# RozDavid/UnScene3D

Measured on AMD Instinct MI355X. Metric: training scenes/sec (Res16UNet34C+Mask3D, 150k voxels), higher is better.
Workload: dtype f32

## Files before the change

include/usc3d.h:

```cpp
#ifndef USC3D_H
#define USC3D_H

#include <stdint.h>

#ifdef __cplusplus
extern "C" {
#endif

typedef void* usc_stream_t;

enum usc_status {
  USC_OK = 0,
  USC_ERR_ARG = -1,
  USC_ERR_LAUNCH = -2,
  USC_ERR_RANGE = -3
};

const char* usc_last_error(void);
int usc_abi_version(void);
const char* usc_build_info(void);
int usc_device_count(void);


int usc_voxel_floor_f64(const double* xyz, int64_t n, double voxel_size,
                        int32_t* coords_out, usc_stream_t s);

int usc_voxel_floor_f64_host(const double* xyz, int64_t n, double voxel_size,
                             int32_t* coords_out);
int usc_unique_coords_host(const int32_t* coords, int64_t n, int32_t d,
                           int64_t* unique_idx, int64_t* inverse,
                           int64_t* n_out);

int64_t usc_coordmap_capacity(int64_t n);
int64_t usc_coordmap_ws_bytes(int64_t n);

int usc_coordmap_build(const int32_t* coords, int64_t n, int32_t quant,
                       uint64_t* table_keys, int32_t* table_vals, int64_t cap,
                       int64_t* unique_idx, int64_t* inverse,
                       int32_t* out_coords, int64_t* n_out,
                       void* ws, int64_t ws_bytes, usc_stream_t s);

int usc_morton_cell_ids(const int32_t* coords, int64_t n, int32_t shift,
                        int32_t lo_x, int32_t lo_y, int32_t lo_z,
                        int32_t bits_per_axis, int64_t* ids, usc_stream_t s);


int usc_kernel_map_cube(const int32_t* coords, int64_t n, int32_t tensor_stride,
                        int32_t ksize, const uint64_t* table_keys,
                        const int32_t* table_vals, int64_t cap, int32_t* nbr,
                        usc_stream_t s);

int usc_kernel_map_down2(const int32_t* fine_coords, int64_t n_fine,
                         int32_t tensor_stride, const int64_t* parent,
                         const int32_t* coarse_coords, int64_t n_coarse,
                         int32_t* nbr2, uint8_t* kidx, usc_stream_t s);

int64_t usc_rulebook_ws_bytes(int64_t K, int64_t n_out);
int usc_rulebook_compact(const int32_t* nbr, int64_t K, int64_t n_out,
                         int32_t* in_idx, int32_t* out_idx, int64_t* koff,
                         void* ws, int64_t ws_bytes, usc_stream_t s);


int usc_weight_transpose(const float* W, int32_t K, int32_t cin, int32_t cout,
                         int32_t mirror, float* out, usc_stream_t s);

int usc_spconv_plan(int32_t kind, int64_t n, int32_t cin, int32_t cout,
                    int32_t K);
int64_t usc_rowsort_ws_bytes(int32_t K, int64_t n_out);
int usc_rowsort_build(const int32_t* nbr, int32_t K, int64_t n_out,
                      int32_t* perm, uint32_t* tile_mask, void* ws,
                      int64_t ws_bytes, usc_stream_t s);
int64_t usc_spconv_sorted_ws_bytes(int64_t n_out, int32_t cin, int32_t cout,
                                   int32_t K);
int usc_spconv_sorted_gemm(const float* in, int64_t n_in, int32_t cin,
                           const float* W, int32_t K, int32_t cout,
                           const int32_t* nbr, const int32_t* perm,
                           const uint32_t* tile_mask, int64_t n_out,
                           const float* bias, float* out, int32_t accumulate,
                           int32_t w_transposed, void* ws, int64_t ws_bytes,
                           usc_stream_t s);
int usc_spconv_sorted_gemm_ex(const float* in, int64_t n_in, int32_t cin,
                              const float* W, int32_t K, int32_t cout,
                              const int32_t* nbr, const int32_t* perm,
                              const uint32_t* tile_mask, int64_t n_out,
                              const float* bias, float* out, int32_t accumulate,
                              int32_t w_transposed, void* ws, int64_t ws_bytes,
                              int32_t* slices_left, usc_stream_t s);
int usc_group_reduce(const float* partial, int32_t G, int64_t n, int32_t c,
                     const float* bias, int32_t accumulate, float* out,
                     usc_stream_t s);

int64_t usc_spconv_gather_gemm_ws_bytes(int64_t n_out, int32_t cin,
                                        int32_t cout, int32_t K);
int usc_spconv_gather_gemm(const float* in, int64_t n_in, int32_t cin,
                           const float* W, int32_t K, int32_t cout,
                           const int32_t* nbr, int64_t n_out,
                           const float* bias, float* out, int32_t accumulate, int32_t w_transposed,
                           void* ws, int64_t ws_bytes, usc_stream_t s);

int usc_spconv_pairs_gemm(const float* in, int32_t cin, const float* W,
                          int32_t K, int32_t cout, const int32_t* rows_in,
                          const int32_t* rows_out, const int64_t* koff,
                          int64_t P_capacity, float* out, usc_stream_t s);

int usc_cast_bf16(const float* in, int64_t n, uint16_t* out, usc_stream_t s);
int usc_spconv_pack_w_bf16(const float* W, int32_t K, int32_t cin, int32_t cout,
                           uint16_t* Wp, usc_stream_t s);
int64_t usc_spconv_gather_gemm_bf16_ws_bytes(int64_t n_out, int32_t cin,
                                             int32_t cout, int32_t K);
int usc_spconv_gather_gemm_bf16(const uint16_t* in, int64_t n_in, int32_t cin,
                                const uint16_t* Wp, int32_t K, int32_t cout,
                                const int32_t* nbr, int64_t n_out,
                                const float* bias, float* out, int32_t accumulate,
                                void* ws, int64_t ws_bytes, usc_stream_t s);

int usc_split_bf16_rows(const float* in, int64_t rows, int32_t c, int32_t P,
                        uint16_t* out, usc_stream_t s);
int usc_split_bf16(const float* in, int64_t n, int32_t P, uint16_t* out,
                   usc_stream_t s);
int usc_spconv_pack_w_split(const float* W, int32_t K, int32_t cin, int32_t cout,
                            int32_t P, int32_t transposed, uint16_t* Wp,
                            usc_stream_t s);
int64_t usc_spconv_gather_gemm_split_ws_bytes(int64_t n_out, int32_t cin,
                                              int32_t cout, int32_t K, int32_t P);
int usc_spconv_gather_gemm_split(const uint16_t* in, int64_t n_in, int32_t cin,
                                 const uint16_t* Wp, int32_t K, int32_t cout,
                                 int32_t P, const int32_t* nbr, int64_t n_out,
                                 const float* bias, float* out,
                                 int32_t accumulate, void* ws, int64_t ws_bytes,
                                 usc_stream_t s);

int64_t usc_spconv_wgrad_ws_bytes(int32_t K, int32_t cin, int32_t cout);
int usc_spconv_wgrad(const float* a, int32_t cin, const float* b, int32_t cout,
                     int32_t K, const int32_t* a_idx, const int32_t* b_idx,
                     const int64_t* koff, int64_t n_rows, float* dW, int32_t accumulate, void* ws,
                     int64_t ws_bytes, usc_stream_t s);
int64_t usc_spconv_wgrad_ws_bytes_rows(int32_t K, int32_t cin, int32_t cout,
                                       int64_t n_rows);
int64_t usc_spconv_wgrad_table_ws_bytes(int32_t K, int32_t cin, int32_t cout);
int usc_spconv_wgrad_table(const float* in, int32_t cin, const float* dy, int32_t cout, const int32_t* nbr, int32_t K,
                           int64_t n_out, float* dW, int32_t accumulate, void* ws, int64_t ws_bytes, usc_stream_t s);

void usc_spconv_wgrad_grid_limit(int32_t max_workgroups);
int32_t usc_spconv_wgrad_group_max(void);
int usc_spconv_wgrad_group_ok(int32_t R, int32_t cin, int32_t cout, int32_t K, int64_t n_rows);
int usc_spconv_wgrad_group(int32_t R, const float* const* a, const float* const* b, float* const* dW, int32_t cin,
                           int32_t cout, int32_t K, const int32_t* a_idx, const int32_t* b_idx, const int64_t* koff,
                           int64_t n_rows, int32_t accumulate, usc_stream_t s);

typedef struct usc_kmap {
  const int32_t* nbr;
  const int32_t* perm;
  const uint32_t* tile_mask;
  const int32_t* pair_in;
  const int32_t* pair_out;
  const int64_t* koff;
  int64_t n_in, n_out;
  int64_t pair_capacity;
  int32_t K;
  int32_t reserved;
} usc_kmap;

enum usc_conv_kind { USC_CONV_SAME = 0, USC_CONV_DOWN = 1, USC_CONV_UP = 2 };

typedef struct usc_bn {
  const float* gamma;
  const float* beta;
  float* running_mean;
  float* running_var;
  int64_t* num_batches_tracked;
  float eps, momentum;
  int32_t c;
  int32_t training;
} usc_bn;

int usc_set_wgrad_lane(usc_stream_t lane, void* lane_ws, int64_t lane_ws_bytes, int64_t max_rows);
int usc_wgrad_lane_join(usc_stream_t s);
int usc_wgrad_lane_hold(int32_t mode, int64_t hold_min_rows, int64_t release_max_rows, usc_stream_t s);
int32_t usc_wgrad_lane_holding(void);
typedef struct usc_launch_stat { int64_t n_out; int32_t cin, cout, K, nb; } usc_launch_stat;
int usc_launch_stats_begin(void* ring_dev, int64_t slots, usc_stream_t s);
int64_t usc_launch_stats_end(usc_launch_stat* host_out, int64_t max_out);
int64_t usc_wall_clock_khz(void);
int64_t usc_conv_ws_bytes(const usc_kmap* m, int32_t kind, int32_t cin,
                          int32_t cout);
int64_t usc_unit_ws_bytes(const usc_kmap* m, int32_t kind, int32_t cin,
                          int32_t cout);
int usc_conv_forward(const usc_kmap* m, int32_t kind, const float* x,
                     int32_t cin, const float* W, int32_t cout,
                     const float* bias, float* y, void* ws, int64_t ws_bytes,
                     usc_stream_t s);
int usc_conv_backward(const usc_kmap* m, int32_t kind, const float* x,
                      int32_t cin, const float* W, int32_t cout,
                      const float* dy, float* dx, int32_t dx_accumulate,
                      float* dW, int32_t dW_accumulate, void* ws,
                      int64_t ws_bytes, usc_stream_t s);
int usc_bn_eval_stats(const float* gamma, const float* beta,
                      const float* running_mean, const float* running_var,
                      float eps, int32_t c, float* mean, float* invstd,
                      float* scale, float* shift, usc_stream_t s);
int usc_conv_bn_act_forward(const usc_kmap* m, int32_t kind, const float* x,
                            int32_t cin, const float* W, int32_t cout,
                            const usc_bn* bn, const float* residual,
                            int32_t relu, float* y, float* stats, float* out,
                            void* ws, int64_t ws_bytes, usc_stream_t s);
int usc_conv_bn_act_backward(const usc_kmap* m, int32_t kind, const float* x,
                             int32_t cin, const float* W, int32_t cout,
                             const usc_bn* bn, const float* y,
                             const float* stats, const float* out_relu,
                             const float* dout, float* dy, float* dres,
                             float* dx, int32_t dx_accumulate, float* dW,
                             int32_t dW_accumulate, float* dgamma,
                             float* dbeta, int32_t dbn_accumulate, void* ws,
                             int64_t ws_bytes, usc_stream_t s);
int64_t usc_unit_bf16_ws_bytes(const usc_kmap* m, int32_t kind, int32_t cin,
                               int32_t cout);
int usc_conv_bn_act_forward_bf16(const usc_kmap* m, int32_t kind,
                                 const float* x, int32_t cin,
                                 const uint16_t* Wp, int32_t cout,
                                 const usc_bn* bn, const float* residual,
                                 int32_t relu, float* y, float* stats,
                                 float* out, void* ws, int64_t ws_bytes,
                                 usc_stream_t s);

int64_t usc_unit_split_ws_bytes(const usc_kmap* m, int32_t kind, int32_t cin,
                                int32_t cout, int32_t P);
int usc_conv_bn_act_forward_split(const usc_kmap* m, int32_t kind,
                                  const float* x, int32_t cin, const float* W,
                                  int32_t cout, int32_t P, const usc_bn* bn,
                                  const float* residual, int32_t relu, float* y,
                                  float* stats, float* out, void* ws,
                                  int64_t ws_bytes, usc_stream_t s);
int usc_conv_bn_act_backward_split(const usc_kmap* m, int32_t kind,
                                   const float* x, int32_t cin, const float* W,
                                   int32_t cout, int32_t P, const usc_bn* bn,
                                   const float* y, const float* stats,
                                   const float* out_relu, const float* dout,
                                   float* dy, float* dres, float* dx,
                                   int32_t dx_accumulate, float* dW,
                                   int32_t dW_accumulate, float* dgamma,
                                   float* dbeta, int32_t dbn_accumulate,
                                   void* ws, int64_t ws_bytes, usc_stream_t s);

enum usc_step_op { USC_STEP_UNIT_FWD = 0, USC_STEP_UNIT_BWD = 1, USC_STEP_CAT = 2, USC_STEP_SPLIT = 3, USC_STEP_ADD = 4,
                   USC_STEP_UNIT_FWD_BF16 = 5 };
typedef struct usc_step {
  int32_t op, kind, cin, cout, relu;
  int32_t dx_accumulate, dW_accumulate, dbn_accumulate, defer_wgrad, accumulate;
  const usc_kmap* map;
  const usc_bn* bn;
  const float* x;
  const float* W;
  const float* residual;
  float* y;
  float* stats;
  float* out;
  const float* dout;
  float* dy;
  float* dres;
  float* dx;
  float* dW;
  float* dgamma;
  float* dbeta;
  const float* a;
  const float* b;
  float* dst;
  float* dst2;
  int64_t n;
  int32_t ca, cb;
  int32_t split_planes, reserved;
} usc_step;
int32_t usc_step_size(void);
int64_t usc_program_ws_bytes(const usc_step* steps, int32_t n_steps);
int usc_program_run(const usc_step* steps, int32_t begin, int32_t end, void* ws, int64_t ws_bytes, usc_stream_t s);


int64_t usc_colstats_ws_bytes(int64_t n, int32_t c);
int usc_colstats(const float* x, const float* y, int64_t n, int32_t c,
                 double* sum1, double* sum2, void* ws, int64_t ws_bytes,
                 usc_stream_t s);
int usc_bn_forward_stats(const float* x, int64_t n, int32_t c, const float* gamma,
                         const float* beta, float eps, float momentum,
                         float* running_mean, float* running_var, int64_t* num_batches_tracked, float* mean,
                         float* invstd, float* scale, float* shift, void* ws,
                         int64_t ws_bytes, usc_stream_t s);
int usc_bn_apply(const float* x, const float* scale, const float* shift,
                 const float* residual, int32_t relu, float* y, int64_t n,
                 int32_t c, usc_stream_t s);
int usc_bn_backward_dx(const float* x, const float* dy, const float* y_out,
                       const float* mean, const float* invstd,
                       const float* gamma, const float* mean_g,
                       const float* mean_gxhat, float* dx, float* dres,
                       int64_t n, int32_t c, usc_stream_t s);
int64_t usc_bn_tile_max_rows(void);
int64_t usc_bn_plan(int64_t n, int32_t c, int32_t backward);
int usc_bn_tile_ok(int64_t n, int32_t c);
int64_t usc_bn_tile_ws_bytes(int32_t c);
int usc_bn_tile_forward(const float* partial, int32_t G, float* y, int64_t n,
                        int32_t c, const float* gamma, const float* beta,
                        float eps, float momentum, float* running_mean,
                        float* running_var, int64_t* num_batches_tracked,
                        float* mean, float* invstd, float* scale, float* shift,
                        const float* residual, int32_t relu, float* out,
                        void* ws, int64_t ws_bytes, usc_stream_t s);
int usc_bn_tile_backward(const float* partial, int32_t G, int32_t accumulate,
                         float* dout, const float* y, const float* y_out,
                         const float* mean, const float* invstd,
                         const float* gamma, int64_t n, int32_t c,
                         int32_t training, int32_t dbn_accumulate,
                         float* dgamma, float* dbeta, float* dy, float* dres,
                         void* ws, int64_t ws_bytes, usc_stream_t s);
int usc_bn_backward_reduce(const float* x, const float* dy, const float* y_out,
                           const float* mean, const float* invstd, int64_t n,
                           int32_t c, int32_t training, int32_t accumulate, float* dgamma,
                           float* dbeta, float* mean_g, float* mean_gxhat,
                           void* ws, int64_t ws_bytes, usc_stream_t s);
int usc_relu_fwd(const float* x, float* y, int64_t numel, usc_stream_t s);
int usc_relu_bwd(const float* y, const float* dy, float* dx, int64_t numel,
                 usc_stream_t s);

int usc_avgpool_down2(const float* in, int32_t c, const int32_t* nbr2,
                      int64_t n_coarse, float* out, usc_stream_t s);
int usc_avgpool_down2_ex(const float* in, int32_t c, int32_t ld,
                         const int64_t* row_of, const int32_t* nbr2,
                         int64_t n_coarse, float* out, uint8_t* mask_out,
                         usc_stream_t s);

int usc_gather_rows(const float* src, int32_t c, const int64_t* idx, int64_t n,
                    float* out, usc_stream_t s);

int usc_scatter_add_rows(const float* src, int32_t c, const int64_t* idx,
                         int64_t n, float* dst, usc_stream_t s);

int usc_scatter_rows_unique(const float* src, int32_t c, const int64_t* idx,
                            int64_t n, float* dst, usc_stream_t s);
int usc_scatter_rows_unique_add(const float* src, int32_t c, const int64_t* idx,
                                int64_t n, float* dst, usc_stream_t s);

int64_t usc_sample_keys_ws_bytes(int32_t n_scenes, int32_t K, int32_t q);
int usc_sample_keys(const float* feats, int32_t c, const uint8_t* mask, int32_t q, const float* pos, int32_t p,
                    const int64_t* idx, int32_t n_scenes, int32_t K, const int32_t* n_valid, float* out_feats,
                    uint8_t* out_mask, float* out_pos, void* ws, int64_t ws_bytes, usc_stream_t s);

int64_t usc_segment_csr_ws_bytes(int64_t n, int64_t S);
int usc_segment_csr(const int64_t* seg, int64_t n, int64_t S, int64_t* order,
                    int64_t* seg_off, void* ws, int64_t ws_bytes,
                    usc_stream_t s);
int usc_segment_mean_fwd(const float* src, int32_t c, const int64_t* order,
                         const int64_t* seg_off, int64_t S, float* out,
                         usc_stream_t s);
int usc_segment_mean_bwd(const float* dout, int32_t c, const int64_t* seg,
                         const int64_t* seg_off, int64_t n, float* dsrc,
                         usc_stream_t s);

int usc_segment_mean_nonzero(const float* feats, int32_t d,
                             const int64_t* order, const int64_t* seg_off,
                             int64_t S, float* out, int64_t* nonzero_cnt,
                             usc_stream_t s);
int usc_segment_max_nonzero(const float* feats, int32_t d,
                            const int64_t* order, const int64_t* seg_off,
                            int64_t S, float* out, int64_t* nonzero_cnt,
                            usc_stream_t s);

int32_t usc_attn_max_queries(void);
int32_t usc_attn_lse_stride(int32_t L);
int64_t usc_attn_ws_bytes(int32_t L, int32_t S, int32_t B, int32_t H);
int usc_attn_fwd(const float* q, const float* k, const float* v,
                 const uint8_t* mask, int32_t L, int32_t S, int32_t B, int32_t H,
                 int32_t E, float* o, float* lse, void* ws, int64_t ws_bytes,
                 usc_stream_t s);
int usc_attn_bwd(const float* q, const float* k, const float* v,
                 const uint8_t* mask, const float* o, const float* lse,
                 const float* dO, int32_t L, int32_t S, int32_t B, int32_t H,
                 int32_t E, float* dq, float* dk, float* dv,
                 int32_t mask_bits_in_ws ,
                 void* ws, int64_t ws_bytes, usc_stream_t s);

int usc_self_attn_fwd(const float* q, const float* k, const float* v, int32_t L,
                      int32_t B, int32_t H, int32_t E, float* o, float* lse,
                      usc_stream_t s);
int usc_self_attn_bwd(const float* q, const float* k, const float* v, const float* o,
                      const float* lse, const float* dO, int32_t L, int32_t B,
                      int32_t H, int32_t E, float* dq, float* dk, float* dv,
                      usc_stream_t s);

int usc_lsap_batch(const float* cost, int32_t n_prob, int32_t nr, int32_t nc,
                   int64_t* row_ind, int64_t* col_ind, int32_t* status, usc_stream_t s);

int64_t usc_criterion_ws_bytes(int32_t L, int32_t S, int32_t T);
int usc_criterion_target_bits(const uint8_t* tm, int32_t T, int32_t max_targets, int32_t S,
                              uint32_t* bits, int32_t* cnt, usc_stream_t s);
int usc_criterion_costs(const float* const* masks, int32_t L, int32_t ld, int32_t S,
                        int32_t Q, int32_t T, int32_t max_targets, const uint32_t* bits,
                        const int32_t* cnt, const float* logits, int64_t ls_level, int64_t ls_q,
                        int32_t C, const int64_t* labels, float w_mask, float w_class,
                        float w_dice, float* cost, float* cmask, float* cdice, float* nmat,
                        float* ssum, float* logp, void* ws, int64_t ws_bytes, usc_stream_t s);
int usc_criterion_drop_counts(const float* const* masks, int32_t L, int32_t ld, int32_t S,
                              int32_t Q, int32_t T, int32_t max_targets, const uint32_t* bits,
                              const int64_t* src, const int64_t* tid, int32_t* counts,
                              usc_stream_t s);
int usc_criterion_losses(const float* cmask, const float* cdice, const float* logp,
                         const int64_t* src, const int64_t* tid, const int64_t* labels,
                         const float* class_w, int32_t L, int32_t Q, int32_t T,
                         int32_t max_targets, int32_t C, int32_t noobj, int32_t* tcls, float* part,
                         const int32_t* counts, const int32_t* cnt, float thresh, float* wts,
                         usc_stream_t s);
int usc_criterion_table(const float* parts, int32_t B, int32_t L, float* table,
                        float* den_tot, usc_stream_t s);
int usc_criterion_backward(const float* const* masks, float* const* dmasks, int32_t L,
                           int32_t ld, int32_t S, int32_t Q, int32_t T, int32_t max_targets,
                           const uint32_t* bits, const int32_t* cnt, const int64_t* src,
                           const int64_t* tid, const float* nmat, const float* ssum,
                           const float* logp, const int32_t* tcls, const float* class_w,
                           const float* gtable, const float* den_tot, int32_t C, int64_t ls_level,
                           int64_t ls_q, float* dlogits, const float* wts, usc_stream_t s);

int usc_linear_fwd(const float* x, const float* W, const float* b, int32_t M,
                   int32_t N, int32_t K, float* y, usc_stream_t s);
int usc_linear_bwd(const float* dy, const float* x, const float* W, int32_t M,
                   int32_t N, int32_t K, float* dx, float* dW, float* db,
                   int32_t accumulate, usc_stream_t s);
int usc_linear_fwd_ex(const float* x, const float* x2, const float* W,
                      const float* b, int32_t M, int32_t N, int32_t K,
                      int32_t relu, float* y, usc_stream_t s);
int usc_linear_fwd_pad(const float* x, const float* x2, const float* W, const float* b, int32_t M, int32_t N, int32_t K,
                       int32_t relu, float* y, int32_t M_pad, usc_stream_t s);
int usc_linear_fwd_split(const float* x, const float* x2, const float* W, const float* b, int32_t M, int32_t N, int32_t K,
                         int32_t x2_cols, int32_t split_cols, float* y, usc_stream_t s);
int usc_linear_bwd_ex(const float* dy, const float* y_relu, const float* x,
                      const float* x2, const float* W, int32_t M, int32_t N,
                      int32_t K, float* dx, const float* dx_add, float* dW,
                      float* db, int32_t accumulate, usc_stream_t s);
int usc_linear_bwd_ex2(const float* dy, const float* y_relu, const float* x, const float* x2, const float* W, int32_t M,
                       int32_t N, int32_t K, float* dx, const float* dx_add, const float* dx_add2, float* dx_b, float* dW,
                       float* db, int32_t accumulate, usc_stream_t s);
int usc_qkv_proj_bwd(const float* dy3, const float* x, const float* pos, const float* W, int32_t M, int32_t E, float* dx,
                     float* dx_b, const float* dres, float* dW, float* db, int32_t accumulate, usc_stream_t s);
int64_t usc_col_sum_ws_bytes(int64_t n, int32_t c);
int usc_col_sum(const float* x, int64_t n, int32_t c, float* out,
                int32_t accumulate, void* ws, int64_t ws_bytes, usc_stream_t s);

int usc_layernorm_fwd(const float* x, const float* gamma, const float* beta,
                      int64_t rows, int32_t d, float eps, float* y, float* mean,
                      float* rstd, usc_stream_t s);
int usc_add_layernorm_fwd(const float* x, const float* res, const float* gamma,
                          const float* beta, int64_t rows, int32_t d, float eps,
                          float* y, float* sum_out, float* mean, float* rstd,
                          usc_stream_t s);
int64_t usc_layernorm_bwd_ws_bytes(int64_t rows, int32_t d);
int usc_layernorm_bwd(const float* dy, const float* x, const float* mean,
                      const float* rstd, const float* gamma, int64_t rows,
                      int32_t d, float* dx, float* dgamma, float* dbeta,
                      int32_t accumulate, void* ws, int64_t ws_bytes,
                      usc_stream_t s);
int usc_layernorm_bwd_ex(const float* dy, const float* x, const float* mean,
                         const float* rstd, const float* gamma, int64_t rows,
                         int32_t d, const float* dx_add, float* dx, float* dgamma,
                         float* dbeta, int32_t accumulate, void* ws,
                         int64_t ws_bytes, usc_stream_t s);

int usc_furthest_point_sampling(const float* xyz, int32_t b, int32_t n,
                                int32_t m, float* tmp, int32_t* idx,
                                usc_stream_t s);

int usc_fourier_posenc(const float* xyz, int64_t n, const float* lo,
                       const float* hi, const float* gauss_B, int32_t d,
                       float* out, usc_stream_t s);

int usc_ncut_similarity(const float* F, int64_t S, int32_t d,
                        int32_t cosine_mode, float* normed, float* sim,
                        usc_stream_t s);
int usc_ncut_similarity_masked(const float* F, const uint8_t* zero_rows, int64_t S,
                               int32_t d, int32_t cosine_mode, float* normed,
                               float* sim, usc_stream_t s);
int usc_ncut_normalize_mat(float* A, int64_t S, void* ws, int64_t ws_bytes,
                           usc_stream_t s);
int usc_ncut_binarize(const float* simA, const float* simB, int64_t S, float tau,
                      double eps, const uint8_t* painted, uint8_t* Abin,
                      double* deg, usc_stream_t s);
int64_t usc_ncut_fiedler_ws_bytes(int64_t S);
int usc_ncut_fiedler(const uint8_t* Abin, const double* deg, int64_t S, double eps,
                     double* evec, double* eval, void* ws, int64_t ws_bytes,
                     usc_stream_t s);
int usc_ncut_fiedler_ex(const uint8_t* Abin, const double* deg, int64_t S, double eps,
                        double* evec, double* eval, void* ws, int64_t ws_bytes,
                        usc_stream_t s, int32_t flags);
int32_t usc_ncut_fiedler_plan(int64_t S, int32_t cus, int32_t flags);

int usc_knn1(const float* query, int64_t nq, const float* ref, int64_t nr,
             int64_t* idx, float* dist2, usc_stream_t s);

int usc_cc_eps_init(int32_t* label, int64_t n, usc_stream_t s);
int usc_cc_eps_step(const float* xyz, int64_t n, float eps,
                    const int32_t* label_in, int32_t* label_out,
                    int32_t* changed, usc_stream_t s);
int usc_cc_eps_finish(const int32_t* label, int64_t n, int32_t* rank_ws,
                      int64_t* labels, usc_stream_t s);

int usc_project_planes_fwd(const int32_t* coords, const float* pred,
                           const float* target, int64_t V, int32_t inst,
                           int32_t dim_x, int32_t dim_y, int32_t dim_z,
                           float* pred_xy, float* pred_xz, float* pred_yz,
                           float* tgt_xy, float* tgt_xz, float* tgt_yz,
                           int32_t* cnt_xy, int32_t* cnt_xz, int32_t* cnt_yz,
                           usc_stream_t s);
int usc_project_planes_bwd(const int32_t* coords, int64_t V, int32_t inst,
                           int32_t dim_x, int32_t dim_y, int32_t dim_z,
                           const float* g_xy, const float* g_xz,
                           const float* g_yz, float* grad_pred,
                           usc_stream_t s);

int usc_brick_mask_build(const int32_t* coords, int64_t n, const int32_t* shift, int32_t B,
                         int32_t bricks_x, int32_t bricks_y, int32_t bricks_z,
                         uint32_t* mask, usc_stream_t s);
int usc_raycast_first_hit_map(const uint64_t* table_keys, const int32_t* table_vals,
                              int64_t cap, int64_t n_rows, const int32_t* shift,
                              const uint32_t* brick_mask , int32_t bricks_x,
                              int32_t bricks_y, int32_t bricks_z,
                              const float* views, const float* intrinsics,
                              int32_t B, int32_t V, int32_t H, int32_t W,
                              float depth_min, float depth_max, float ray_increment,
                              int32_t* hit, int64_t* seg, usc_stream_t s);
int usc_raycast_first_hit_dense(const int64_t* occupancy, int32_t dim_z, int32_t dim_y,
                                int32_t dim_x, int64_t n_rows, const float* views,
                                const float* intrinsics, int32_t B, int32_t V,
                                int32_t H, int32_t W, float depth_min, float depth_max,
                                float ray_increment, int32_t* hit, int64_t* seg,
                                usc_stream_t s);
int usc_project_reduce(const float* feats, int32_t c, const int64_t* order,
                       const int64_t* seg_off, int64_t n_rows, int32_t mode,
                       float* out, int32_t* num, usc_stream_t s);
int usc_project_predictions(const int32_t* preds, int32_t c, const int32_t* hit,
                            int64_t n_pix, int32_t* out, usc_stream_t s);
int usc_unproject_depth(const float* depth, const float* views, const float* intrinsics,
                        int32_t V, int32_t H, int32_t W, float* cloud, usc_stream_t s);

int usc_spin(int64_t microseconds, int wgs, usc_stream_t s);

int usc_adamw_step(float* param, const float* grad, float* exp_avg, float* exp_avg_sq,
                   int64_t n, float lr, float beta1, float beta2, float eps,
                   float weight_decay, int64_t step, usc_stream_t s);

int usc_adamw_step_scaled(float* param, float* grad, float* exp_avg, float* exp_avg_sq, int64_t n,
                          float grad_scale, int32_t write_back_grad,
                          float lr, float beta1, float beta2, float eps, float weight_decay,
                          int64_t step, usc_stream_t s);

int usc_elastic_displace(const void* xyz_in, int32_t is_f64, int64_t n, int32_t row_stride,
                         const float* noise, int32_t dim_x, int32_t dim_y, int32_t dim_z,
                         const double* axis_x, const double* axis_y, const double* axis_z,
                         double magnitude, void* xyz_out, usc_stream_t s);

int usc_affine_rows(void* x, int32_t is_f64, int64_t n, int32_t row_stride,
                    const double* M, const double* t, usc_stream_t s);
int usc_colsum_sequential(const float* x, int64_t n, int32_t row_stride,
                          int32_t cols, float* out, usc_stream_t s);
int usc_color_lut(const float* color, int64_t n, int32_t row_stride,
                  const float* lut, float* out, int32_t out_stride,
                  usc_stream_t s);

int usc_felz_face_normals(const float* vertices, const int32_t* faces,
                          int64_t n_faces, float* face_normals, usc_stream_t s);
int usc_felz_vertex_normals(const float* face_normals, const int64_t* corner_order,
                            const int64_t* vertex_off, int64_t n_vertices,
                            float* normals, usc_stream_t s);
int usc_felz_edge_weights(const float* vertices, const float* colors,
                          const float* normals, const int32_t* faces,
                          int64_t n_faces, int32_t* edge_a, int32_t* edge_b,
                          float* weights, usc_stream_t s);
int usc_felz_merge_host(const int32_t* edge_a, const int32_t* edge_b,
                        const float* weights, int64_t n_edges, int32_t n_vertices,
                        float kthr, int32_t seg_min_verts, int32_t* comps);

int usc_mask_gt_overlap(const uint8_t* masks, int64_t n, int32_t k, int64_t ld,
                        const int32_t* slot, int32_t nslots, int32_t* counts,
                        usc_stream_t s);
// ... 20 lines not shown
```

unscene3d_amd/_lib.py:

```python
from __future__ import annotations

import ctypes as C
import os

import torch

_HERE = os.path.dirname(os.path.abspath(__file__))
LIB_PATH = os.environ.get("USC3D_LIB") or os.path.join(_HERE, "libusc3d_hip.so")

_p = C.c_void_p
_i32 = C.c_int32
_i64 = C.c_int64
_f64 = C.c_double
_f32 = C.c_float

class KMap(C.Structure):
    _fields_ = [("nbr", _p), ("perm", _p), ("tile_mask", _p), ("pair_in", _p), ("pair_out", _p), ("koff", _p),
                ("n_in", _i64), ("n_out", _i64), ("pair_capacity", _i64), ("K", _i32), ("reserved", _i32)]


class BNDesc(C.Structure):
    _fields_ = [("gamma", _p), ("beta", _p), ("running_mean", _p), ("running_var", _p), ("num_batches_tracked", _p),
                ("eps", _f32), ("momentum", _f32), ("c", _i32), ("training", _i32)]


_kp = C.POINTER(KMap)
_bp = C.POINTER(BNDesc)


class Step(C.Structure):
    _fields_ = [("op", _i32), ("kind", _i32), ("cin", _i32), ("cout", _i32), ("relu", _i32),
                ("dx_accumulate", _i32), ("dW_accumulate", _i32), ("dbn_accumulate", _i32), ("defer_wgrad", _i32),
                ("accumulate", _i32),
                ("map", _p), ("bn", _p),
                ("x", _p), ("W", _p), ("residual", _p), ("y", _p), ("stats", _p), ("out", _p),
                ("dout", _p), ("dy", _p), ("dres", _p), ("dx", _p), ("dW", _p), ("dgamma", _p), ("dbeta", _p),
                ("a", _p), ("b", _p), ("dst", _p), ("dst2", _p), ("n", _i64), ("ca", _i32), ("cb", _i32),
                ("split_planes", _i32), ("reserved", _i32)]


_sp = C.POINTER(Step)
STEP_UNIT_FWD, STEP_UNIT_BWD, STEP_CAT, STEP_SPLIT, STEP_ADD, STEP_UNIT_FWD_BF16 = 0, 1, 2, 3, 4, 5

SIGNATURES = {
    "usc_last_error": (C.c_char_p, []),
    "usc_abi_version": (C.c_int, []),
    "usc_build_info": (C.c_char_p, []),
    "usc_device_count": (C.c_int, []),
    "usc_voxel_floor_f64": (C.c_int, [_p, _i64, _f64, _p, _p]),
    "usc_voxel_floor_f64_host": (C.c_int, [_p, _i64, C.c_double, _p]),
    "usc_unique_coords_host": (C.c_int, [_p, _i64, _i32, _p, _p, _p]),
    "usc_coordmap_capacity": (_i64, [_i64]),
    "usc_coordmap_ws_bytes": (_i64, [_i64]),
    "usc_coordmap_build": (C.c_int, [_p, _i64, _i32, _p, _p, _i64, _p, _p, _p, _p, _p, _i64, _p]),
    "usc_morton_cell_ids": (C.c_int, [_p, _i64, _i32, _i32, _i32, _i32, _i32, _p, _p]),
    "usc_kernel_map_cube": (C.c_int, [_p, _i64, _i32, _i32, _p, _p, _i64, _p, _p]),
    "usc_kernel_map_down2": (C.c_int, [_p, _i64, _i32, _p, _p, _i64, _p, _p, _p]),
    "usc_rulebook_ws_bytes": (_i64, [_i64, _i64]),
    "usc_rulebook_compact": (C.c_int, [_p, _i64, _i64, _p, _p, _p, _p, _i64, _p]),
    "usc_weight_transpose": (C.c_int, [_p, _i32, _i32, _i32, _i32, _p, _p]),
    "usc_spconv_plan": (C.c_int, [_i32, _i64, _i32, _i32, _i32]),
    "usc_spconv_gather_gemm_ws_bytes": (_i64, [_i64, _i32, _i32, _i32]),
    "usc_spconv_gather_gemm": (C.c_int, [_p, _i64, _i32, _p, _i32, _i32, _p, _i64, _p, _p, _i32, _i32, _p, _i64, _p]),
    "usc_rowsort_ws_bytes": (_i64, [_i32, _i64]),
    "usc_rowsort_build": (C.c_int, [_p, _i32, _i64, _p, _p, _p, _i64, _p]),
    "usc_spconv_sorted_ws_bytes": (_i64, [_i64, _i32, _i32, _i32]),
    "usc_spconv_sorted_gemm": (C.c_int, [_p, _i64, _i32, _p, _i32, _i32, _p, _p, _p, _i64, _p, _p, _i32, _i32, _p, _i64, _p]),
    "usc_spconv_sorted_gemm_ex": (C.c_int, [_p, _i64, _i32, _p, _i32, _i32, _p, _p, _p, _i64, _p, _p, _i32, _i32, _p, _i64, _p, _p]),
    "usc_group_reduce": (C.c_int, [_p, _i32, _i64, _i32, _p, _i32, _p, _p]),
    "usc_bn_tile_max_rows": (C.c_int64, []),
    "usc_bn_plan": (_i64, [_i64, _i32, _i32]),
    "usc_bn_tile_ok": (C.c_int, [_i64, _i32]),
    "usc_bn_tile_ws_bytes": (C.c_int64, [_i32]),
    "usc_bn_tile_forward": (C.c_int, [_p, _i32, _p, _i64, _i32, _p, _p, _f32, _f32, _p, _p, _p, _p, _p, _p, _p, _p, _i32, _p,
                                      _p, _i64, _p]),
    "usc_bn_tile_backward": (C.c_int, [_p, _i32, _i32, _p, _p, _p, _p, _p, _p, _i64, _i32, _i32, _i32, _p, _p, _p, _p, _p,
                                       _i64, _p]),
    "usc_spconv_pairs_gemm": (C.c_int, [_p, _i32, _p, _i32, _i32, _p, _p, _p, _i64, _p, _p]),
    "usc_cast_bf16": (C.c_int, [_p, _i64, _p, _p]),
    "usc_spconv_pack_w_bf16": (C.c_int, [_p, _i32, _i32, _i32, _p, _p]),
    "usc_spconv_gather_gemm_bf16_ws_bytes": (_i64, [_i64, _i32, _i32, _i32]),
    "usc_spconv_gather_gemm_bf16": (C.c_int, [_p, _i64, _i32, _p, _i32, _i32, _p, _i64, _p, _p, _i32, _p, _i64, _p]),
    "usc_split_bf16_rows": (C.c_int, [_p, _i64, _i32, _i32, _p, _p]),
    "usc_split_bf16": (C.c_int, [_p, _i64, _i32, _p, _p]),
    "usc_spconv_pack_w_split": (C.c_int, [_p, _i32, _i32, _i32, _i32, _i32, _p, _p]),
    "usc_spconv_gather_gemm_split_ws_bytes": (_i64, [_i64, _i32, _i32, _i32, _i32]),
    "usc_spconv_gather_gemm_split": (C.c_int, [_p, _i64, _i32, _p, _i32, _i32, _i32, _p, _i64, _p, _p, _i32, _p, _i64, _p]),
    "usc_spconv_wgrad_ws_bytes": (_i64, [_i32, _i32, _i32]),
    "usc_spconv_wgrad": (C.c_int, [_p, _i32, _p, _i32, _i32, _p, _p, _p, _i64, _p, _i32, _p, _i64, _p]),
    "usc_spconv_wgrad_ws_bytes_rows": (_i64, [_i32, _i32, _i32, _i64]),
    "usc_step_size": (_i32, []),
    "usc_program_ws_bytes": (_i64, [_sp, _i32]),
    "usc_program_run": (C.c_int, [_sp, _i32, _i32, _p, _i64, _p]),
    "usc_spconv_wgrad_group_max": (_i32, []),
    "usc_spconv_wgrad_grid_limit": (None, [_i32]),
    "usc_spconv_wgrad_group_ok": (C.c_int, [_i32, _i32, _i32, _i32, _i64]),
    "usc_spconv_wgrad_group": (C.c_int, [_i32, _p, _p, _p, _i32, _i32, _i32, _p, _p, _p, _i64, _i32, _p]),
    "usc_spconv_wgrad_table_ws_bytes": (_i64, [_i32, _i32, _i32]),
    "usc_spconv_wgrad_table": (C.c_int, [_p, _i32, _p, _i32, _p, _i32, _i64, _p, _i32, _p, _i64, _p]),
    "usc_set_wgrad_lane": (C.c_int, [_p, _p, _i64, _i64]),
    "usc_wgrad_lane_join": (C.c_int, [_p]),
    "usc_wgrad_lane_hold": (C.c_int, [_i32, _i64, _i64, _p]),
    "usc_wgrad_lane_holding": (_i32, []),
    "usc_launch_stats_begin": (C.c_int, [_p, _i64, _p]),
    "usc_launch_stats_end": (_i64, [_p, _i64]),
    "usc_wall_clock_khz": (_i64, []),
    "usc_conv_ws_bytes": (_i64, [_kp, _i32, _i32, _i32]),
    "usc_unit_ws_bytes": (_i64, [_kp, _i32, _i32, _i32]),
    "usc_conv_forward": (C.c_int, [_kp, _i32, _p, _i32, _p, _i32, _p, _p, _p, _i64, _p]),
    "usc_conv_backward": (C.c_int, [_kp, _i32, _p, _i32, _p, _i32, _p, _p, _i32, _p, _i32, _p, _i64, _p]),
    "usc_bn_eval_stats": (C.c_int, [_p, _p, _p, _p, _f32, _i32, _p, _p, _p, _p, _p]),
    "usc_conv_bn_act_forward": (C.c_int, [_kp, _i32, _p, _i32, _p, _i32, _bp, _p, _i32, _p, _p, _p, _p, _i64, _p]),
    "usc_unit_bf16_ws_bytes": (_i64, [_kp, _i32, _i32, _i32]),
    "usc_conv_bn_act_forward_bf16": (C.c_int, [_kp, _i32, _p, _i32, _p, _i32, _bp, _p, _i32, _p, _p, _p, _p, _i64, _p]),
    "usc_unit_split_ws_bytes": (_i64, [_kp, _i32, _i32, _i32, _i32]),
    "usc_conv_bn_act_forward_split": (C.c_int, [_kp, _i32, _p, _i32, _p, _i32, _i32, _bp, _p, _i32, _p, _p, _p, _p, _i64, _p]),
    "usc_conv_bn_act_backward_split": (C.c_int, [_kp, _i32, _p, _i32, _p, _i32, _i32, _bp, _p, _p, _p, _p, _p, _p, _p, _i32, _p,
                                                 _i32, _p, _p, _i32, _p, _i64, _p]),
    "usc_conv_bn_act_backward": (C.c_int, [_kp, _i32, _p, _i32, _p, _i32, _bp, _p, _p, _p, _p, _p, _p, _p, _i32, _p,
                                           _i32, _p, _p, _i32, _p, _i64, _p]),
    "usc_colstats_ws_bytes": (_i64, [_i64, _i32]),
    "usc_colstats": (C.c_int, [_p, _p, _i64, _i32, _p, _p, _p, _i64, _p]),
    "usc_bn_apply": (C.c_int, [_p, _p, _p, _p, _i32, _p, _i64, _i32, _p]),
    "usc_bn_backward_dx": (C.c_int, [_p, _p, _p, _p, _p, _p, _p, _p, _p, _p, _i64, _i32, _p]),
    "usc_bn_backward_reduce": (C.c_int, [_p, _p, _p, _p, _p, _i64, _i32, _i32, _i32, _p, _p, _p, _p, _p, _i64, _p]),
    "usc_bn_forward_stats": (C.c_int, [_p, _i64, _i32, _p, _p, _f32, _f32, _p, _p, _p, _p, _p, _p, _p, _p, _i64, _p]),
    "usc_relu_fwd": (C.c_int, [_p, _p, _i64, _p]),
    "usc_relu_bwd": (C.c_int, [_p, _p, _p, _i64, _p]),
    "usc_avgpool_down2": (C.c_int, [_p, _i32, _p, _i64, _p, _p]),
    "usc_avgpool_down2_ex": (C.c_int, [_p, _i32, _i32, _p, _p, _i64, _p, _p, _p]),
    "usc_gather_rows": (C.c_int, [_p, _i32, _p, _i64, _p, _p]),
    "usc_scatter_add_rows": (C.c_int, [_p, _i32, _p, _i64, _p, _p]),
    "usc_scatter_rows_unique": (C.c_int, [_p, _i32, _p, _i64, _p, _p]),
    "usc_scatter_rows_unique_add": (C.c_int, [_p, _i32, _p, _i64, _p, _p]),
    "usc_sample_keys_ws_bytes": (_i64, [_i32, _i32, _i32]),
    "usc_sample_keys": (C.c_int, [_p, _i32, _p, _i32, _p, _i32, _p, _i32, _i32, _p, _p, _p, _p, _p, _i64, _p]),
    "usc_segment_csr_ws_bytes": (_i64, [_i64, _i64]),
    "usc_segment_csr": (C.c_int, [_p, _i64, _i64, _p, _p, _p, _i64, _p]),
    "usc_segment_mean_fwd": (C.c_int, [_p, _i32, _p, _p, _i64, _p, _p]),
    "usc_segment_mean_bwd": (C.c_int, [_p, _i32, _p, _p, _i64, _p, _p]),
    "usc_segment_mean_nonzero": (C.c_int, [_p, _i32, _p, _p, _i64, _p, _p, _p]),
    "usc_segment_max_nonzero": (C.c_int, [_p, _i32, _p, _p, _i64, _p, _p, _p]),
    "usc_ncut_similarity": (C.c_int, [_p, _i64, _i32, _i32, _p, _p, _p]),
    "usc_ncut_similarity_masked": (C.c_int, [_p, _p, _i64, _i32, _i32, _p, _p, _p]),
    "usc_ncut_normalize_mat": (C.c_int, [_p, _i64, _p, _i64, _p]),
    "usc_ncut_binarize": (C.c_int, [_p, _p, _i64, _f32, _f64, _p, _p, _p, _p]),
    "usc_ncut_fiedler_ws_bytes": (_i64, [_i64]),
    "usc_ncut_fiedler": (C.c_int, [_p, _p, _i64, _f64, _p, _p, _p, _i64, _p]),
    "usc_ncut_fiedler_ex": (C.c_int, [_p, _p, _i64, _f64, _p, _p, _p, _i64, _p, _i32]),
    "usc_ncut_fiedler_plan": (_i32, [_i64, _i32, _i32]),
    "usc_knn1": (C.c_int, [_p, _i64, _p, _i64, _p, _p, _p]),
    "usc_cc_eps_init": (C.c_int, [_p, _i64, _p]),
    "usc_cc_eps_step": (C.c_int, [_p, _i64, _f32, _p, _p, _p, _p]),
    "usc_cc_eps_finish": (C.c_int, [_p, _i64, _p, _p, _p]),
    "usc_project_planes_fwd": (C.c_int, [_p, _p, _p, _i64, _i32, _i32, _i32, _i32] + [_p] * 10),
    "usc_project_planes_bwd": (C.c_int, [_p, _i64, _i32, _i32, _i32, _i32, _p, _p, _p, _p, _p]),
    "usc_brick_mask_build": (C.c_int, [_p, _i64, _p, _i32, _i32, _i32, _i32, _p, _p]),
    "usc_raycast_first_hit_map": (C.c_int, [_p, _p, _i64, _i64, _p, _p, _i32, _i32, _i32, _p, _p, _i32, _i32, _i32, _i32,
                                            _f32, _f32, _f32, _p, _p, _p]),
    "usc_raycast_first_hit_dense": (C.c_int, [_p, _i32, _i32, _i32, _i64, _p, _p, _i32, _i32, _i32, _i32, _f32, _f32,
                                              _f32, _p, _p, _p]),
    "usc_project_reduce": (C.c_int, [_p, _i32, _p, _p, _i64, _i32, _p, _p, _p]),
    "usc_project_predictions": (C.c_int, [_p, _i32, _p, _i64, _p, _p]),
    "usc_unproject_depth": (C.c_int, [_p, _p, _p, _i32, _i32, _i32, _p, _p]),
    "usc_spin": (C.c_int, [_i64, C.c_int, _p]),
    "usc_adamw_step": (C.c_int, [_p, _p, _p, _p, _i64, _f32, _f32, _f32, _f32, _f32, _i64, _p]),
    "usc_adamw_step_scaled": (C.c_int, [_p, _p, _p, _p, _i64, _f32, _i32, _f32, _f32, _f32, _f32, _f32, _i64, _p]),
    "usc_elastic_displace": (C.c_int, [_p, _i32, _i64, _i32, _p, _i32, _i32, _i32, _p, _p, _p, _f64, _p, _p]),
    "usc_attn_max_queries": (_i32, []),
    "usc_attn_lse_stride": (_i32, [_i32]),
    "usc_attn_ws_bytes": (_i64, [_i32, _i32, _i32, _i32]),
    "usc_attn_fwd": (C.c_int, [_p, _p, _p, _p, _i32, _i32, _i32, _i32, _i32, _p, _p, _p, _i64, _p]),
    "usc_attn_bwd": (C.c_int, [_p, _p, _p, _p, _p, _p, _p, _i32, _i32, _i32, _i32, _i32, _p, _p, _p, _i32, _p, _i64, _p]),
    "usc_lsap_batch": (C.c_int, [_p, _i32, _i32, _i32, _p, _p, _p, _p]),
    "usc_criterion_ws_bytes": (_i64, [_i32, _i32, _i32]),
    "usc_criterion_target_bits": (C.c_int, [_p, _i32, _i32, _i32, _p, _p, _p]),
    "usc_criterion_costs": (C.c_int, [_p, _i32, _i32, _i32, _i32, _i32, _i32, _p, _p, _p, _i64, _i64, _i32, _p, _f32, _f32,
                                      _f32, _p, _p, _p, _p, _p, _p, _p, _i64, _p]),
    "usc_criterion_drop_counts": (C.c_int, [_p, _i32, _i32, _i32, _i32, _i32, _i32, _p, _p, _p, _p, _p]),
    "usc_criterion_losses": (C.c_int, [_p, _p, _p, _p, _p, _p, _p, _i32, _i32, _i32, _i32, _i32, _i32, _p, _p, _p, _p,
                                       _f32, _p, _p]),
    "usc_criterion_table": (C.c_int, [_p, _i32, _i32, _p, _p, _p]),
    "usc_criterion_backward": (C.c_int, [_p, _p, _i32, _i32, _i32, _i32, _i32, _i32, _p, _p, _p, _p, _p, _p, _p, _p, _p,
                                         _p, _p, _i32, _i64, _i64, _p, _p, _p]),
    "usc_self_attn_fwd": (C.c_int, [_p, _p, _p, _i32, _i32, _i32, _i32, _p, _p, _p]),
    "usc_self_attn_bwd": (C.c_int, [_p, _p, _p, _p, _p, _p, _i32, _i32, _i32, _i32, _p, _p, _p, _p]),
    "usc_linear_fwd": (C.c_int, [_p, _p, _p, _i32, _i32, _i32, _p, _p]),
    "usc_linear_bwd": (C.c_int, [_p, _p, _p, _i32, _i32, _i32, _p, _p, _p, _i32, _p]),
    "usc_layernorm_fwd": (C.c_int, [_p, _p, _p, _i64, _i32, _f32, _p, _p, _p, _p]),
    "usc_add_layernorm_fwd": (C.c_int, [_p, _p, _p, _p, _i64, _i32, _f32, _p, _p, _p, _p, _p]),
    "usc_linear_fwd_ex": (C.c_int, [_p, _p, _p, _p, _i32, _i32, _i32, _i32, _p, _p]),
    "usc_linear_fwd_pad": (C.c_int, [_p, _p, _p, _p, _i32, _i32, _i32, _i32, _p, _i32, _p]),
    "usc_linear_fwd_split": (C.c_int, [_p, _p, _p, _p, _i32, _i32, _i32, _i32, _i32, _p, _p]),
    "usc_linear_bwd_ex": (C.c_int, [_p, _p, _p, _p, _p, _i32, _i32, _i32, _p, _p, _p, _p, _i32, _p]),
    "usc_qkv_proj_bwd": (C.c_int, [_p, _p, _p, _p, _i32, _i32, _p, _p, _p, _p, _p, _i32, _p]),
    "usc_linear_bwd_ex2": (C.c_int, [_p, _p, _p, _p, _p, _i32, _i32, _i32, _p, _p, _p, _p, _p, _p, _i32, _p]),
    "usc_layernorm_bwd_ws_bytes": (_i64, [_i64, _i32]),
    "usc_layernorm_bwd": (C.c_int, [_p, _p, _p, _p, _p, _i64, _i32, _p, _p, _p, _i32, _p, _i64, _p]),
    "usc_layernorm_bwd_ex": (C.c_int, [_p, _p, _p, _p, _p, _i64, _i32, _p, _p, _p, _p, _i32, _p, _i64, _p]),
    "usc_affine_rows": (C.c_int, [_p, _i32, _i64, _i32, _p, _p, _p]),
    "usc_colsum_sequential": (C.c_int, [_p, _i64, _i32, _i32, _p, _p]),
    "usc_col_sum_ws_bytes": (_i64, [_i64, _i32]),
    "usc_col_sum": (C.c_int, [_p, _i64, _i32, _p, _i32, _p, _i64, _p]),
    "usc_color_lut": (C.c_int, [_p, _i64, _i32, _p, _p, _i32, _p]),
    "usc_felz_face_normals": (C.c_int, [_p, _p, _i64, _p, _p]),
    "usc_felz_vertex_normals": (C.c_int, [_p, _p, _p, _i64, _p, _p]),
    "usc_felz_edge_weights": (C.c_int, [_p, _p, _p, _p, _i64, _p, _p, _p, _p]),
    "usc_felz_merge_host": (C.c_int, [_p, _p, _p, _i64, _i32, _f32, _i32, _p]),
    "usc_furthest_point_sampling": (C.c_int, [_p, _i32, _i32, _i32, _p, _p, _p]),
    "usc_fourier_posenc": (C.c_int, [_p, _i64, _p, _p, _p, _i32, _p, _p]),
    "usc_mask_gt_overlap": (C.c_int, [_p, _i64, _i32, _i64, _p, _i32, _p, _p]),
    "usc_vit_attn_head_dim": (_i32, []),
    "usc_vit_attn_fwd": (C.c_int, [_p, _i32, _i32, _i32, _f32, _i32, _p, _p]),
    "usc_instance_index": (C.c_int, [_p, _i64, _i32, _p, _i32, _p, _p, _p, _p]),
    "usc_instance_select": (C.c_int, [_p, _i64, _i32, _p, _i32, _p, _p, _p, _i32, _i64, _p, _p, _p, _p]),
    "usc_instance_masks": (C.c_int, [_p, _i64, _p, _i32, _i32, _p, _p, _i32, _i64, _p, _p]),
}


class LaunchStat(C.Structure):
    _fields_ = [("n_out", _i64), ("cin", _i32), ("cout", _i32), ("K", _i32), ("nb", _i32)]


def _load():
    if not os.path.exists(LIB_PATH):
        raise ImportError(
            f"{LIB_PATH} is missing: build the HIP extension first "
            "(`python -c 'import __graft_entry__ as g; g.build()'`). "
            "unscene3d_amd has no CPU fallback."
        )
    lib = C.CDLL(LIB_PATH)
    for name, (res, args) in SIGNATURES.items():
        fn = getattr(lib, name)
        fn.restype = res
        fn.argtypes = args
    return lib


lib = _load()
if lib.usc_step_size() != C.sizeof(Step):
    raise ImportError(f"unscene3d_amd._lib.Step ({C.sizeof(Step)} bytes) does not mirror usc_step "
                      f"({lib.usc_step_size()} bytes): rebuild the library or fix the binding")


def last_error() -> str:
    return lib.usc_last_error().decode("utf-8", "replace")


def check(rc: int, what: str = "") -> None:
    if rc != 0:
        raise RuntimeError(f"{what or 'libusc3d_hip'} failed (status {rc}): {last_error()}")


def require_device() -> None:
    n = lib.usc_device_count()
    if n <= 0:
        raise RuntimeError(
            "unscene3d_amd: no HIP device visible — the MI355X kernels cannot run and there is no CPU fallback"
        )
```

unscene3d_amd/csrc/spconv.hip:

```cpp
#include "common.h"

#include <stdlib.h>

#include <vector>

namespace usc {

typedef float f32x16 __attribute__((ext_vector_type(16)));

#define MFMA32(a, b, c) __builtin_amdgcn_mfma_f32_32x32x2f32((a), (b), (c), 0, 0, 0)

struct GemmParams {
  const float* in;
  const float* W;
  const int32_t* nbr;
  const float* bias;
  float* out;
  int64_t n_out;
  int cin, cout, K;
  int accumulate;
  int G;
  int TM;
  int wt1;
  const int32_t* rows_in;
// ... 585 lines not shown
  f32x16 acc[NB];
#pragma unroll
  for (int nb = 0; nb < NB; ++nb)
#pragma unroll
    for (int r = 0; r < 16; ++r) acc[nb][r] = 0.f;

  const bool ci_ok = ci0 + i < cin;
  const int acol = ci0 + i;
  const int bcol = ALIGNED ? co0 + NB * i : co0 + i;
  auto load_idx = [&](int64_t q) -> int64_t {
    int64_t idxreg = -1;
    const int l16 = lane & 15;
    const int64_t pp = q + l16;
    if (lane < 32 && pp < ce) {
      if (p.a_idx)
        idxreg = (lane < 16) ? p.a_idx[pp] : p.b_idx[pp];
      else
        idxreg = pp;
    }
    return idxreg;
  };
  auto load_rows = [&](int64_t idxreg, float (&av)[8], float (&bv)[8][NB]) {
#pragma unroll
    for (int u = 0; u < 8; ++u) {
      const int64_t ia = __shfl(idxreg, 2 * u + h, 64);
      const int64_t ib = __shfl(idxreg, 16 + 2 * u + h, 64);
      if (ALIGNED) {
        const float t = p.a[(ia >= 0 ? ia : 0) * cin + acol];
        av[u] = ia >= 0 ? t : 0.f;
        load_b<NB>(p.b + (ib >= 0 ? ib : 0) * cout + bcol, bv[u]);
      } else {
        av[u] = (ia >= 0 && ci_ok) ? p.a[ia * cin + acol] : 0.f;
#pragma unroll
        for (int nb = 0; nb < NB; ++nb)
          bv[u][nb] = (ib >= 0 && bcol + nb * 32 < cout) ? p.b[ib * cout + bcol + nb * 32] : 0.f;
      }
    }
  };
  auto run = [&](float (&av)[8], float (&bv)[8][NB]) {
#pragma unroll
    for (int u = 0; u < 8; ++u)
#pragma unroll
      for (int nb = 0; nb < NB; ++nb) acc[nb] = MFMA32(av[u], bv[u][nb], acc[nb]);
  };
  if (ALIGNED) {
    float aX[8], aY[8];
    float bX[8][NB], bY[8][NB];
    int64_t id1 = load_idx(cb), id2 = load_idx(cb + 16);
    load_rows(id1, aX, bX);
    for (int64_t q = cb; q < ce; q += 32) {
      int64_t id3 = load_idx(q + 32);
      load_rows(id2, aY, bY);
      run(aX, bX);
      id2 = load_idx(q + 48);
      load_rows(id3, aX, bX);
      if (q + 16 < ce) run(aY, bY);
    }
  } else {
    float av[8];
    float bv[8][NB];
    for (int64_t q = cb; q < ce; q += 16) {
      load_rows(load_idx(q), av, bv);
      run(av, bv);
    }
  }

  if (wave > 0) {
#pragma unroll
    for (int nb = 0; nb < NB; ++nb)
#pragma unroll
      for (int r = 0; r < 16; ++r) red[((wave - 1) * NB * 16 + nb * 16 + r) * 64 + lane] = acc[nb][r];
  }
  __syncthreads();
  if (wave == 0) {
#pragma unroll
    for (int w = 0; w < 3; ++w)
#pragma unroll
      for (int nb = 0; nb < NB; ++nb)
#pragma unroll
        for (int r = 0; r < 16; ++r) acc[nb][r] += red[(w * NB * 16 + nb * 16 + r) * 64 + lane];
    float* dst = p.partial + ((int64_t)s * p.K + k) * cin * cout;
#pragma unroll
    for (int r = 0; r < 16; ++r) {
      const int ci = ci0 + acc_row(r, h);
      if (ci >= cin) continue;
#pragma unroll
      for (int nb = 0; nb < NB; ++nb) {
        const int co = ALIGNED ? bcol + nb : bcol + nb * 32;
        if (co < cout) dst[(int64_t)ci * cout + co] = acc[nb][r];
      }
    }
  }
}

constexpr int kMaxWgradGroup = 16;
struct WgradGroup { const float* a[kMaxWgradGroup]; const float* b[kMaxWgradGroup]; float* dW[kMaxWgradGroup]; int R; };

template <int CT, int NB>
__global__ __launch_bounds__(256, (CT * NB > 9) ? 1 : 2) void wgrad_full_kernel(WgradParams p, WgradGroup g) {
  extern __shared__ float red[];
  constexpr int NA = CT * NB;
  const int lane = threadIdx.x & 63, wave = threadIdx.x >> 6;
  const int i = lane & 31, h = lane >> 5;
  const int vtotal = p.vblocks > 0 ? p.vblocks : (int)gridDim.x;
  for (int vb = blockIdx.x; vb < vtotal; vb += gridDim.x) {
  int bx = vb;
  if (g.R > 0) {
    const int per = p.K * p.S, r = bx / per;
    bx -= r * per;
    p.a = g.a[r]; p.b = g.b[r]; p.direct = g.dW[r];
  }
  const int k = bx / p.S, s = bx % p.S;
  const int ci0 = blockIdx.y * (32 * CT), co0 = blockIdx.z * (NB * 32);
  const int cin = p.cin, cout = p.cout;
  int64_t pb, pe;
  if (p.a_idx) { pb = p.koff[k]; pe = p.koff[k + 1]; } else { pb = 0; pe = p.n_rows; }
  const int64_t nchunks = (int64_t)p.S * 4;
  int64_t L = (pe - pb + nchunks - 1) / nchunks;
  L = (L + 7) & ~7ll;
  const int64_t cb = pb + ((int64_t)s * 4 + wave) * L;
  int64_t ce = cb + L;
  if (ce > pe) ce = pe;

  f32x16 acc[NA];
#pragma unroll
  for (int t = 0; t < NA; ++t)
#pragma unroll
    for (int r = 0; r < 16; ++r) acc[t][r] = 0.f;

  auto load_idx = [&](int64_t q) __attribute__((always_inline)) -> int {
    int v = -1;
    const int64_t pp = q + (lane & 7);
    if (lane < 16 && pp < ce) v = p.a_idx ? ((lane < 8) ? p.a_idx[pp] : p.b_idx[pp]) : (int)pp;
    return v;
  };
  auto load_rows = [&](int idxreg, float (&av)[4][CT], float (&bv)[4][NB]) __attribute__((always_inline)) {
#pragma unroll
    for (int u = 0; u < 4; ++u) {
      const int ia = __shfl(idxreg, 2 * u + h, 64);
      const int ib = __shfl(idxreg, 8 + 2 * u + h, 64);
      const float* ap = p.a + (int64_t)(ia >= 0 ? ia : 0) * cin + ci0 + CT * i;
      const float* bp = p.b + (int64_t)(ib >= 0 ? ib : 0) * cout + co0 + NB * i;
      const float keep = ia >= 0 ? 1.f : 0.f;
      load_b<CT>(ap, av[u]);
#pragma unroll
      for (int ct = 0; ct < CT; ++ct) av[u][ct] *= keep;
      load_b<NB>(bp, bv[u]);
    }
  };
  auto run = [&](float (&av)[4][CT], float (&bv)[4][NB]) __attribute__((always_inline)) {
#pragma unroll
    for (int u = 0; u < 4; ++u)
#pragma unroll
      for (int ct = 0; ct < CT; ++ct)
#pragma unroll
        for (int nb = 0; nb < NB; ++nb) acc[ct * NB + nb] = MFMA32(av[u][ct], bv[u][nb], acc[ct * NB + nb]);
  };
  float aX[4][CT], aY[4][CT], bX[4][NB], bY[4][NB];
  int id1 = load_idx(cb), id2 = load_idx(cb + 8);
  load_rows(id1, aX, bX);
  for (int64_t q = cb; q < ce; q += 16) {
    const int id3 = load_idx(q + 16);
    load_rows(id2, aY, bY);
    run(aX, bX);
    id2 = load_idx(q + 24);
    load_rows(id3, aX, bX);
    if (q + 8 < ce) run(aY, bY);
  }

  float* dst = (p.direct ? p.direct : p.partial + (int64_t)s * p.K * cin * cout) + (int64_t)k * cin * cout;
  const bool rmw = p.direct && p.accumulate;
  const bool vec_ok = (reinterpret_cast<uintptr_t>(dst) & (NB * 4 - 1)) == 0;
#pragma unroll
  for (int ct = 0; ct < CT; ++ct) {
    if (ct) __syncthreads();
#pragma unroll
    for (int nb = 0; nb < NB; ++nb)
#pragma unroll
      for (int r = 0; r < 16; ++r) red[((wave * NB + nb) * 16 + r) * 64 + lane] = acc[ct * NB + nb][r];
    __syncthreads();
#pragma unroll
    for (int rr = 0; rr < 4; ++rr) {
      const int r = 4 * wave + rr;
      float v[NB];
#pragma unroll
      for (int nb = 0; nb < NB; ++nb) {
        float t = red[((3 * NB + nb) * 16 + r) * 64 + lane];
        t += red[((2 * NB + nb) * 16 + r) * 64 + lane];
        t += red[((1 * NB + nb) * 16 + r) * 64 + lane];
        v[nb] = red[(nb * 16 + r) * 64 + lane] + t;
      }
      const int ci = ci0 + CT * acc_row(r, h) + ct;
      float* o = dst + (int64_t)ci * cout + co0 + NB * i;
      if (NB == 4 && vec_ok) {
        float4 w4 = make_float4(v[0], v[1], v[2 % NB], v[3 % NB]);
        if (rmw) {
          const float4 old = *reinterpret_cast<const float4*>(o);
          w4.x += old.x; w4.y += old.y; w4.z += old.z; w4.w += old.w;
        }
        *reinterpret_cast<float4*>(o) = w4;
      } else if (NB == 2 && vec_ok) {
        float2 w2 = make_float2(v[0], v[1 % NB]);
        if (rmw) {
          const float2 old = *reinterpret_cast<const float2*>(o);
          w2.x += old.x; w2.y += old.y;
        }
        *reinterpret_cast<float2*>(o) = w2;
      } else {
#pragma unroll
        for (int nb = 0; nb < NB; ++nb) o[nb] = rmw ? o[nb] + v[nb] : v[nb];
      }
    }
  }
  __syncthreads();
  }
}

constexpr int kStemSplits = 64;
constexpr int kStemWaves = 16;
__global__ __launch_bounds__(64 * kStemWaves) void stem_wgrad_kernel(const float* __restrict__ in, const float* __restrict__ dy,
                                                                    const int32_t* __restrict__ nbr, int64_t n_out, int K,
                                                                    int cin, float* __restrict__ partial) {
  __shared__ float red[kStemWaves][16][64];
  const int lane = threadIdx.x & 63, wave = threadIdx.x >> 6, i = lane & 31, h = lane >> 5;
  const int per = 32 / cin;
  const int g = blockIdx.y, s = blockIdx.x, S = gridDim.x;
  const int j = i / cin, c = i - j * cin, k = g * per + j;
  const bool active = j < per && k < K;
  int64_t L = (n_out + S - 1) / S;
  L = (L + 2 * kStemWaves - 1) / (2 * kStemWaves) * (2 * kStemWaves);
  const int64_t r_begin = (int64_t)s * L;
  int64_t r_end = r_begin + L;
  if (r_end > n_out) r_end = n_out;
  const int32_t* nk = nbr + (int64_t)(active ? k : 0) * n_out;
  f32x16 acc;
#pragma unroll
  for (int r = 0; r < 16; ++r) acc[r] = 0.f;
  for (int64_t rb = r_begin + 2 * wave; rb < r_end; rb += 8 * kStemWaves) {
    int id[4];
    float b[4];
#pragma unroll
    for (int u = 0; u < 4; ++u) {
      const int64_t r = rb + h + 2 * kStemWaves * u;
      const bool ok = r < r_end;
      id[u] = (ok && active) ? nk[r] : -1;
      b[u] = ok ? dy[r * 32 + i] : 0.f;
    }
    float a[4];
#pragma unroll
    for (int u = 0; u < 4; ++u) a[u] = id[u] >= 0 ? in[(int64_t)id[u] * cin + c] : 0.f;
#pragma unroll
    for (int u = 0; u < 4; ++u) acc = __builtin_amdgcn_mfma_f32_32x32x2f32(a[u], b[u], acc, 0, 0, 0);
  }
#pragma unroll
  for (int r = 0; r < 16; ++r) red[wave][r][lane] = acc[r];
  __syncthreads();
  if (wave >= 4) return;
  float* dst = partial + (int64_t)s * K * cin * 32;
#pragma unroll
  for (int q = 0; q < 4; ++q) {
    const int r = 4 * wave + q;
    const int m = acc_row(r, h);
    float v = red[kStemWaves - 1][r][lane];
#pragma unroll
    for (int w = kStemWaves - 2; w >= 0; --w) v += red[w][r][lane];
    const int row = g * per * cin + m;
    if (m < per * cin && row < K * cin) dst[(int64_t)row * 32 + i] = v;
  }
}

__global__ void wgrad_reduce_kernel(const float* __restrict__ partial, int S, int64_t numel, int accumulate,
                                    float* __restrict__ dW) {
  if ((numel & 3) == 0 && (reinterpret_cast<uintptr_t>(dW) & 15) == 0) {
    const int64_t n4 = numel >> 2;
    for (int64_t j = (int64_t)blockIdx.x * blockDim.x + threadIdx.x; j < n4; j += (int64_t)gridDim.x * blockDim.x) {
      float4 v = make_float4(0.f, 0.f, 0.f, 0.f);
      int s = 0;
      for (; s + 8 <= S; s += 8) {
        float4 t[8];
#pragma unroll
        for (int u = 0; u < 8; ++u) t[u] = reinterpret_cast<const float4*>(partial)[(int64_t)(s + u) * n4 + j];
#pragma unroll
        for (int u = 0; u < 8; ++u) { v.x += t[u].x; v.y += t[u].y; v.z += t[u].z; v.w += t[u].w; }
      }
      for (; s < S; ++s) {
        const float4 t = reinterpret_cast<const float4*>(partial)[(int64_t)s * n4 + j];
        v.x += t.x; v.y += t.y; v.z += t.z; v.w += t.w;
      }
      if (accumulate) {
        const float4 o = reinterpret_cast<const float4*>(dW)[j];
        v.x += o.x; v.y += o.y; v.z += o.z; v.w += o.w;
      }
      reinterpret_cast<float4*>(dW)[j] = v;
    }
    return;
  }
  for (int64_t j = (int64_t)blockIdx.x * blockDim.x + threadIdx.x; j < numel; j += (int64_t)gridDim.x * blockDim.x) {
    float v = 0.f;
    for (int s = 0; s < S; ++s) v += partial[(int64_t)s * numel + j];
    dW[j] = accumulate ? dW[j] + v : v;
  }
}

__global__ void weight_transpose_kernel(const float* __restrict__ W, int K, int cin, int cout, int mirror,
                                        float* __restrict__ out) {
  const int64_t per = (int64_t)cin * cout;
  const int64_t total = per * K;
  for (int64_t j = (int64_t)blockIdx.x * blockDim.x + threadIdx.x; j < total; j += (int64_t)gridDim.x * blockDim.x) {
    const int k = (int)(j / per);
    const int64_t rem = j - (int64_t)k * per;
    const int co = (int)(rem / cin), ci = (int)(rem - (int64_t)co * cin);
    const int ks = mirror ? (K - 1 - k) : k;
    out[j] = W[(int64_t)ks * per + (int64_t)ci * cout + co];
  }
}

__global__ void weight_pack_kernel(const float* __restrict__ W, int K, int cin, int cout, int NB, int wt,
                                   float* __restrict__ out) {
  const int64_t total = (int64_t)K * cin * cout;
  const int nq = cin >> 3, BN = NB * 32;
  for (int64_t e = (int64_t)blockIdx.x * blockDim.x + threadIdx.x; e < total; e += (int64_t)gridDim.x * blockDim.x) {
    int64_t r = e;
    const int j = (int)(r & 3); r >>= 2;
    const int ln = (int)(r & 63); r >>= 6;
    const int nb = (int)(r % NB); r /= NB;
    const int q = (int)(r % nq); r /= nq;
    const int k = (int)(r % K);
    const int cb = (int)(r / K);
    const int i = ln & 31, h = ln >> 5;
    const int c = 8 * q + 4 * h + j, n = cb * BN + NB * i + nb;
    out[e] = wt ? W[((int64_t)(K - 1 - k) * cout + n) * cin + c] : W[((int64_t)k * cin + c) * cout + n];
  }
}

static int wgrad_splits(int K, int cin, int cout, int NB, int64_t n_rows) {
  const int64_t tiles = (int64_t)K * ceil_div(cin, 32) * ceil_div(cout, NB * 32);
  const int target = (K > 1 && n_rows >= (int64_t)2 << 20) ? 4096 : 2048;
  int64_t S = ceil_div(target, tiles);
  const int64_t by_rows = n_rows / 2048 + 1;
  if (S > by_rows) S = by_rows;
  if (S > 64) S = 64;
  if (S < 1) S = 1;
  return (int)S;
}
static int wgrad_full_nb(int cb) { return (cb % 3 == 0) ? 3 : (cb % 4 == 0 ? 4 : (cb % 2 == 0 ? 2 : 1)); }
static int wgrad_full_ct(int ctiles, int NBf) {
  if (NBf == 3 && ctiles % 3 != 0 && ctiles % 4 == 0) return 4;
  return (ctiles % 3 == 0 && NBf * 3 <= 9) ? 3 : ((ctiles % 4 == 0 && NBf * 4 <= 9) ? 4 : ((ctiles % 2 == 0 && NBf * 2 <= 9) ? 2 : 1));
}
static int64_t wgrad_full_splits(int K, int ctiles, int cb, int CT, int NBf, int64_t n_rows) {
  const int64_t blocks_per_split = (int64_t)K * (ctiles / CT) * (cb / NBf);
  const int64_t tgt = (K > 1 && n_rows >= (int64_t)2 << 20) ? 2048 : 512;
  int64_t S = tgt / blocks_per_split;
  const int64_t by_rows = n_rows / (K > 1 ? 4096 : 256) + 1;
  if (S > by_rows) S = by_rows;
  if (S > 64) S = 64;
  if (S < 1) S = 1;
  return S;
}
static int pick_nb(int cout) {
  if (cout <= 32) return 1;
  if (cout <= 64) return 2;
  if (cout % 128 == 0) return 4;
  if (cout % 96 == 0) return 3;
  return 4;
}

struct GemmPlan { int NB; int G; bool aligned; int TM; };
constexpr int64_t kTargetWaves = 3072;

static bool stem_form(bool has_table, int cin, int cout, int K) {
  return has_table && cin >= 1 && cin <= 4 && cout == 32 && K >= 1 && K <= 32;
}

static GemmPlan plan_table(int64_t n_out, int cin, int cout, int K) {
  GemmPlan pl{pick_nb(cout), 1, false, 0};
  const bool al = (cin % 32 == 0) && (cout % 32 == 0);
  if (!al) return pl;
  pl.aligned = true;
  if (K > 1 && K <= kMaxK && n_out >= 24576 && cin >= 64 && cin <= kZeroRowFloats) {
    const int cb = cout / 32;
    const int nb = (cb % 3 == 0) ? 3 : (cb % 2 == 0 ? 2 : 1);
    constexpr int kTmMax3 = 192;
    constexpr int64_t kTileSlots = 256;
    const int tm_max = nb == 3 ? kTmMax3 : 256;
    int64_t R = 1;
    int64_t tm = ceil_div(n_out, kTileSlots * R);
    while (tm > tm_max) { ++R; tm = ceil_div(n_out, kTileSlots * R); }
    tm = (tm + 3) & ~3ll;
    pl.NB = nb;
    pl.TM = (int)tm;
    return pl;
  }
  const int64_t row_tiles = ceil_div(n_out, 32);
  const int cb = cout / 32;
  const int cands[4] = {4, 3, 2, 1};
  int chosen = 1;
  for (int c = 0; c < 4; ++c) {
    const int nb = cands[c];
    if (cb % nb) continue;
    if (row_tiles * (cb / nb) >= kTargetWaves) { chosen = nb; break; }
  }
  pl.NB = chosen;
  const int64_t waves = row_tiles * (cb / chosen);
  if (waves > 0 && waves < kTargetWaves && K > 1) {
    int64_t G = ceil_div(kTargetWaves, waves);
    if (G > K) G = K;
    pl.G = (int)G;
  }
  return pl;
}
static GemmPlan plan_list(int64_t max_tiles, int cin, int cout) {
  GemmPlan pl{pick_nb(cout), 1, false, 0};
  const bool al = (cin % 32 == 0) && (cout % 32 == 0);
  if (!al) return pl;
  pl.aligned = true;
  const int cb = cout / 32;
  const int cands[4] = {4, 3, 2, 1};
  int chosen = 1;
  for (int c = 0; c < 4; ++c) {
    const int nb = cands[c];
    if (cb % nb) continue;
    if (max_tiles * (cb / nb) >= kTargetWaves) { chosen = nb; break; }
  }
  pl.NB = chosen;
  return pl;
}

template <bool LIST>
static void launch_gemm(const GemmPlan& pl, dim3 grid, hipStream_t st, const GemmParams& p) {
#define USC_GG(NBv)                                                                                      \
  if (pl.aligned && p.wt1)        \
    hipLaunchKernelGGL((gather_gemm_aligned_kernel<NBv, false, true>), grid, dim3(256), 0, st, p);      \
  else if (pl.aligned)                                                                                   \
    hipLaunchKernelGGL((gather_gemm_aligned_kernel<NBv, LIST>), grid, dim3(256), 0, st, p);             \
  else                                                                                                   \
    hipLaunchKernelGGL((gather_gemm_kernel<NBv, LIST>), grid, dim3(256), 0, st, p);
  switch (pl.NB) {
    case 1: USC_GG(1) break;
    case 2: USC_GG(2) break;
    case 3: USC_GG(3) break;
    default: USC_GG(4) break;
  }
#undef USC_GG
}

}

using namespace usc;

extern "C" {

int usc_weight_transpose(const float* W, int32_t K, int32_t cin, int32_t cout, int32_t mirror, float* out,
                         usc_stream_t s) {
  USC_REQUIRE(W && out && K >= 1 && cin >= 1 && cout >= 1, "usc_weight_transpose: bad argument");
  const int64_t total = (int64_t)K * cin * cout;
  hipLaunchKernelGGL(weight_transpose_kernel, dim3(stream_grid(total, 256)), dim3(256), 0, as_stream(s), W, (int)K,
                     (int)cin, (int)cout, (int)mirror, out);
  USC_CHECK_LAUNCH("usc_weight_transpose");
  return USC_OK;
}

int usc_spconv_plan(int32_t kind, int64_t n, int32_t cin, int32_t cout, int32_t K) {
  GemmPlan pl;
  if (kind == 0 && stem_form(K > 1, cin, cout, K)) return 1 | (1 << 14);
  if (kind == 0) pl = plan_table(n, cin, cout, K);
  else if (kind == 1) pl = plan_list(ceil_div(n, 32) + K, cin, cout);
  else {
    const int ctiles = cin / 32, cb = cout / 32;
    const int NBf = (cb % 3 == 0) ? 3 : (cb % 4 == 0 ? 4 : (cb % 2 == 0 ? 2 : 1));
    if (cin % 32 == 0 && cout % 32 == 0 && (!(NBf == 3 && ctiles % 3 != 0) || ctiles % 4 == 0)) {
      const int CT = wgrad_full_ct(ctiles, NBf);
      return NBf | (1 << 8) | (1 << 13) | (CT << 16);
    }
    const int NB = pick_nb(cout);
    pl = GemmPlan{NB, 1, (cin % 32 == 0) && (cout % (NB * 32) == 0), 0};
  }
  return pl.NB | ((pl.aligned ? 1 : 0) << 8) | ((pl.TM > 0 ? 1 : 0) << 12) | (pl.G << 16);
}

int64_t usc_spconv_gather_gemm_ws_bytes(int64_t n_out, int32_t cin, int32_t cout, int32_t K) {
  const GemmPlan pl = plan_table(n_out, cin, cout, K);
  if (pl.TM > 0) return (int64_t)K * cin * cout * 4;
  return pl.G > 1 ? (int64_t)pl.G * n_out * cout * 4 : 0;
}

namespace {
struct LaunchStats { unsigned long long* ring = nullptr; int64_t slots = 0, count = 0; std::vector<usc_launch_stat> meta; };
LaunchStats g_lstats;
__global__ void launch_stats_init_kernel(unsigned long long* ring, int64_t slots) {
  const int64_t i = (int64_t)blockIdx.x * blockDim.x + threadIdx.x;
  if (i < slots) { ring[4 * i] = ~0ull; ring[4 * i + 1] = 0; ring[4 * i + 2] = 0; ring[4 * i + 3] = 0; }
}
}

int usc_launch_stats_begin(void* ring_dev, int64_t slots, usc_stream_t s) {
  USC_REQUIRE(ring_dev && slots > 0, "usc_launch_stats_begin: needs a device ring of slots x 4 x u64");
  hipLaunchKernelGGL(launch_stats_init_kernel, dim3((unsigned)ceil_div(slots, 256)), dim3(256), 0, as_stream(s),
                     (unsigned long long*)ring_dev, slots);
  USC_CHECK_LAUNCH("usc_launch_stats_begin");
  g_lstats.ring = (unsigned long long*)ring_dev;
  g_lstats.slots = slots;
  g_lstats.count = 0;
  g_lstats.meta.clear();
  g_lstats.meta.reserve((size_t)slots);
  return USC_OK;
}

int64_t usc_launch_stats_end(usc_launch_stat* host_out, int64_t max_out) {
  const int64_t n = g_lstats.count;
  if (host_out)
    for (int64_t i = 0; i < n && i < max_out; ++i) host_out[i] = g_lstats.meta[(size_t)i];
  g_lstats.ring = nullptr;
  g_lstats.slots = g_lstats.count = 0;
  g_lstats.meta.clear();
  return n;
}

int64_t usc_wall_clock_khz(void) {
  int dev = 0, khz = 0;
  if (hipGetDevice(&dev) != hipSuccess || hipDeviceGetAttribute(&khz, hipDeviceAttributeWallClockRate, dev) != hipSuccess) return 0;
  return khz;
}

int usc_spconv_gather_gemm(const float* in, int64_t n_in, int32_t cin, const float* W, int32_t K, int32_t cout,
                           const int32_t* nbr, int64_t n_out, const float* bias, float* out, int32_t accumulate,
                           int32_t w_transposed, void* ws, int64_t ws_bytes, usc_stream_t s) {
  USC_REQUIRE(cin >= 1 && cout >= 1 && K >= 1 && n_out >= 0 && n_in >= 0, "usc_spconv_gather_gemm: bad sizes");
  USC_REQUIRE(nbr || K == 1, "usc_spconv_gather_gemm: K>1 needs a neighbour table");
  USC_REQUIRE(nbr || n_in == n_out, "usc_spconv_gather_gemm: identity map needs n_in == n_out");
  if (n_out == 0) return USC_OK;
  USC_REQUIRE(in && W && out, "usc_spconv_gather_gemm: null pointer");
  if (stem_form(nbr != nullptr, cin, cout, K) && !accumulate && !w_transposed) {
    hipLaunchKernelGGL(stem_conv_kernel, dim3((unsigned)ceil_div(n_out, 256)), dim3(256), 0, as_stream(s), in, W, nbr, bias,
                       out, n_out, (int)K, (int)cin);
    USC_CHECK_LAUNCH("usc_spconv_gather_gemm");
    return USC_OK;
  }
  const GemmPlan pl = plan_table(n_out, cin, cout, K);
  GemmParams p{};
  p.in = in; p.W = W; p.nbr = nbr; p.bias = bias; p.out = out;
  p.n_out = n_out; p.cin = cin; p.cout = cout; p.K = K; p.accumulate = accumulate; p.G = pl.G;
  if (pl.G > 1) {
    USC_REQUIRE(ws && ws_bytes >= (int64_t)pl.G * n_out * cout * 4, "usc_spconv_gather_gemm: workspace too small");
    p.out = (float*)ws;
  }
  hipStream_t st = as_stream(s);
  const bool wt1 = w_transposed && K == 1 && !nbr && pl.aligned && pl.TM == 0;
  USC_REQUIRE(!w_transposed || pl.TM > 0 || wt1,
              "usc_spconv_gather_gemm: w_transposed is only folded into the tile-compacted kernel (usc_spconv_plan bit 12) "
              "and, for K = 1 on identity rows with channel counts in multiples of 32, into the row-order kernel; "
              "use usc_weight_transpose for other shapes");
  p.wt1 = wt1 ? 1 : 0;
  if (pl.TM > 0) {
    p.TM = pl.TM;
    USC_REQUIRE(ws && ws_bytes >= (int64_t)K * cin * cout * 4, "usc_spconv_gather_gemm: workspace too small");
    hipLaunchKernelGGL(weight_pack_kernel, dim3(stream_grid((int64_t)K * cin * cout, 256)), dim3(256), 0, st, W, (int)K,
                       (int)cin, (int)cout, pl.NB, (int)w_transposed, (float*)ws);
    p.W = (const float*)ws;
    dim3 cgrid((unsigned)ceil_div(n_out, pl.TM), (unsigned)(cout / (pl.NB * 32)));
    const size_t lds = compact_lds_bytes(pl.NB, pl.TM);
    if (g_lstats.ring && g_lstats.count < g_lstats.slots) {
      p.stats = g_lstats.ring + 4 * g_lstats.count++;
      g_lstats.meta.push_back(usc_launch_stat{n_out, cin, cout, K, pl.NB});
    }
#define USC_CG(NBv)                                                                                        \
    {                                                                                                      \
      static bool attr_set = false;                                                                        \
      auto kfn = gather_gemm_compact_kernel<NBv>;                                                          \
      if (!attr_set) {                                                                                     \
        (void)hipFuncSetAttribute((const void*)kfn, hipFuncAttributeMaxDynamicSharedMemorySize, 160 * 1024); \
        attr_set = true;                                                                                   \
      }                                                                                                    \
      hipLaunchKernelGGL(kfn, cgrid, dim3(64 * kCompactWaves), lds, st, p);                                \
    }
    if (pl.NB == 3) USC_CG(3) else if (pl.NB == 2) USC_CG(2) else USC_CG(1)
#undef USC_CG
    USC_CHECK_LAUNCH("usc_spconv_gather_gemm");
    return USC_OK;
  }
  dim3 grid((unsigned)ceil_div(n_out, 128), (unsigned)ceil_div(cout, pl.NB * 32), (unsigned)pl.G);
  launch_gemm<false>(pl, grid, st, p);
  if (pl.G > 1) {
    const int64_t numel4 = n_out * cout / 4;
    hipLaunchKernelGGL(group_reduce_kernel, dim3(stream_grid(numel4, 256)), dim3(256), 0, st, (const float*)ws, pl.G,
                       numel4, (int)cout, bias, (int)accumulate, out);
  }
  USC_CHECK_LAUNCH("usc_spconv_gather_gemm");
  return USC_OK;
}

int usc_spconv_pairs_gemm(const float* in, int32_t cin, const float* W, int32_t K, int32_t cout,
                          const int32_t* rows_in, const int32_t* rows_out, const int64_t* koff, int64_t P_capacity,
                          float* out, usc_stream_t s) {
  USC_REQUIRE(cin >= 1 && cout >= 1 && K >= 1 && P_capacity >= 0, "usc_spconv_pairs_gemm: bad sizes");
  if (P_capacity == 0) return USC_OK;
  USC_REQUIRE(in && W && rows_in && rows_out && koff && out, "usc_spconv_pairs_gemm: null pointer");
  GemmParams p{};
  p.in = in; p.W = W; p.out = out; p.cin = cin; p.cout = cout; p.K = K; p.G = 1;
  p.rows_in = rows_in; p.rows_out = rows_out; p.koff = koff;
  const int64_t max_tiles = ceil_div(P_capacity, 32) + K;
  const GemmPlan pl = plan_list(max_tiles, cin, cout);
  dim3 grid((unsigned)ceil_div(max_tiles, 4), (unsigned)ceil_div(cout, pl.NB * 32));
  launch_gemm<true>(pl, grid, as_stream(s), p);
  USC_CHECK_LAUNCH("usc_spconv_pairs_gemm");
  return USC_OK;
}

int64_t usc_spconv_wgrad_ws_bytes(int32_t K, int32_t cin, int32_t cout) {
  return (int64_t)64 * K * cin * cout * (int64_t)sizeof(float);
}

int64_t usc_spconv_wgrad_ws_bytes_rows(int32_t K, int32_t cin, int32_t cout, int64_t n_rows) {
  const int64_t numel = (int64_t)K * cin * cout;
  const int ctiles = cin / 32, cb = cout / 32;
  if (cin % 32 == 0 && cout % 32 == 0 && cb > 0) {
    const int NBf = wgrad_full_nb(cb);
    if (!(NBf == 3 && ctiles % 3 != 0) || ctiles % 4 == 0)
      return wgrad_full_splits(K, ctiles, cb, wgrad_full_ct(ctiles, NBf), NBf, n_rows) * numel * 4;
  }
  return (int64_t)wgrad_splits(K, cin, cout, pick_nb(cout), n_rows) * numel * 4;
}

int64_t usc_spconv_wgrad_table_ws_bytes(int32_t K, int32_t cin, int32_t cout) {
  return (int64_t)kStemSplits * K * cin * cout * 4;
}

int usc_spconv_wgrad_table(const float* in, int32_t cin, const float* dy, int32_t cout, const int32_t* nbr, int32_t K,
                           int64_t n_out, float* dW, int32_t accumulate, void* ws, int64_t ws_bytes, usc_stream_t s) {
  USC_REQUIRE(cin >= 1 && cin <= 4 && cout == 32 && K >= 1 && K <= 32 && n_out >= 0,
              "usc_spconv_wgrad_table: the table form covers <= 4 input channels and 32 output channels (the stem)");
  USC_REQUIRE(in && dy && nbr && dW && ws, "usc_spconv_wgrad_table: null pointer");
  USC_REQUIRE(ws_bytes >= usc_spconv_wgrad_table_ws_bytes(K, cin, cout), "usc_spconv_wgrad_table: workspace too small");
  hipStream_t st = as_stream(s);
  const int per = 32 / cin, groups = (K + per - 1) / per;
  const int64_t numel = (int64_t)K * cin * 32;
  hipLaunchKernelGGL(stem_wgrad_kernel, dim3(kStemSplits, (unsigned)groups), dim3(64 * kStemWaves), 0, st, in, dy, nbr, n_out, (int)K,
                     (int)cin, (float*)ws);
  hipLaunchKernelGGL(wgrad_reduce_kernel, dim3(stream_grid(numel, 256)), dim3(256), 0, st, (const float*)ws, kStemSplits, numel,
                     (int)accumulate, dW);
  USC_CHECK_LAUNCH("usc_spconv_wgrad_table");
  return USC_OK;
}

static int g_wgrad_grid_limit = 0;
void usc_spconv_wgrad_grid_limit(int32_t max_workgroups) { g_wgrad_grid_limit = max_workgroups; }

int usc_spconv_wgrad(const float* a, int32_t cin, const float* b, int32_t cout, int32_t K, const int32_t* a_idx,
                     const int32_t* b_idx, const int64_t* koff, int64_t n_rows, float* dW, int32_t accumulate, void* ws, int64_t ws_bytes,
                     usc_stream_t s) {
  USC_REQUIRE(cin >= 1 && cout >= 1 && K >= 1 && n_rows >= 0, "usc_spconv_wgrad: bad sizes");
  USC_REQUIRE(a && b && dW && ws, "usc_spconv_wgrad: null pointer");
  USC_REQUIRE((a_idx && b_idx && koff) || (!a_idx && K == 1), "usc_spconv_wgrad: pair lists required for K>1");
  const int64_t numel = (int64_t)K * cin * cout;
  hipStream_t st = as_stream(s);
  WgradParams p{};
  p.a = a; p.b = b; p.a_idx = a_idx; p.b_idx = b_idx; p.koff = koff; p.n_rows = n_rows;
  p.partial = (float*)ws; p.cin = cin; p.cout = cout; p.K = K;
  const int ctiles = cin / 32, cb = cout / 32;
  const int NBf = wgrad_full_nb(cb);
  if (cin % 32 == 0 && cout % 32 == 0 && (!(NBf == 3 && ctiles % 3 != 0) || ctiles % 4 == 0)) {
    const int CT = wgrad_full_ct(ctiles, NBf);
    const int64_t S = wgrad_full_splits(K, ctiles, cb, CT, NBf, n_rows);
    USC_REQUIRE(ws_bytes >= S * numel * 4, "usc_spconv_wgrad: workspace too small");
    p.S = (int)S;
    if (S == 1) { p.direct = dW; p.accumulate = accumulate; }
    dim3 grid((unsigned)(K * S), (unsigned)(ctiles / CT), (unsigned)(cb / NBf));
    if (g_wgrad_grid_limit > 0 && (int64_t)K * S > g_wgrad_grid_limit) {
      p.vblocks = (int)(K * S);
      grid.x = (unsigned)g_wgrad_grid_limit;
    }
    const size_t lds = (size_t)4 * NBf * 16 * 64 * sizeof(float);
#define USC_WF(C, N) if (CT == C && NBf == N) { \
      static bool attr_set = false; auto kfn = wgrad_full_kernel<C, N>; \
      if (!attr_set) { (void)hipFuncSetAttribute((const void*)kfn, hipFuncAttributeMaxDynamicSharedMemorySize, 64 * 1024); attr_set = true; } \
      hipLaunchKernelGGL(kfn, grid, dim3(256), lds, st, p, WgradGroup{}); }
    USC_WF(3, 3) USC_WF(2, 3) USC_WF(1, 3) USC_WF(2, 4) USC_WF(1, 4) USC_WF(4, 2) USC_WF(3, 2) USC_WF(2, 2) USC_WF(1, 2) USC_WF(4, 1) USC_WF(3, 1) USC_WF(2, 1) USC_WF(1, 1)
    USC_WF(4, 3)
#undef USC_WF
    if (S > 1)
      hipLaunchKernelGGL(wgrad_reduce_kernel, dim3(stream_grid(numel, 256)), dim3(256), 0, st, (const float*)ws, (int)S,
                         numel, (int)accumulate, dW);
    USC_CHECK_LAUNCH("usc_spconv_wgrad");
    return USC_OK;
  }
  const int NB = pick_nb(cout);
  const bool aligned = (cin % 32 == 0) && (cout % (NB * 32) == 0);
  const int S = wgrad_splits(K, cin, cout, NB, n_rows);
  USC_REQUIRE(ws_bytes >= (int64_t)S * numel * 4, "usc_spconv_wgrad: workspace too small");
  p.S = S;
  dim3 grid((unsigned)(K * S), (unsigned)ceil_div(cin, 32), (unsigned)ceil_div(cout, NB * 32));
  const size_t lds = (size_t)3 * NB * 16 * 64 * sizeof(float);
#define USC_WG(NBv)                                                                          \
  if (aligned) hipLaunchKernelGGL((wgrad_kernel<NBv, true>), grid, dim3(256), lds, st, p);  \
  else hipLaunchKernelGGL((wgrad_kernel<NBv, false>), grid, dim3(256), lds, st, p);
  switch (NB) {
    case 1: USC_WG(1) break;
    case 2: USC_WG(2) break;
    case 3: USC_WG(3) break;
    default: USC_WG(4) break;
  }
#undef USC_WG
  hipLaunchKernelGGL(wgrad_reduce_kernel, dim3(stream_grid(numel, 256)), dim3(256), 0, st, (const float*)ws, S, numel,
                     (int)accumulate, dW);
  USC_CHECK_LAUNCH("usc_spconv_wgrad");
  return USC_OK;
}

int32_t usc_spconv_wgrad_group_max(void) { return kMaxWgradGroup; }

int usc_spconv_wgrad_group_ok(int32_t R, int32_t cin, int32_t cout, int32_t K, int64_t n_rows) {
  if (R < 2 || R > kMaxWgradGroup || cin % 32 || cout % 32 || K < 1 || n_rows <= 0) return 0;
  const int ctiles = cin / 32, cb = cout / 32;
  const int NBf = wgrad_full_nb(cb);
  if (NBf == 3 && ctiles % 3 != 0) return 0;
  const int CT = wgrad_full_ct(ctiles, NBf);
  const int64_t blocks = (int64_t)R * K * (ctiles / CT) * (cb / NBf);
  return blocks >= 256 && n_rows / K <= 2048 ? 1 : 0;
}

int usc_spconv_wgrad_group(int32_t R, const float* const* a, const float* const* b, float* const* dW, int32_t cin,
                           int32_t cout, int32_t K, const int32_t* a_idx, const int32_t* b_idx, const int64_t* koff,
                           int64_t n_rows, int32_t accumulate, usc_stream_t s) {
  USC_REQUIRE(R >= 1 && R <= kMaxWgradGroup, "usc_spconv_wgrad_group: 1 <= R <= %d problems per launch", kMaxWgradGroup);
  USC_REQUIRE(a && b && dW, "usc_spconv_wgrad_group: null pointer table");
  USC_REQUIRE(cin >= 32 && cin % 32 == 0 && cout >= 32 && cout % 32 == 0 && K >= 1 && n_rows >= 0,
              "usc_spconv_wgrad_group: channels must be multiples of 32");
  USC_REQUIRE((a_idx && b_idx && koff) || (!a_idx && K == 1), "usc_spconv_wgrad_group: pair lists required for K>1");
  const int ctiles = cin / 32, cb = cout / 32;
  const int NBf = wgrad_full_nb(cb);
  USC_REQUIRE(!(NBf == 3 && ctiles % 3 != 0), "usc_spconv_wgrad_group: unsupported channel pair %d -> %d", cin, cout);
  if (n_rows == 0) return USC_OK;
  WgradGroup g{};
  g.R = R;
  for (int r = 0; r < R; ++r) {
    USC_REQUIRE(a[r] && b[r] && dW[r], "usc_spconv_wgrad_group: null pointer in problem %d", r);
    g.a[r] = a[r]; g.b[r] = b[r]; g.dW[r] = dW[r];
  }
  WgradParams p{};
  p.a_idx = a_idx; p.b_idx = b_idx; p.koff = koff; p.n_rows = n_rows; p.cin = cin; p.cout = cout; p.K = K;
  p.S = 1; p.accumulate = accumulate; p.direct = g.dW[0]; p.a = g.a[0]; p.b = g.b[0];
  const int CT = wgrad_full_ct(ctiles, NBf);
  hipStream_t st = as_stream(s);
  dim3 grid((unsigned)(R * K), (unsigned)(ctiles / CT), (unsigned)(cb / NBf));
  const size_t lds = (size_t)4 * NBf * 16 * 64 * sizeof(float);
#define USC_WF(C, N) if (CT == C && NBf == N) { \
    static bool attr_set = false; auto kfn = wgrad_full_kernel<C, N>; \
    if (!attr_set) { (void)hipFuncSetAttribute((const void*)kfn, hipFuncAttributeMaxDynamicSharedMemorySize, 64 * 1024); attr_set = true; } \
    hipLaunchKernelGGL(kfn, grid, dim3(256), lds, st, p, g); }
  USC_WF(3, 3) USC_WF(2, 3) USC_WF(1, 3) USC_WF(2, 4) USC_WF(1, 4) USC_WF(4, 2) USC_WF(3, 2) USC_WF(2, 2) USC_WF(1, 2) USC_WF(4, 1) USC_WF(3, 1) USC_WF(2, 1) USC_WF(1, 1)
#undef USC_WF
  USC_CHECK_LAUNCH("usc_spconv_wgrad_group");
  return USC_OK;
}

}
```

unscene3d_amd/csrc/units.hip:

```cpp
#include <stdlib.h>

#include <vector>

#include "common.h"

namespace usc { bool tile_rows_ok(int64_t n, int c); }

using namespace usc;

namespace {

struct WsCursor {
  char* base; int64_t bytes; int64_t off;
  void* take(int64_t n) {
    n = align_up(n > 0 ? n : 16, 256);
    if (off + n > bytes) return nullptr;
    void* p = base + off;
    off += n;
    return p;
  }
  int64_t left() const { return bytes - off; }
  void* rest() { return base + off; }
};

inline bool table_is_compact(int64_t n_out, int cin, int cout, int K) {
  return (usc_spconv_plan(0, n_out, cin, cout, K) >> 12) & 1;
}
inline bool sorted_ok(const usc_kmap* m, int cin, int cout) {
  return m->nbr && m->perm && m->tile_mask && m->K > 1 && m->K <= 32 && cin % 32 == 0 && cout % 32 == 0 && cin <= 4096;
}

int64_t table_gemm_ws(const usc_kmap* m, int64_t n_out, int cin, int cout, int K, bool want_transposed) {
  if (m->nbr && sorted_ok(m, cin, cout) && !table_is_compact(n_out, cin, cout, K))
    return align_up(usc_spconv_sorted_ws_bytes(n_out, cin, cout, K), 256);
  int64_t b = align_up(usc_spconv_gather_gemm_ws_bytes(n_out, cin, cout, K), 256);
  if (want_transposed && !(m->nbr && table_is_compact(n_out, cin, cout, K))) b += align_up((int64_t)K * cin * cout * 4, 256);
  return b;
}

struct Slices { const float* partial = nullptr; int G = 0; };

int table_gemm(const usc_kmap* m, const int32_t* nbr, const float* in, int64_t n_in, int cin, const float* W, int K,
               int cout, int64_t n_out, const float* bias, float* out, int accumulate, int wt, WsCursor ws,
               usc_stream_t s, Slices* left = nullptr) {
  if (left) *left = Slices{};
  if (n_out == 0) return USC_OK;
  const bool compact = nbr && table_is_compact(n_out, cin, cout, K);
  if (nbr && nbr == m->nbr && sorted_ok(m, cin, cout) && !compact) {
    const int64_t b = usc_spconv_sorted_ws_bytes(n_out, cin, cout, K);
    void* w = b > 0 ? ws.take(b) : nullptr;
    USC_REQUIRE(b == 0 || w, "usc unit: workspace too small (sorted gemm)");
    int32_t G = 0;
    const int rc = usc_spconv_sorted_gemm_ex(in, n_in, cin, W, K, cout, nbr, m->perm, m->tile_mask, n_out, bias, out,
                                             accumulate, wt, w, b, left ? &G : nullptr, s);
    if (!rc && left && G > 0) { left->partial = (const float*)w; left->G = G; }
    return rc;
  }
  if (wt && !compact) {
    float* Wt = (float*)ws.take((int64_t)K * cin * cout * 4);
    USC_REQUIRE(Wt, "usc unit: workspace too small (weight transpose)");
    int rc = usc_weight_transpose(W, K, cout, cin, K > 1 ? 1 : 0, Wt, s);
    if (rc) return rc;
    W = Wt;
    wt = 0;
  }
  const int64_t b = usc_spconv_gather_gemm_ws_bytes(n_out, cin, cout, K);
  void* w = b > 0 ? ws.take(b) : nullptr;
  USC_REQUIRE(b == 0 || w, "usc unit: workspace too small (gather gemm)");
  return usc_spconv_gather_gemm(in, n_in, cin, W, K, cout, nbr, n_out, bias, out, accumulate, wt, w, b, s);
}

struct HeldWgrad { const float* x; const float* dy; float* dW; const int32_t* a_idx; const int32_t* b_idx; const int64_t* koff;
                   int64_t rows, ws_bytes; int cin, cout, K; };
struct Lane { hipStream_t st = nullptr; hipEvent_t fork = nullptr, join = nullptr; void* ws = nullptr; int64_t ws_bytes = 0;
              int64_t max_rows = 0; bool dirty = false;
              bool hold = false; int64_t hold_min_rows = 0, release_max_rows = 0; std::vector<HeldWgrad> held; };
Lane g_lane[16];
Lane* lane_for_current_device() {
  int dev = 0;
  if (hipGetDevice(&dev) != hipSuccess || dev < 0 || dev >= 16) return nullptr;
  return g_lane[dev].st ? &g_lane[dev] : nullptr;
}

int lane_release(Lane* lane, usc_stream_t s) {
  lane->hold = false;
  if (lane->held.empty()) return USC_OK;
  if (hipEventRecord(lane->fork, as_stream(s)) != hipSuccess || hipStreamWaitEvent(lane->st, lane->fork, 0) != hipSuccess) {
    lane->held.clear();
    set_error("usc wgrad lane: releasing the held weight gradients failed (event)");
    return USC_ERR_LAUNCH;
  }
  int rc = USC_OK;
  lane->dirty = true;
  for (const HeldWgrad& h : lane->held) {
    rc = usc_spconv_wgrad(h.x, h.cin, h.dy, h.cout, h.K, h.a_idx, h.b_idx, h.koff, h.rows, h.dW, 1, lane->ws, h.ws_bytes,
                          (usc_stream_t)lane->st);
    if (rc) break;
  }
  lane->held.clear();
  return rc;
}

struct ConvShape { int64_t n_in, n_out; };
inline ConvShape conv_shape(const usc_kmap* m, int kind) {
  return kind == USC_CONV_UP ? ConvShape{m->n_out, m->n_in} : ConvShape{m->n_in, m->n_out};
}

int check_map(const usc_kmap* m, int kind, int cin, int cout, const char* who) {
  USC_REQUIRE(m, "%s: null kernel map", who);
  USC_REQUIRE(kind == USC_CONV_SAME || kind == USC_CONV_DOWN || kind == USC_CONV_UP, "%s: unknown conv kind %d", who, kind);
  USC_REQUIRE(cin >= 1 && cout >= 1 && m->K >= 1 && m->n_in >= 0 && m->n_out >= 0, "%s: bad sizes", who);
  USC_REQUIRE(m->nbr || (m->K == 1 && kind == USC_CONV_SAME), "%s: K>1 needs a neighbour table", who);
  USC_REQUIRE(kind != USC_CONV_SAME || m->n_in == m->n_out, "%s: a stride-1 map has n_in == n_out", who);
  return USC_OK;
}


__global__ __launch_bounds__(256) void cat_cols_kernel(const float4* __restrict__ a, int ca4, const float4* __restrict__ b,
                                                      int cb4, float4* __restrict__ dst, int64_t total4) {
  const int c4 = ca4 + cb4;
  for (int64_t e = (int64_t)blockIdx.x * 256 + threadIdx.x; e < total4; e += (int64_t)gridDim.x * 256) {
    const int64_t r = e / c4;
    const int j = (int)(e - r * c4);
    dst[e] = j < ca4 ? a[r * ca4 + j] : b[r * cb4 + (j - ca4)];
  }
}
__global__ __launch_bounds__(256) void split_cols_kernel(const float4* __restrict__ src, int ca4, int cb4, float4* __restrict__ da,
                                                        float4* __restrict__ db, int accumulate, int64_t total4) {
  const int c4 = ca4 + cb4;
  for (int64_t e = (int64_t)blockIdx.x * 256 + threadIdx.x; e < total4; e += (int64_t)gridDim.x * 256) {
    const int64_t r = e / c4;
    const int j = (int)(e - r * c4);
    const float4 v = src[e];
    if (j < ca4) {
      da[r * ca4 + j] = v;
    } else {
      float4* o = db + r * cb4 + (j - ca4);
      if (accumulate) { const float4 t = *o; *o = make_float4(t.x + v.x, t.y + v.y, t.z + v.z, t.w + v.w); }
      else *o = v;
    }
  }
}
__global__ __launch_bounds__(256) void add_inplace_kernel(float* __restrict__ dst, const float* __restrict__ src, int64_t n) {
  const int64_t n4 = n >> 2;
  for (int64_t e = (int64_t)blockIdx.x * 256 + threadIdx.x; e < n4; e += (int64_t)gridDim.x * 256) {
    float4 d = reinterpret_cast<float4*>(dst)[e];
    const float4 v = reinterpret_cast<const float4*>(src)[e];
    d.x += v.x; d.y += v.y; d.z += v.z; d.w += v.w;
    reinterpret_cast<float4*>(dst)[e] = d;
  }
  for (int64_t e = (n4 << 2) + (int64_t)blockIdx.x * 256 + threadIdx.x; e < n; e += (int64_t)gridDim.x * 256) dst[e] += src[e];
}
inline unsigned ew_grid(int64_t work) {
  int64_t g = ceil_div(work, (int64_t)256 * 4);
  if (g < 1) g = 1;
  if (g > 2048) g = 2048;
  return (unsigned)g;
}

struct DeferredWgrads {
  const usc_kmap* map = nullptr; int cin = 0, cout = 0, n = 0;
  const float* a[16]; const float* b[16]; float* dW[16];
};
int flush_deferred(DeferredWgrads& q, void* ws, int64_t ws_bytes, usc_stream_t s) {
  if (q.n == 0) return USC_OK;
  const usc_kmap* m = q.map;
  int rc = USC_OK;
  if (q.n >= 2 && usc_spconv_wgrad_group_ok(q.n, q.cin, q.cout, m->K, m->pair_capacity)) {
    rc = usc_spconv_wgrad_group(q.n, q.a, q.b, q.dW, q.cin, q.cout, m->K, m->pair_in, m->pair_out, m->koff, m->pair_capacity, 1, s);
  } else {
    const int64_t b = usc_spconv_wgrad_ws_bytes_rows(m->K, q.cin, q.cout, m->pair_capacity);
    if (b > ws_bytes) { set_error("usc_program_run: workspace too small (weight gradient)"); rc = USC_ERR_ARG; }
    for (int r = 0; r < q.n && !rc; ++r)
      rc = usc_spconv_wgrad(q.a[r], q.cin, q.b[r], q.cout, m->K, m->pair_in, m->pair_out, m->koff, m->pair_capacity, q.dW[r], 1, ws, b, s);
  }
  q.n = 0;
  q.map = nullptr;
  return rc;
}
}

extern "C" {

int usc_set_wgrad_lane(usc_stream_t lane, void* lane_ws, int64_t lane_ws_bytes, int64_t max_rows) {
  int dev = 0;
  if (hipGetDevice(&dev) != hipSuccess || dev < 0 || dev >= 16) {
    set_error("usc_set_wgrad_lane: unsupported device index");
    return USC_ERR_ARG;
  }
  Lane& e = g_lane[dev];
  if (!lane) {
    e.st = nullptr;
    e.held.clear();
    e.hold = false;
    return USC_OK;
  }
  USC_REQUIRE(lane_ws && lane_ws_bytes > 0 && max_rows > 0, "usc_set_wgrad_lane: the lane needs its own scratch and a row bound");
  if (!e.fork) {
    if (hipEventCreateWithFlags(&e.fork, hipEventDisableTiming) != hipSuccess ||
        hipEventCreateWithFlags(&e.join, hipEventDisableTiming) != hipSuccess) {
      set_error("usc_set_wgrad_lane: hipEventCreate failed");
      return USC_ERR_LAUNCH;
    }
  }
  e.st = as_stream(lane);
  e.ws = lane_ws;
  e.ws_bytes = lane_ws_bytes;
  e.max_rows = max_rows;
  e.dirty = false;
  return USC_OK;
}

int usc_wgrad_lane_hold(int32_t mode, int64_t hold_min_rows, int64_t release_max_rows, usc_stream_t s) {
  Lane* lane = lane_for_current_device();
  if (!lane) return USC_OK;
  if (mode > 0) {
    USC_REQUIRE(hold_min_rows > release_max_rows && release_max_rows >= 0, "usc_wgrad_lane_hold: hold_min_rows must exceed release_max_rows");
    if (!lane->held.empty()) { const int rc = lane_release(lane, s); if (rc) return rc; }
    lane->hold = true;
    lane->hold_min_rows = hold_min_rows;
    lane->release_max_rows = release_max_rows;
    return USC_OK;
  }
  if (mode < 0) {
    lane->held.clear();
    lane->hold = false;
    return USC_OK;
  }
  return lane_release(lane, s);
}

int32_t usc_wgrad_lane_holding(void) {
  Lane* lane = lane_for_current_device();
  return lane && lane->hold ? 1 : 0;
}

int usc_wgrad_lane_join(usc_stream_t s) {
  Lane* lane = lane_for_current_device();
  if (lane && !lane->held.empty()) { const int rc = lane_release(lane, s); if (rc) return rc; }
  if (!lane || !lane->dirty) return USC_OK;
  if (hipEventRecord(lane->join, lane->st) != hipSuccess || hipStreamWaitEvent(as_stream(s), lane->join, 0) != hipSuccess) {
    set_error("usc_wgrad_lane_join: joining the lane failed");
    return USC_ERR_LAUNCH;
  }
  lane->dirty = false;
  return USC_OK;
}

static bool split_dgrad_ok(const usc_kmap* m, int cin, int cout, int planes) {
  return usc_spconv_gather_gemm_split_ws_bytes(m->n_in, cout, cin, m->K, planes) >= 0;
}
static int64_t split_gemm_ws(const usc_kmap* m, int64_t n_src, int c_src, int c_dst, int planes) {
  const int64_t g = usc_spconv_gather_gemm_split_ws_bytes(m->n_out, c_src, c_dst, m->K, planes);
  return align_up(n_src * c_src * planes * 2, 256) + align_up((int64_t)planes * m->K * c_src * c_dst * 2, 256) +
         align_up(g > 0 ? g : 16, 256);
}
static int split_gemm(const usc_kmap* m, const float* src, int64_t n_src, int c_src, const float* W, int c_dst, int64_t n_dst,
                      int planes, int transposed, float* dst, int accumulate, WsCursor cur, usc_stream_t s, const char* who) {
  const int K = m->K;
  const int64_t gb = usc_spconv_gather_gemm_split_ws_bytes(n_dst, c_src, c_dst, K, planes);
  USC_REQUIRE(gb >= 0, "%s: shape not covered by the split kernel (P=%d, K=%d, %d -> %d channels)", who, planes, K, c_src, c_dst);
  uint16_t* xs = (uint16_t*)cur.take(n_src * c_src * planes * 2);
  uint16_t* wp = (uint16_t*)cur.take((int64_t)planes * K * c_src * c_dst * 2);
  void* gws = gb > 0 ? cur.take(gb) : nullptr;
  USC_REQUIRE(xs && wp && (gb == 0 || gws), "%s: workspace too small for the split precision (usc_unit_split_ws_bytes)", who);
  int rc = usc_split_bf16_rows(src, n_src, c_src, planes, xs, s);
  if (rc) return rc;
  rc = transposed ? usc_spconv_pack_w_split(W, K, c_dst, c_src, planes, 1, wp, s)
                  : usc_spconv_pack_w_split(W, K, c_src, c_dst, planes, 0, wp, s);
  if (rc) return rc;
  return usc_spconv_gather_gemm_split(xs, n_src, c_src, wp, K, c_dst, planes, m->nbr, n_dst, nullptr, dst, accumulate, gws, gb, s);
}

static void conv_ws_parts(const usc_kmap* m, int kind, int cin, int cout, int64_t* fwd, int64_t* dgrad, int64_t* wg) {
  const int K = m->K;
  const ConvShape sh = conv_shape(m, kind);
  const int64_t wbytes = align_up((int64_t)K * cin * cout * 4, 256);
  if (kind == USC_CONV_SAME) {
    *fwd = table_gemm_ws(m, sh.n_out, cin, cout, K, false);
    *dgrad = table_gemm_ws(m, sh.n_in, cout, cin, K, true);
  } else if (kind == USC_CONV_DOWN) {
    *fwd = table_gemm_ws(m, sh.n_out, cin, cout, K, false);
    *dgrad = wbytes;
  } else {
    *fwd = 0;
    *dgrad = wbytes + table_gemm_ws(m, sh.n_in, cout, cin, K, false);
  }
  *dgrad = align_up(*dgrad + 256, 256);
  const int64_t rows = m->nbr ? m->pair_capacity : sh.n_in;
  *wg = align_up(usc_spconv_wgrad_ws_bytes_rows(K, cin, cout, rows), 256);
  if (kind == USC_CONV_SAME && m->nbr && cin <= 4 && cout == 32) {
    const int64_t t = align_up(usc_spconv_wgrad_table_ws_bytes(K, cin, cout), 256);
    if (t > *wg) *wg = t;
  }
}

int64_t usc_conv_ws_bytes(const usc_kmap* m, int32_t kind, int32_t cin, int32_t cout) {
  if (!m) return 0;
  int64_t fwd, dgrad, wg;
  conv_ws_parts(m, kind, cin, cout, &fwd, &dgrad, &wg);
  const int64_t bwd = dgrad + wg;
  return (fwd > bwd ? fwd : bwd) + 256;
}

static int conv_forward_impl(const usc_kmap* m, int32_t kind, const float* x, int32_t cin, const float* W, int32_t cout,
                             const float* bias, float* y, void* ws, int64_t ws_bytes, usc_stream_t s, Slices* left);

int usc_conv_forward(const usc_kmap* m, int32_t kind, const float* x, int32_t cin, const float* W, int32_t cout,
                     const float* bias, float* y, void* ws, int64_t ws_bytes, usc_stream_t s) {
  return conv_forward_impl(m, kind, x, cin, W, cout, bias, y, ws, ws_bytes, s, nullptr);
}

static int conv_forward_impl(const usc_kmap* m, int32_t kind, const float* x, int32_t cin, const float* W, int32_t cout,
                             const float* bias, float* y, void* ws, int64_t ws_bytes, usc_stream_t s, Slices* left) {
  if (left) *left = Slices{};
  int rc = check_map(m, kind, cin, cout, "usc_conv_forward");
  if (rc) return rc;
  const ConvShape sh = conv_shape(m, kind);
  if (sh.n_out == 0) return USC_OK;
  USC_REQUIRE(x && W && y, "usc_conv_forward: null pointer");
  WsCursor cur{(char*)ws, ws ? ws_bytes : 0, 0};
  if (kind == USC_CONV_UP) {
    USC_REQUIRE(m->pair_in && m->pair_out && m->koff, "usc_conv_forward: transposed conv needs the pair lists");
    USC_REQUIRE(!bias, "usc_conv_forward: bias is not supported on the pair-list form");
    return usc_spconv_pairs_gemm(x, cin, W, m->K, cout, m->pair_out, m->pair_in, m->koff, sh.n_out, y, s);
  }
  return table_gemm(m, m->nbr, x, sh.n_in, cin, W, m->K, cout, sh.n_out, bias, y, 0, 0, cur, s, left);
}

struct Pending { float* dx = nullptr; const float* partial = nullptr; int G = 0; int64_t n = 0; int c = 0; int accumulate = 0; };

static int flush_pending(Pending& p, usc_stream_t s) {
  if (p.G <= 0) return USC_OK;
  const int rc = usc_group_reduce(p.partial, p.G, p.n, p.c, nullptr, p.accumulate, p.dx, s);
  p = Pending{};
  return rc;
}

static int conv_backward_impl(const usc_kmap* m, int32_t kind, const float* x, int32_t cin, const float* W, int32_t cout,
                              const float* dy, float* dx, int32_t dx_accumulate, float* dW, int32_t dW_accumulate, void* ws,
                              int64_t ws_bytes, usc_stream_t s, Pending* out, int planes = 0);

int usc_conv_backward(const usc_kmap* m, int32_t kind, const float* x, int32_t cin, const float* W, int32_t cout,
                      const float* dy, float* dx, int32_t dx_accumulate, float* dW, int32_t dW_accumulate, void* ws,
                      int64_t ws_bytes, usc_stream_t s) {
  return conv_backward_impl(m, kind, x, cin, W, cout, dy, dx, dx_accumulate, dW, dW_accumulate, ws, ws_bytes, s, nullptr);
}

static int conv_backward_impl(const usc_kmap* m, int32_t kind, const float* x, int32_t cin, const float* W, int32_t cout,
                              const float* dy, float* dx, int32_t dx_accumulate, float* dW, int32_t dW_accumulate, void* ws,
                              int64_t ws_bytes, usc_stream_t s, Pending* out, int planes) {
  if (out) *out = Pending{};
  int rc = check_map(m, kind, cin, cout, "usc_conv_backward");
  if (rc) return rc;
  const ConvShape sh = conv_shape(m, kind);
  const int K = m->K;
  USC_REQUIRE(x && W && dy, "usc_conv_backward: null pointer");
  WsCursor cur{(char*)ws, ws ? ws_bytes : 0, 0};
  if (dW && dW_accumulate && x && dy) {
    Lane* lane = lane_for_current_device();
    const int64_t rows = m->nbr ? m->pair_capacity : sh.n_in;
    const int64_t b = usc_spconv_wgrad_ws_bytes_rows(K, cin, cout, rows);
    const bool lane_ok = lane && sh.n_in > 0 && sh.n_in <= lane->max_rows && sh.n_out <= lane->max_rows &&
                         b <= lane->ws_bytes && (!m->nbr || (m->pair_in && m->pair_out && m->koff));
    const int64_t big = sh.n_in > sh.n_out ? sh.n_in : sh.n_out;
    if (lane && lane->hold && big <= lane->release_max_rows) { rc = lane_release(lane, s); if (rc) return rc; }
    if (lane_ok && lane->hold && big >= lane->hold_min_rows) {
      HeldWgrad h{x, dy, dW, nullptr, nullptr, nullptr, m->nbr ? rows : sh.n_in, b, cin, cout, m->nbr ? K : 1};
      if (m->nbr) {
        h.a_idx = kind == USC_CONV_UP ? m->pair_out : m->pair_in;
        h.b_idx = kind == USC_CONV_UP ? m->pair_in : m->pair_out;
        h.koff = m->koff;
      }
      lane->held.push_back(h);
      dW = nullptr;
    } else if (lane_ok &&
        hipEventRecord(lane->fork, as_stream(s)) == hipSuccess && hipStreamWaitEvent(lane->st, lane->fork, 0) == hipSuccess) {
      usc_stream_t ls = (usc_stream_t)lane->st;
      lane->dirty = true;
      const int64_t bt = usc_spconv_wgrad_table_ws_bytes(K, cin, cout);
      if (kind == USC_CONV_SAME && m->nbr && cin <= 4 && cout == 32 && K <= 32 && bt <= lane->ws_bytes)
        rc = usc_spconv_wgrad_table(x, cin, dy, cout, m->nbr, K, sh.n_out, dW, 1, lane->ws, bt, ls);
      else if (!m->nbr)
        rc = usc_spconv_wgrad(x, cin, dy, cout, 1, nullptr, nullptr, nullptr, sh.n_in, dW, 1, lane->ws, b, ls);
      else if (kind == USC_CONV_UP)
        rc = usc_spconv_wgrad(x, cin, dy, cout, K, m->pair_out, m->pair_in, m->koff, rows, dW, 1, lane->ws, b, ls);
      else
        rc = usc_spconv_wgrad(x, cin, dy, cout, K, m->pair_in, m->pair_out, m->koff, rows, dW, 1, lane->ws, b, ls);
      if (rc) return rc;
      dW = nullptr;
    }
  }
  int64_t dgrad_bytes = 0;
  Slices left;
  const bool split_dx = planes > 0 && kind == USC_CONV_SAME && split_dgrad_ok(m, cin, cout, planes);
  const bool may_defer = !split_dx && out && dx && tile_rows_ok(sh.n_in, cin);
  if (may_defer) {
    int64_t f_, w_;
    conv_ws_parts(m, kind, cin, cout, &f_, &dgrad_bytes, &w_);
    if (dgrad_bytes + w_ > cur.bytes) dgrad_bytes = 0;
  }
  Slices* want = (may_defer && dgrad_bytes > 0) ? &left : nullptr;
  if (dx && sh.n_in > 0) {
    if (split_dx) {
      rc = split_gemm(m, dy, sh.n_out, cout, W, cin, sh.n_in, planes, 1, dx, dx_accumulate, cur, s, "usc_conv_backward");
    } else if (kind == USC_CONV_SAME) {
      rc = table_gemm(m, m->nbr, dy, sh.n_out, cout, W, K, cin, sh.n_in, nullptr, dx, dx_accumulate, 1, cur, s, want);
    } else if (kind == USC_CONV_DOWN) {
      USC_REQUIRE(!dx_accumulate, "usc_conv_backward: accumulate is not supported on the pair-list form");
      USC_REQUIRE(m->pair_in && m->pair_out && m->koff, "usc_conv_backward: strided conv needs the pair lists");
      float* Wt = (float*)cur.take((int64_t)K * cin * cout * 4);
      USC_REQUIRE(Wt, "usc_conv_backward: workspace too small");
      rc = usc_weight_transpose(W, K, cin, cout, 0, Wt, s);
      if (!rc) rc = usc_spconv_pairs_gemm(dy, cout, Wt, K, cin, m->pair_out, m->pair_in, m->koff, sh.n_in, dx, s);
    } else {
      float* Wt = (float*)cur.take((int64_t)K * cin * cout * 4);
      USC_REQUIRE(Wt, "usc_conv_backward: workspace too small");
      rc = usc_weight_transpose(W, K, cin, cout, 0, Wt, s);
      if (!rc) rc = table_gemm(m, m->nbr, dy, sh.n_out, cout, Wt, K, cin, sh.n_in, nullptr, dx, dx_accumulate, 0, cur, s, want);
    }
    if (!rc && left.G > 0) {
      out->dx = dx; out->partial = left.partial; out->G = left.G; out->n = sh.n_in; out->c = cin; out->accumulate = dx_accumulate;
    }
    if (rc) dW = nullptr;
  }
  if (dW) {
    WsCursor wc{(char*)ws, ws ? ws_bytes : 0, left.G > 0 ? dgrad_bytes : 0};
    const int64_t rows = m->nbr ? m->pair_capacity : sh.n_in;
    const int64_t b = usc_spconv_wgrad_ws_bytes_rows(K, cin, cout, rows);
    void* w = wc.take(b);
    if (!w) set_error("usc_conv_backward: workspace too small (weight gradient)");
    const int64_t bt = usc_spconv_wgrad_table_ws_bytes(K, cin, cout);
    if (!w) rc = USC_ERR_ARG;
    else if (kind == USC_CONV_SAME && m->nbr && cin <= 4 && cout == 32 && K <= 32 && (char*)w + bt <= (char*)ws + ws_bytes)
      rc = usc_spconv_wgrad_table(x, cin, dy, cout, m->nbr, K, sh.n_out, dW, dW_accumulate, w, bt, s);
    else if (!m->nbr)
      rc = usc_spconv_wgrad(x, cin, dy, cout, 1, nullptr, nullptr, nullptr, sh.n_in, dW, dW_accumulate, w, b, s);
    else if (kind == USC_CONV_UP)
      rc = usc_spconv_wgrad(x, cin, dy, cout, K, m->pair_out, m->pair_in, m->koff, rows, dW, dW_accumulate, w, b, s);
    else
      rc = usc_spconv_wgrad(x, cin, dy, cout, K, m->pair_in, m->pair_out, m->koff, rows, dW, dW_accumulate, w, b, s);
  }
  return rc;
}

int64_t usc_unit_ws_bytes(const usc_kmap* m, int32_t kind, int32_t cin, int32_t cout) {
  return usc_conv_ws_bytes(m, kind, cin, cout) + align_up(usc_colstats_ws_bytes(0, cout), 256) +
         align_up(2 * (int64_t)cout * 4, 256) + 256;
}

int usc_conv_bn_act_forward(const usc_kmap* m, int32_t kind, const float* x, int32_t cin, const float* W, int32_t cout,
                            const usc_bn* bn, const float* residual, int32_t relu, float* y, float* stats, float* out,
                            void* ws, int64_t ws_bytes, usc_stream_t s) {
  USC_REQUIRE(bn && bn->c == cout, "usc_conv_bn_act_forward: batch-norm width must equal the conv's output width");
  USC_REQUIRE(y && stats && out && bn->gamma && bn->beta, "usc_conv_bn_act_forward: null pointer");
  const ConvShape sh = conv_shape(m, kind);
  WsCursor cur{(char*)ws, ws ? ws_bytes : 0, 0};
  const int64_t sb = usc_colstats_ws_bytes(sh.n_out, cout);
  void* sws = cur.take(sb);
  USC_REQUIRE(sws, "usc_conv_bn_act_forward: workspace too small");
  const bool tile = bn->training && tile_rows_ok(sh.n_out, cout) && sb >= usc_bn_tile_ws_bytes(cout);
  Slices left;
  int rc = conv_forward_impl(m, kind, x, cin, W, cout, nullptr, y, cur.rest(), cur.left(), s, tile ? &left : nullptr);
  if (rc) return rc;
  if (sh.n_out == 0) return USC_OK;
  float* mean = stats, *invstd = stats + cout, *scale = stats + 2 * cout, *shift = stats + 3 * cout;
  if (tile)
    return usc_bn_tile_forward(left.partial, left.G, y, sh.n_out, cout, bn->gamma, bn->beta, bn->eps, bn->momentum,
                               bn->running_mean, bn->running_var, bn->num_batches_tracked, mean, invstd, scale, shift,
                               residual, relu, out, sws, sb, s);
  if (bn->training) {
    rc = usc_bn_forward_stats(y, sh.n_out, cout, bn->gamma, bn->beta, bn->eps, bn->momentum, bn->running_mean,
                              bn->running_var, bn->num_batches_tracked, mean, invstd, scale, shift, sws, sb, s);
  } else {
    USC_REQUIRE(bn->running_mean && bn->running_var, "usc_conv_bn_act_forward: eval mode needs running statistics");
    rc = usc_bn_eval_stats(bn->gamma, bn->beta, bn->running_mean, bn->running_var, bn->eps, cout, mean, invstd, scale,
                           shift, s);
  }
  if (rc) return rc;
  return usc_bn_apply(y, scale, shift, residual, relu, out, sh.n_out, cout, s);
}


int64_t usc_unit_bf16_ws_bytes(const usc_kmap* m, int32_t kind, int32_t cin, int32_t cout) {
  if (!m) return 0;
  const ConvShape sh = conv_shape(m, kind);
  const int64_t g = usc_spconv_gather_gemm_bf16_ws_bytes(sh.n_out, cin, cout, m->K);
  if (g < 0) return -1;
  int64_t b = align_up(usc_colstats_ws_bytes(sh.n_out, cout), 256) + align_up(sh.n_in * cin * 2, 256) + align_up(g, 256);
  if (kind == USC_CONV_UP) b += align_up((int64_t)m->K * sh.n_out * 4, 256);
  return b + 256;
}

int usc_conv_bn_act_forward_bf16(const usc_kmap* m, int32_t kind, const float* x, int32_t cin, const uint16_t* Wp,
                                 int32_t cout, const usc_bn* bn, const float* residual, int32_t relu, float* y,
                                 float* stats, float* out, void* ws, int64_t ws_bytes, usc_stream_t s) {
  int rc = check_map(m, kind, cin, cout, "usc_conv_bn_act_forward_bf16");
  if (rc) return rc;
  USC_REQUIRE(bn && bn->c == cout, "usc_conv_bn_act_forward_bf16: batch-norm width must equal the conv's output width");
  USC_REQUIRE(y && stats && out && bn->gamma && bn->beta, "usc_conv_bn_act_forward_bf16: null pointer");
  const ConvShape sh = conv_shape(m, kind);
  const int64_t gb = usc_spconv_gather_gemm_bf16_ws_bytes(sh.n_out, cin, cout, m->K);
  USC_REQUIRE(gb >= 0, "usc_conv_bn_act_forward_bf16: shape not covered (K=%d, %d -> %d channels)", m->K, cin, cout);
  if (sh.n_out == 0) return USC_OK;
  USC_REQUIRE(x && Wp, "usc_conv_bn_act_forward_bf16: null pointer");
  USC_REQUIRE(m->nbr || kind == USC_CONV_SAME, "usc_conv_bn_act_forward_bf16: strided maps need the child table");
  hipStream_t st = as_stream(s);
  WsCursor cur{(char*)ws, ws ? ws_bytes : 0, 0};
  const int64_t sb = usc_colstats_ws_bytes(sh.n_out, cout);
  void* sws = cur.take(sb);
  uint16_t* xb = (uint16_t*)cur.take(sh.n_in * cin * 2);
  void* gws = gb > 0 ? cur.take(gb) : nullptr;
  int32_t* table = kind == USC_CONV_UP ? (int32_t*)cur.take((int64_t)m->K * sh.n_out * 4) : nullptr;
  USC_REQUIRE(sws && xb && (gb == 0 || gws) && (kind != USC_CONV_UP || table),
              "usc_conv_bn_act_forward_bf16: workspace too small (usc_unit_bf16_ws_bytes)");
  rc = usc_cast_bf16(x, sh.n_in * cin, xb, s);
  if (rc) return rc;
  const int32_t* nbr = m->nbr;
  if (kind == USC_CONV_UP) {
    rc = spconv_up_table(m->nbr, m->K, m->n_out, sh.n_out, table, st);
    if (rc) return rc;
    nbr = table;
  }
  rc = usc_spconv_gather_gemm_bf16(xb, sh.n_in, cin, Wp, m->K, cout, nbr, sh.n_out, nullptr, y, 0, gws, gb, s);
  if (rc) return rc;
  float* mean = stats, *invstd = stats + cout, *scale = stats + 2 * cout, *shift = stats + 3 * cout;
  if (bn->training) {
    rc = usc_bn_forward_stats(y, sh.n_out, cout, bn->gamma, bn->beta, bn->eps, bn->momentum, bn->running_mean,
                              bn->running_var, bn->num_batches_tracked, mean, invstd, scale, shift, sws, sb, s);
  } else {
    USC_REQUIRE(bn->running_mean && bn->running_var, "usc_conv_bn_act_forward_bf16: eval mode needs running statistics");
    rc = usc_bn_eval_stats(bn->gamma, bn->beta, bn->running_mean, bn->running_var, bn->eps, cout, mean, invstd, scale,
                           shift, s);
  }
  if (rc) return rc;
  return usc_bn_apply(y, scale, shift, residual, relu, out, sh.n_out, cout, s);
}

static int unit_backward_impl(const usc_kmap* m, int32_t kind, const float* x, int32_t cin, const float* W, int32_t cout,
                              const usc_bn* bn, const float* y, const float* stats, const float* out_relu,
                              const float* dout, float* dy, float* dres, float* dx, int32_t dx_accumulate, float* dW,
                              int32_t dW_accumulate, float* dgamma, float* dbeta, int32_t dbn_accumulate, void* ws,
                              int64_t ws_bytes, usc_stream_t s, Pending* in, Pending* out, int planes = 0);

int usc_conv_bn_act_backward(const usc_kmap* m, int32_t kind, const float* x, int32_t cin, const float* W, int32_t cout,
                             const usc_bn* bn, const float* y, const float* stats, const float* out_relu,
                             const float* dout, float* dy, float* dres, float* dx, int32_t dx_accumulate, float* dW,
                             int32_t dW_accumulate, float* dgamma, float* dbeta, int32_t dbn_accumulate, void* ws,
                             int64_t ws_bytes, usc_stream_t s) {
  return unit_backward_impl(m, kind, x, cin, W, cout, bn, y, stats, out_relu, dout, dy, dres, dx, dx_accumulate, dW,
                            dW_accumulate, dgamma, dbeta, dbn_accumulate, ws, ws_bytes, s, nullptr, nullptr);
}

static int unit_backward_impl(const usc_kmap* m, int32_t kind, const float* x, int32_t cin, const float* W, int32_t cout,
                              const usc_bn* bn, const float* y, const float* stats, const float* out_relu,
                              const float* dout, float* dy, float* dres, float* dx, int32_t dx_accumulate, float* dW,
                              int32_t dW_accumulate, float* dgamma, float* dbeta, int32_t dbn_accumulate, void* ws,
                              int64_t ws_bytes, usc_stream_t s, Pending* in, Pending* out, int planes) {
  if (out) *out = Pending{};
  USC_REQUIRE(bn && bn->c == cout, "usc_conv_bn_act_backward: batch-norm width must equal the conv's output width");
  USC_REQUIRE(y && stats && dout && dy && dgamma && dbeta && bn->gamma, "usc_conv_bn_act_backward: null pointer");
  const ConvShape sh = conv_shape(m, kind);
  if (sh.n_out == 0) return USC_OK;
  if (planes > 0)
    USC_REQUIRE(ws && ws_bytes >= usc_unit_split_ws_bytes(m, kind, cin, cout, planes),
                "usc_conv_bn_act_backward_split: workspace too small (usc_unit_split_ws_bytes)");
  WsCursor cur{(char*)ws, ws ? ws_bytes : 0, 0};
  const int64_t sb = usc_colstats_ws_bytes(sh.n_out, cout);
  void* sws = cur.take(sb);
  float* red = (float*)cur.take(2 * (int64_t)cout * 4);
  USC_REQUIRE(sws && red, "usc_conv_bn_act_backward: workspace too small");
  const float* mean = stats, *invstd = stats + cout;
  int rc;
  const bool has_in = in && in->G > 0;
  if (has_in) USC_REQUIRE(in->dx == dout && in->n == sh.n_out && in->c == cout, "usc unit: pending slices do not belong to this unit");
  if (tile_rows_ok(sh.n_out, cout) && sb >= usc_bn_tile_ws_bytes(cout)) {
    rc = usc_bn_tile_backward(has_in ? in->partial : nullptr, has_in ? in->G : 0, has_in ? in->accumulate : 0, (float*)dout, y,
                              out_relu, mean, invstd, bn->gamma, sh.n_out, cout, bn->training, dbn_accumulate, dgamma,
                              dbeta, dy, dres, sws, sb, s);
    if (has_in) *in = Pending{};
    if (rc) return rc;
  } else {
    if (has_in) { rc = flush_pending(*in, s); if (rc) return rc; }
    rc = usc_bn_backward_reduce(y, dout, out_relu, mean, invstd, sh.n_out, cout, bn->training, dbn_accumulate, dgamma,
                                dbeta, red, red + cout, sws, sb, s);
    if (rc) return rc;
    rc = usc_bn_backward_dx(y, dout, out_relu, mean, invstd, bn->gamma, red, red + cout, dy, dres, sh.n_out, cout, s);
    if (rc) return rc;
  }
  return conv_backward_impl(m, kind, x, cin, W, cout, dy, dx, dx_accumulate, dW, dW_accumulate, cur.rest(), cur.left(), s, out,
                            planes);
}

static int check_split(const usc_kmap* m, int32_t kind, int32_t P, const char* who) {
  USC_REQUIRE(m, "%s: null kernel map", who);
  USC_REQUIRE(P == 2 || P == 3, "%s: P must be 2 or 3 (got %d)", who, P);
  USC_REQUIRE(kind == USC_CONV_SAME, "%s: the split precision covers stride-1 units only", who);
  return USC_OK;
}

int64_t usc_unit_split_ws_bytes(const usc_kmap* m, int32_t kind, int32_t cin, int32_t cout, int32_t P) {
  if (!m) return 0;
  if ((P != 2 && P != 3) || kind != USC_CONV_SAME) return -1;
  if (usc_spconv_gather_gemm_split_ws_bytes(m->n_out, cin, cout, m->K, P) < 0) return -1;
  const int64_t f = split_gemm_ws(m, m->n_in, cin, cout, P);
  const int64_t b = split_dgrad_ok(m, cin, cout, P) ? split_gemm_ws(m, m->n_out, cout, cin, P) : 0;
  return usc_unit_ws_bytes(m, kind, cin, cout) + (f > b ? f : b) + 256;
}

int usc_conv_bn_act_forward_split(const usc_kmap* m, int32_t kind, const float* x, int32_t cin, const float* W, int32_t cout,
                                  int32_t P, const usc_bn* bn, const float* residual, int32_t relu, float* y, float* stats,
                                  float* out, void* ws, int64_t ws_bytes, usc_stream_t s) {
  int rc = check_split(m, kind, P, "usc_conv_bn_act_forward_split");
  if (rc) return rc;
  rc = check_map(m, kind, cin, cout, "usc_conv_bn_act_forward_split");
  if (rc) return rc;
  USC_REQUIRE(bn && bn->c == cout, "usc_conv_bn_act_forward_split: batch-norm width must equal the conv's output width");
  USC_REQUIRE(y && stats && out && bn->gamma && bn->beta, "usc_conv_bn_act_forward_split: null pointer");
  const ConvShape sh = conv_shape(m, kind);
  USC_REQUIRE(usc_spconv_gather_gemm_split_ws_bytes(sh.n_out, cin, cout, m->K, P) >= 0,
              "usc_conv_bn_act_forward_split: shape not covered (K=%d, %d -> %d channels)", m->K, cin, cout);
  if (sh.n_out == 0) return USC_OK;
  USC_REQUIRE(x && W, "usc_conv_bn_act_forward_split: null pointer");
  WsCursor cur{(char*)ws, ws ? ws_bytes : 0, 0};
  const int64_t sb = usc_colstats_ws_bytes(sh.n_out, cout);
  void* sws = cur.take(sb);
  USC_REQUIRE(sws, "usc_conv_bn_act_forward_split: workspace too small (usc_unit_split_ws_bytes)");
  WsCursor conv{(char*)cur.rest(), cur.left(), 0};
  rc = split_gemm(m, x, sh.n_in, cin, W, cout, sh.n_out, P, 0, y, 0, conv, s, "usc_conv_bn_act_forward_split");
  if (rc) return rc;
  float* mean = stats, *invstd = stats + cout, *scale = stats + 2 * cout, *shift = stats + 3 * cout;
  if (bn->training && tile_rows_ok(sh.n_out, cout) && sb >= usc_bn_tile_ws_bytes(cout))
    return usc_bn_tile_forward(nullptr, 0, y, sh.n_out, cout, bn->gamma, bn->beta, bn->eps, bn->momentum, bn->running_mean,
                               bn->running_var, bn->num_batches_tracked, mean, invstd, scale, shift, residual, relu, out, sws,
                               sb, s);
  if (bn->training) {
    rc = usc_bn_forward_stats(y, sh.n_out, cout, bn->gamma, bn->beta, bn->eps, bn->momentum, bn->running_mean,
                              bn->running_var, bn->num_batches_tracked, mean, invstd, scale, shift, sws, sb, s);
  } else {
    USC_REQUIRE(bn->running_mean && bn->running_var, "usc_conv_bn_act_forward_split: eval mode needs running statistics");
    rc = usc_bn_eval_stats(bn->gamma, bn->beta, bn->running_mean, bn->running_var, bn->eps, cout, mean, invstd, scale,
                           shift, s);
  }
  if (rc) return rc;
  return usc_bn_apply(y, scale, shift, residual, relu, out, sh.n_out, cout, s);
}

int usc_conv_bn_act_backward_split(const usc_kmap* m, int32_t kind, const float* x, int32_t cin, const float* W, int32_t cout,
                                   int32_t P, const usc_bn* bn, const float* y, const float* stats, const float* out_relu,
                                   const float* dout, float* dy, float* dres, float* dx, int32_t dx_accumulate, float* dW,
                                   int32_t dW_accumulate, float* dgamma, float* dbeta, int32_t dbn_accumulate, void* ws,
                                   int64_t ws_bytes, usc_stream_t s) {
  const int rc = check_split(m, kind, P, "usc_conv_bn_act_backward_split");
  if (rc) return rc;
  return unit_backward_impl(m, kind, x, cin, W, cout, bn, y, stats, out_relu, dout, dy, dres, dx, dx_accumulate, dW,
                            dW_accumulate, dgamma, dbeta, dbn_accumulate, ws, ws_bytes, s, nullptr, nullptr, P);
}

int32_t usc_step_size(void) { return (int32_t)sizeof(usc_step); }

static int64_t program_half_bytes(const usc_step* steps, int32_t n_steps) {
  int64_t need = 256;
  if (!steps) return need;
  for (int i = 0; i < n_steps; ++i) {
    const usc_step& t = steps[i];
    if ((t.op == USC_STEP_UNIT_FWD || t.op == USC_STEP_UNIT_BWD) && t.map) {
      int64_t b = usc_unit_ws_bytes(t.map, t.kind, t.cin, t.cout);
      if (t.split_planes) {
        const int64_t sb = usc_unit_split_ws_bytes(t.map, t.kind, t.cin, t.cout, t.split_planes);
        if (sb > b) b = sb;
      }
      if (b > need) need = b;
    } else if (t.op == USC_STEP_UNIT_FWD_BF16 && t.map) {
      const int64_t b = usc_unit_bf16_ws_bytes(t.map, t.kind, t.cin, t.cout);
      if (b > need) need = b;
    }
  }
  return align_up(need, 256);
}

int64_t usc_program_ws_bytes(const usc_step* steps, int32_t n_steps) { return 2 * program_half_bytes(steps, n_steps) + 256; }

int usc_program_run(const usc_step* steps, int32_t begin, int32_t end, void* ws_all, int64_t ws_all_bytes, usc_stream_t s) {
  USC_REQUIRE(steps && begin >= 0 && end >= begin, "usc_program_run: bad step range");
  hipStream_t st = as_stream(s);
  DeferredWgrads q;
  Pending pend;
  int rc = USC_OK;
  const int64_t half = ws_all_bytes > 256 ? (((ws_all_bytes - 256) / 2) & ~(int64_t)255) : 0;
  const bool two = ws_all && half >= program_half_bytes(steps + begin, end - begin);
  void* ws = ws_all;
  int64_t ws_bytes = two ? half : ws_all_bytes;
  for (int i = begin; i < end && !rc; ++i) {
    const usc_step& t = steps[i];
    if (two) ws = (char*)ws_all + (i & 1) * half;
    if (pend.G > 0 && !(t.op == USC_STEP_UNIT_BWD && t.dout == pend.dx)) {
      rc = flush_pending(pend, s);
      if (rc) break;
    }
    switch (t.op) {
      case USC_STEP_UNIT_FWD:
        if (t.split_planes) {
          rc = usc_conv_bn_act_forward_split(t.map, t.kind, t.x, t.cin, t.W, t.cout, t.split_planes, t.bn, t.residual, t.relu,
                                             t.y, t.stats, t.out, ws, ws_bytes, s);
          break;
        }
        rc = usc_conv_bn_act_forward(t.map, t.kind, t.x, t.cin, t.W, t.cout, t.bn, t.residual, t.relu, t.y, t.stats, t.out,
                                     ws, ws_bytes, s);
        break;
      case USC_STEP_UNIT_FWD_BF16:
        rc = usc_conv_bn_act_forward_bf16(t.map, t.kind, t.x, t.cin, (const uint16_t*)t.W, t.cout, t.bn, t.residual, t.relu,
                                          t.y, t.stats, t.out, ws, ws_bytes, s);
        break;
      case USC_STEP_UNIT_BWD: {
        USC_REQUIRE(t.map, "usc_program_run: step %d has no kernel map", i);
        const bool defer = t.defer_wgrad && t.dW && t.dW_accumulate && t.kind == USC_CONV_SAME && t.map->K > 1 && t.map->pair_in &&
                           t.cin % 32 == 0 && t.cout % 32 == 0 &&
                           (usc_spconv_wgrad_group_ok(2, t.cin, t.cout, t.map->K, t.map->pair_capacity) ||
                            usc_spconv_wgrad_group_ok(usc_spconv_wgrad_group_max(), t.cin, t.cout, t.map->K, t.map->pair_capacity));
        if (defer && q.n > 0 && (q.map != t.map || q.cin != t.cin || q.cout != t.cout || q.n == 16)) {
          rc = flush_deferred(q, ws, ws_bytes, s);
          if (rc) break;
        }
        Pending next;
        if (t.split_planes) rc = check_split(t.map, t.kind, t.split_planes, "usc_program_run");
        if (rc) break;
        rc = unit_backward_impl(t.map, t.kind, t.x, t.cin, t.W, t.cout, t.bn, t.y, t.stats, t.out, t.dout, t.dy, t.dres,
                                t.dx, t.dx_accumulate, defer ? nullptr : t.dW, t.dW_accumulate, t.dgamma, t.dbeta,
                                t.dbn_accumulate, ws, ws_bytes, s, &pend, two ? &next : nullptr, t.split_planes);
        if (!rc && pend.G > 0) rc = flush_pending(pend, s);
        pend = next;
        if (!rc && defer) {
          q.map = t.map; q.cin = t.cin; q.cout = t.cout;
          q.a[q.n] = t.x; q.b[q.n] = t.dy; q.dW[q.n] = t.dW;
          ++q.n;
        }
        break;
      }
      case USC_STEP_CAT: {
        USC_REQUIRE(t.a && t.b && t.dst && t.ca % 4 == 0 && t.cb % 4 == 0 && t.n >= 0, "usc_program_run: bad cat step %d", i);
        const int64_t total4 = t.n * ((t.ca + t.cb) / 4);
        if (total4 > 0)
          hipLaunchKernelGGL(cat_cols_kernel, dim3(ew_grid(total4)), dim3(256), 0, st, (const float4*)t.a, t.ca / 4,
                             (const float4*)t.b, t.cb / 4, (float4*)t.dst, total4);
        break;
      }
      case USC_STEP_SPLIT: {
        USC_REQUIRE(t.a && t.dst && t.dst2 && t.ca % 4 == 0 && t.cb % 4 == 0 && t.n >= 0, "usc_program_run: bad split step %d", i);
        const int64_t total4 = t.n * ((t.ca + t.cb) / 4);
        if (total4 > 0)
          hipLaunchKernelGGL(split_cols_kernel, dim3(ew_grid(total4)), dim3(256), 0, st, (const float4*)t.a, t.ca / 4, t.cb / 4,
                             (float4*)t.dst, (float4*)t.dst2, (int)t.accumulate, total4);
        break;
      }
      case USC_STEP_ADD:
        USC_REQUIRE(t.a && t.dst && t.n >= 0, "usc_program_run: bad add step %d", i);
        if (t.n > 0) hipLaunchKernelGGL(add_inplace_kernel, dim3(ew_grid(t.n / 4 + 1)), dim3(256), 0, st, t.dst, t.a, t.n);
        break;
      default:
        set_error("usc_program_run: unknown step op");
        rc = USC_ERR_ARG;
    }
  }
  const int rc3 = flush_pending(pend, s);
  const int rc2 = flush_deferred(q, ws, ws_bytes, s);
  if (rc) return rc;
  if (rc3) return rc3;
  if (rc2) return rc2;
  USC_CHECK_LAUNCH("usc_program_run");
  return USC_OK;
}

}
```

unscene3d_amd/program.py:

```python
from __future__ import annotations

import ctypes as C
import os

import torch

from . import ops, precision, units
from ._lib import STEP_ADD, STEP_CAT, STEP_SPLIT, STEP_UNIT_BWD, STEP_UNIT_FWD, STEP_UNIT_FWD_BF16, Step, check, lib

ENABLED = os.environ.get("USC3D_BACKBONE_PROGRAM", "1") == "1"
SAME, DOWN, UP = units.SAME, units.DOWN, units.UP
_ALIGN = 64


class _Plan:

    def __init__(self):
        self.ops, self.bufs, self.levels = [], {}, []
        self.input = None
        self.params = []

    def new(self, level, c):
        i = len(self.bufs)
        self.bufs[i] = (level, c)
        return i


def _plan(model):
    from .MinkowskiEngine import MinkowskiBatchNorm, MinkowskiConvolution, MinkowskiConvolutionTranspose
    from .models.modules.resnet_block import BasicBlockBase
    pl = _Plan()

    def unit(stage, conv, norm, kind, level, x, res, relu):
        if not (conv.bias is None and isinstance(norm, MinkowskiBatchNorm) and norm.bn.affine
                and norm.bn.momentum is not None):
            raise NotImplementedError
        if kind == SAME and not (isinstance(conv, MinkowskiConvolution) and conv.stride == 1):
            raise NotImplementedError
        if kind == DOWN and not (isinstance(conv, MinkowskiConvolution) and conv.stride == 2 and conv.ksize == 2):
            raise NotImplementedError
        if kind == UP and not (isinstance(conv, MinkowskiConvolutionTranspose) and conv.stride == 2 and conv.ksize == 2):
            raise NotImplementedError
        lout = level + 1 if kind == DOWN else (level - 1 if kind == UP else level)
        y, out = pl.new(lout, conv.out_channels), pl.new(lout, conv.out_channels)
        pl.ops.append(dict(t="unit", stage=stage, conv=conv, bn=norm.bn, kind=kind, lin=level, lout=lout, x=x, res=res,
                           relu=relu, y=y, out=out, cin=conv.in_channels, cout=conv.out_channels,
                           ksize=conv.ksize, kvol=conv.kernel_volume))
        return out

    def blocks(stage, seq, level, x):
        for blk in seq:
            if not isinstance(blk, BasicBlockBase) or blk.conv1.stride != 1 or blk.conv2.stride != 1 \
                    or blk.conv1.kernel_volume == 1 or blk.conv1.ksize != blk.conv2.ksize:
                raise NotImplementedError
            a1 = unit(stage, blk.conv1, blk.norm1, SAME, level, x, None, True)
            r = x
            if blk.downsample is not None:
                ds = blk.downsample
                if len(ds) != 2 or ds[0].kernel_volume != 1:
                    raise NotImplementedError
                r = unit(stage, ds[0], ds[1], SAME, level, x, None, False)
            x = unit(stage, blk.conv2, blk.norm2, SAME, level, a1, r, True)
        return x

    try:
        pl.input = pl.new(0, model.conv0p1s1.in_channels)
        x = unit("conv0p1s1", model.conv0p1s1, model.bn0, SAME, 0, pl.input, None, True)
        skip = [x]
        for i, (cname, nname, bname) in enumerate(model._DOWN):
            x = unit(cname, getattr(model, cname), getattr(model, nname), DOWN, i, x, None, True)
            x = blocks(bname, getattr(model, bname), i + 1, x)
            skip.append(x)
        pl.levels = [x]
        top = len(model._DOWN)
        for j, (cname, nname, bname) in enumerate(model._UP):
            u = unit(cname, getattr(model, cname), getattr(model, nname), UP, top - j, x, None, True)
            s = skip[top - 1 - j]
            ca, cb = pl.bufs[u][1], pl.bufs[s][1]
            if ca % 4 or cb % 4:
                raise NotImplementedError
            c = pl.new(top - 1 - j, ca + cb)
            pl.ops.append(dict(t="cat", stage=cname, a=u, b=s, out=c, level=top - 1 - j, ca=ca, cb=cb))
            x = blocks(bname, getattr(model, bname), top - 1 - j, c)
            pl.levels.append(x)
    except (NotImplementedError, AttributeError):
        return None
    n_levels = top + 1
    pl.n_levels = n_levels
    act, grad = [0] * n_levels, [0] * n_levels
    n_act = n_grad = 0
    for op in pl.ops:
        if op["t"] == "unit":
            act[op["lout"]] += 2 * op["cout"]
            n_act += 3
            grad[op["lout"]] += 2 * op["cout"]
            grad[op["lin"]] += 2 * op["cin"]
            n_grad += 4
        else:
            act[op["level"]] += op["ca"] + op["cb"]
            n_act += 1
            grad[op["level"]] += op["ca"] + op["cb"]
            n_grad += 2
    pl.act_floats, pl.grad_floats, pl.n_act, pl.n_grad = act, grad, n_act, n_grad
    pl.stat_floats = sum(4 * op["cout"] for op in pl.ops if op["t"] == "unit")
    seen, params = set(), []
    for op in pl.ops:
        if op["t"] == "unit":
            for p in (op["conv"].kernel, op["bn"].weight, op["bn"].bias):
                if id(p) not in seen:
                    seen.add(id(p))
                    params.append(p)
    pl.params = params
    return pl


def _module_key(model):
    return tuple(id(m) for m in model.modules())


def plan_of(model):
    cached = model.__dict__.get("_usc_program_plan")
    key = _module_key(model)
    if cached is None or cached[1] != key:
        cached = model.__dict__["_usc_program_plan"] = (_plan(model) or False, key)
    return cached[0] or None


class _Carver:

    def __init__(self, floats, device):
        self.arena = torch.empty(int(floats), dtype=torch.float32, device=device)
        self.base, self.off, self.cap = self.arena.data_ptr(), 0, int(floats)

    def take(self, n):
        off = self.off
        self.off = (off + int(n) + _ALIGN - 1) // _ALIGN * _ALIGN
        if self.off > self.cap:
            raise RuntimeError("step program: arena too small (planning bug)")
        return self.base + 4 * off, off

    def view(self, off, n, c):
        return self.arena[off:off + n * c].view(n, c)


class _Pool:

    def __init__(self, device, chunk_floats):
        self.device, self.chunk_floats = device, int(chunk_floats)
        self.chunks, self.base, self.off, self.cap = [], 0, 0, 0
        self.free = {}

    def take(self, n):
        n = (int(n) + _ALIGN - 1) // _ALIGN * _ALIGN
        lst = self.free.get(n)
        if lst:
            return lst.pop()
        if self.off + n > self.cap:
            self.cap = max(self.chunk_floats, n)
            t = torch.empty(self.cap, dtype=torch.float32, device=self.device)
            self.chunks.append(t)
            self.base, self.off = t.data_ptr(), 0
        p = self.base + 4 * self.off
        self.off += n
        return p

    def release(self, p, n):
        n = (int(n) + _ALIGN - 1) // _ALIGN * _ALIGN
        self.free.setdefault(n, []).append(p)


def usable(model, x):
    if not (ENABLED and units.usable(x.F, None) and x.F.shape[0] > 0):
        return None
    pl = plan_of(model)
    if pl is None:
        return None
    if torch.is_grad_enabled():
        need = [p.requires_grad for p in pl.params]
        if any(need):
            if not all(need) or x.F.requires_grad:
                return None
            for p in pl.params:
                if ops._grad_target(p) is None:
                    return None
    return pl


class _Trunk(torch.autograd.Function):
    @staticmethod
    def forward(ctx, model, pl, cm, ts, bf16, split, feats, *params):
        dev = feats.device
        rows = [cm.coord_map(ts << l).n for l in range(pl.n_levels)]
        floats = sum(r * f for r, f in zip(rows, pl.act_floats)) + pl.stat_floats + (pl.n_act + 8) * _ALIGN
        car = _Carver(floats, dev)
        ptr, offs = {pl.input: feats.data_ptr()}, {}
        steps = (Step * len(pl.ops))()
        kcache = {}

        def kmap(op):
            key = (op["kind"], op["lin"], op["kvol"])
            k = kcache.get(key)
            if k is None:
                t = ts << op["lin"]
                if op["kind"] == SAME:
                    k = cm.kmap_identity(t) if op["kvol"] == 1 else cm.kmap_cube(t, op["ksize"])
                elif op["kind"] == DOWN:
                    k = cm.kmap_down(t)
                else:
                    k = cm.kmap_down(t >> 1)
                kcache[key] = k
            return k

        stats_ptr, kmaps, bnrefs = [], [], []
        for i, op in enumerate(pl.ops):
            st = steps[i]
            if op["t"] == "unit":
                n_out, cout = rows[op["lout"]], op["cout"]
                py, offs[op["y"]] = car.take(n_out * cout)
                po, offs[op["out"]] = car.take(n_out * cout)
                ps, _ = car.take(4 * cout)
                ptr[op["y"]], ptr[op["out"]] = py, po
                km = kmap(op)
                bdesc, _ = units._bn_desc(op["bn"], units._training(op["bn"]))
                bref = C.addressof(bdesc)
                st.op, st.kind, st.cin, st.cout, st.relu = STEP_UNIT_FWD, op["kind"], op["cin"], cout, int(op["relu"])
                st.map, st.bn = C.addressof(km.struct), bref
                st.x, st.W = ptr[op["x"]], op["conv"].kernel.data_ptr()
                wp = bf16.get(id(op["conv"].kernel)) if bf16 else None
                if wp is not None:
                    st.op, st.W = STEP_UNIT_FWD_BF16, wp.data_ptr()
                if split:
                    st.split_planes = split.get(i, 0)
                st.residual = ptr[op["res"]] if op["res"] is not None else None
                st.y, st.stats, st.out = py, ps, po
                stats_ptr.append(ps)
                kmaps.append(km)
                bnrefs.append((bref, bdesc))
            else:
                n = rows[op["level"]]
                pc, offs[op["out"]] = car.take(n * (op["ca"] + op["cb"]))
                ptr[op["out"]] = pc
                st.op, st.a, st.b, st.dst, st.n, st.ca, st.cb = STEP_CAT, ptr[op["a"]], ptr[op["b"]], pc, n, op["ca"], op["cb"]
                stats_ptr.append(None)
                kmaps.append(None)
                bnrefs.append(None)
        wsb = lib.usc_program_ws_bytes(steps, len(pl.ops))
        ws = units.workspace(wsb, dev)
        check(lib.usc_program_run(steps, 0, len(pl.ops), ws.data_ptr(), ws.numel(), ops._stream()), "usc_program_run")
        outs = tuple(car.view(offs[b], rows[pl.bufs[b][0]], pl.bufs[b][1]) for b in pl.levels)
        ctx.state = (model, pl, cm, ts, feats, car, ptr, stats_ptr, kmaps, bnrefs, rows, split)
        return outs

    @staticmethod
    def backward(ctx, *gouts):
        model, pl, cm, ts, feats, car, ptr, stats_ptr, kmaps, bnrefs, rows, split = ctx.state
        dev = feats.device
        gar = _Pool(dev, max(rows[0] * 256, 1 << 20))
        lane = units._lane(dev)
        if lane is not None:
            gar.release = lambda p_, n_: None
            car.arena.record_stream(lane[0])
        keep = [g.contiguous() if g is not None else None for g in gouts]
        G = {}
        held_dy = []
        for b, g in zip(pl.levels, keep):
            if g is not None:
                G[b] = [g.data_ptr(), True, g.numel()]
        steps = (Step * (3 * len(pl.ops) + 8))()
        ns = 0
        segments, cur_params, stage = [], [], None

        def add_step(dst, src, n):
            nonlocal ns
            st = steps[ns]
            ns += 1
            st.op, st.dst, st.a, st.n = STEP_ADD, dst, src, n

        def contribute(bid, numel, can_accumulate):
            cur = G.get(bid)
            if cur is None:
                p = gar.take(numel)
                G[bid] = [p, False, numel]
                return p, 0, None
            if can_accumulate and not cur[1]:
                return cur[0], 1, None
            p = gar.take(numel)
            if cur[1]:
                def fin(p=p, old=cur[0]):
                    add_step(p, old, numel)
                    G[bid] = [p, False, numel]
            else:
                def fin(p=p, old=cur[0]):
                    add_step(old, p, numel)
                    gar.release(p, numel)
            return p, 0, fin

        def consumed(bid):
            cur = G.pop(bid, None)
            if cur is not None and not cur[1]:
                gar.release(cur[0], cur[2])

        for i in range(len(pl.ops) - 1, -1, -1):
            op = pl.ops[i]
            if op["stage"] != stage:
                if stage is not None:
                    segments.append((ns, cur_params))
                    cur_params = []
                    for p_, n_ in held_dy:
                        gar.release(p_, n_)
                    held_dy = []
                stage = op["stage"]
            if op["t"] == "cat":
                g = G.get(op["out"])
                if g is None:
                    continue
                n = rows[op["level"]]
                pa, _, fa = contribute(op["a"], n * op["ca"], False)
                cur_b = G.get(op["b"])
                if cur_b is not None and not cur_b[1]:
                    pb, acc_b, fb = cur_b[0], 1, None
                else:
                    pb, acc_b, fb = contribute(op["b"], n * op["cb"], False)
                st = steps[ns]
                ns += 1
                st.op, st.a, st.dst, st.dst2, st.n, st.ca, st.cb, st.accumulate = STEP_SPLIT, g[0], pa, pb, n, op["ca"], \
                    op["cb"], acc_b
                for f in (fa, fb):
                    if f is not None:
                        f()
                consumed(op["out"])
                continue
            g = G.get(op["out"])
            if g is None:
                continue
            n_out, n_in, cin, cout = rows[op["lout"]], rows[op["lin"]], op["cin"], op["cout"]
            pdy = gar.take(n_out * cout)
            pres, fres = None, None
            if op["res"] is not None:
                pres, _, fres = contribute(op["res"], n_out * cout, False)
            need_dx = op["x"] != pl.input
            pdx, acc, fdx = (None, 0, None)
            if need_dx:
                pdx, acc, fdx = contribute(op["x"], n_in * cin, op["kind"] != DOWN)
            conv, bn = op["conv"], op["bn"]
            tW, tg, tb = ops._grad_target(conv.kernel), ops._grad_target(bn.weight), ops._grad_target(bn.bias)
            if tW is None or tg is None or tb is None:
                raise RuntimeError("step program: a parameter lost its in-place gradient target between forward and "
                                   "backward (keep p.grad allocated: optimizer.zero_grad(set_to_none=False))")
            st = steps[ns]
            ns += 1
            st.op, st.kind, st.cin, st.cout = STEP_UNIT_BWD, op["kind"], cin, cout
            st.map, st.bn = C.addressof(kmaps[i].struct), bnrefs[i][0]
            st.x, st.W = ptr[op["x"]], conv.kernel.data_ptr()
            st.y, st.stats = ptr[op["y"]], stats_ptr[i]
            st.out = ptr[op["out"]] if op["relu"] else None
            st.dout, st.dy, st.dres, st.dx, st.dx_accumulate = g[0], pdy, pres, pdx, acc
            st.dW, st.dW_accumulate, st.dgamma, st.dbeta, st.dbn_accumulate = tW.data_ptr(), 1, tg.data_ptr(), \
                tb.data_ptr(), 1
            st.defer_wgrad = int(units.GROUP_WGRAD)
            if split:
                st.split_planes = split.get(i, 0)
            cur_params.extend((conv.kernel, bn.weight, bn.bias))
            for f in (fres, fdx):
                if f is not None:
                    f()
            consumed(op["out"])
            if st.defer_wgrad and op["kind"] == SAME and op["kvol"] > 1:
                held_dy.append((pdy, n_out * cout))
            else:
                gar.release(pdy, n_out * cout)
        segments.append((ns, cur_params))
        wsb = lib.usc_program_ws_bytes(steps, ns)
        ws = units.workspace(wsb, dev)
        stream = ops._stream()
        begin = 0
        holding = lane is not None and units.LANE_HOLD_MIN_ROWS > units.LANE_RELEASE_ROWS > 0 and \
            any(min(rows[o["lin"]], rows[o["lout"]]) <= units.LANE_RELEASE_ROWS for o in pl.ops if o["t"] == "unit")
        unreported = []
        if holding:
            check(lib.usc_wgrad_lane_hold(1, units.LANE_HOLD_MIN_ROWS, units.LANE_RELEASE_ROWS, stream), "usc_wgrad_lane_hold")
        try:
            for end, plist in segments:
                if end > begin:
                    check(lib.usc_program_run(steps, begin, end, ws.data_ptr(), ws.numel(), stream), "usc_program_run")
                if holding and lib.usc_wgrad_lane_holding():
                    unreported.extend(plist)
                elif plist or unreported:
                    ops._grad_written(*unreported, *plist)
                    ops._params_final(unreported + plist)
                    unreported = []
                begin = end
            if holding:
                check(lib.usc_wgrad_lane_hold(0, 0, 0, stream), "usc_wgrad_lane_hold")
                if unreported:
                    ops._grad_written(*unreported)
                    ops._params_final(unreported)
        except BaseException:
            if holding:
                lib.usc_wgrad_lane_hold(-1, 0, 0, None)
            raise
        if lane is not None:
            for t in gar.chunks:
                t.record_stream(lane[0])
            key = dev.index if dev.index is not None else torch.cuda.current_device()
            units.queue_lane_join(key)
        ctx.state = None
        return (None, None, None, None, None, None, None) + (None,) * len(pl.params)


def trunk(model, x):
    pl = usable(model, x)
    if pl is None:
        return None
    cm, ts = x.coordinate_manager, x._ts()
    feats = x.F.contiguous()
    bf16 = None
    if precision.bf16_active():
        bf16 = {}
        for op in pl.ops:
            if op["t"] == "unit":
                wp = precision.unit_weights(op["conv"].kernel, op["kind"] == SAME, cm.coord_map(ts << op["lout"]).n)
                if wp is not None:
                    bf16[id(op["conv"].kernel)] = wp
    split = None
    if precision.current_training() != "f32" and torch.is_grad_enabled():
        split = {}
        for i, op in enumerate(pl.ops):
            if op["t"] == "unit":
                planes = precision.train_planes(op["conv"].kernel, op["kind"] == SAME, cm.coord_map(ts << op["lout"]).n)
                if planes:
                    split[i] = planes
        split = split or None
    return list(_Trunk.apply(model, pl, cm, ts, bf16, split, feats, *pl.params))
```

Measured before the change: 44.69.

## Batch all weight packing/transposes into one prepack kernel per forward

Adds a batched weight-prepare kernel that packs or transposes every conv weight for both forward and backward in a single launch at the start of the step program. The packed copies are stored in a persistent buffer and handed to the gather-GEMM and backward paths, so per-layer weight_pack and weight_transpose launches are skipped. This is meant to cut kernel-launch count and repeated repacking. The cost is an extra persistent buffer holding two prepared copies of every weight, plus a generation check so backward falls back if the buffer has since been reused.

Result: no change. 44.79 (median of 3 runs) (+0.2%).

```diff
diff --git a/include/usc3d.h b/include/usc3d.h
--- a/include/usc3d.h
+++ b/include/usc3d.h
@@ -63,6 +63,15 @@
 
 int usc_weight_transpose(const float* W, int32_t K, int32_t cin, int32_t cout,
                          int32_t mirror, float* out, usc_stream_t s);
+
+enum usc_wprep_form { USC_WPREP_PACK = 0, USC_WPREP_PACK_WT = 1, USC_WPREP_PACK_WT_PLAIN = 2, USC_WPREP_TRANSPOSE = 3,
+                      USC_WPREP_TRANSPOSE_MIRROR = 4 };
+typedef struct usc_wprep {
+  const float* W;
+  int64_t dst_off;
+  int32_t K, cin, cout, form;
+} usc_wprep;
+int usc_weight_prepare(const usc_wprep* descs, int32_t n, float* dst, int64_t dst_floats, usc_stream_t s);
 
 int usc_spconv_plan(int32_t kind, int64_t n, int32_t cin, int32_t cout,
                     int32_t K);
@@ -97,6 +106,11 @@
                            const int32_t* nbr, int64_t n_out,
                            const float* bias, float* out, int32_t accumulate, int32_t w_transposed,
                            void* ws, int64_t ws_bytes, usc_stream_t s);
+int usc_spconv_gather_gemm_prepared(const float* in, int64_t n_in, int32_t cin,
+                                    const float* Wp, int32_t K, int32_t cout,
+                                    const int32_t* nbr, int64_t n_out,
+                                    const float* bias, float* out, int32_t accumulate,
+                                    usc_stream_t s);
 
 int usc_spconv_pairs_gemm(const float* in, int32_t cin, const float* W,
                           int32_t K, int32_t cout, const int32_t* rows_in,
@@ -266,6 +280,8 @@
   const float* b;
   float* dst;
   float* dst2;
+  const float* W_fwd_prep;
+  const float* W_bwd_prep;
   int64_t n;
   int32_t ca, cb;
   int32_t split_planes, reserved;
@@ -273,6 +289,9 @@
 int32_t usc_step_size(void);
 int64_t usc_program_ws_bytes(const usc_step* steps, int32_t n_steps);
 int usc_program_run(const usc_step* steps, int32_t begin, int32_t end, void* ws, int64_t ws_bytes, usc_stream_t s);
+int64_t usc_program_prepack_floats(const usc_step* steps, int32_t n_steps);
+int usc_program_prepack(usc_step* steps, int32_t n_steps, int32_t with_backward, float* buf, int64_t buf_floats,
+                        usc_stream_t s);
 
 
 int64_t usc_colstats_ws_bytes(int64_t n, int32_t c);
diff --git a/unscene3d_amd/_lib.py b/unscene3d_amd/_lib.py
--- a/unscene3d_amd/_lib.py
+++ b/unscene3d_amd/_lib.py
@@ -35,10 +35,15 @@
                 ("map", _p), ("bn", _p),
                 ("x", _p), ("W", _p), ("residual", _p), ("y", _p), ("stats", _p), ("out", _p),
                 ("dout", _p), ("dy", _p), ("dres", _p), ("dx", _p), ("dW", _p), ("dgamma", _p), ("dbeta", _p),
-                ("a", _p), ("b", _p), ("dst", _p), ("dst2", _p), ("n", _i64), ("ca", _i32), ("cb", _i32),
-                ("split_planes", _i32), ("reserved", _i32)]
-
-
+                ("a", _p), ("b", _p), ("dst", _p), ("dst2", _p), ("W_fwd_prep", _p), ("W_bwd_prep", _p),
+                ("n", _i64), ("ca", _i32), ("cb", _i32), ("split_planes", _i32), ("reserved", _i32)]
+
+
+class WPrep(C.Structure):
+    _fields_ = [("W", _p), ("dst_off", _i64), ("K", _i32), ("cin", _i32), ("cout", _i32), ("form", _i32)]
+
+
+WPREP_PACK, WPREP_PACK_WT, WPREP_PACK_WT_PLAIN, WPREP_TRANSPOSE, WPREP_TRANSPOSE_MIRROR = 0, 1, 2, 3, 4
 _sp = C.POINTER(Step)
 STEP_UNIT_FWD, STEP_UNIT_BWD, STEP_CAT, STEP_SPLIT, STEP_ADD, STEP_UNIT_FWD_BF16 = 0, 1, 2, 3, 4, 5
 
@@ -59,6 +64,10 @@
     "usc_rulebook_ws_bytes": (_i64, [_i64, _i64]),
     "usc_rulebook_compact": (C.c_int, [_p, _i64, _i64, _p, _p, _p, _p, _i64, _p]),
     "usc_weight_transpose": (C.c_int, [_p, _i32, _i32, _i32, _i32, _p, _p]),
+    "usc_weight_prepare": (C.c_int, [C.POINTER(WPrep), _i32, _p, _i64, _p]),
+    "usc_spconv_gather_gemm_prepared": (C.c_int, [_p, _i64, _i32, _p, _i32, _i32, _p, _i64, _p, _p, _i32, _p]),
+    "usc_program_prepack_floats": (_i64, [_sp, _i32]),
+    "usc_program_prepack": (C.c_int, [_sp, _i32, _i32, _p, _i64, _p]),
     "usc_spconv_plan": (C.c_int, [_i32, _i64, _i32, _i32, _i32]),
     "usc_spconv_gather_gemm_ws_bytes": (_i64, [_i64, _i32, _i32, _i32]),
     "usc_spconv_gather_gemm": (C.c_int, [_p, _i64, _i32, _p, _i32, _i32, _p, _i64, _p, _p, _i32, _i32, _p, _i64, _p]),
diff --git a/unscene3d_amd/csrc/spconv.hip b/unscene3d_amd/csrc/spconv.hip
--- a/unscene3d_amd/csrc/spconv.hip
+++ b/unscene3d_amd/csrc/spconv.hip
@@ -911,34 +911,67 @@
   }
 }
 
+template <typename I>
+__device__ __forceinline__ I weight_transpose_src(I j, int K, int cin, int cout, int mirror) {
+  const I per = (I)cin * (I)cout;
+  const int k = (int)(j / per);
+  const I rem = j - (I)k * per;
+  const int co = (int)(rem / (I)cin), ci = (int)(rem - (I)co * (I)cin);
+  const int ks = mirror ? (K - 1 - k) : k;
+  return (I)ks * per + (I)ci * (I)cout + (I)co;
+}
 __global__ void weight_transpose_kernel(const float* __restrict__ W, int K, int cin, int cout, int mirror,
                                         float* __restrict__ out) {
-  const int64_t per = (int64_t)cin * cout;
-  const int64_t total = per * K;
-  for (int64_t j = (int64_t)blockIdx.x * blockDim.x + threadIdx.x; j < total; j += (int64_t)gridDim.x * blockDim.x) {
-    const int k = (int)(j / per);
-    const int64_t rem = j - (int64_t)k * per;
-    const int co = (int)(rem / cin), ci = (int)(rem - (int64_t)co * cin);
-    const int ks = mirror ? (K - 1 - k) : k;
-    out[j] = W[(int64_t)ks * per + (int64_t)ci * cout + co];
-  }
-}
-
+  const int64_t total = (int64_t)cin * cout * K;
+  for (int64_t j = (int64_t)blockIdx.x * blockDim.x + threadIdx.x; j < total; j += (int64_t)gridDim.x * blockDim.x)
+    out[j] = W[weight_transpose_src<int64_t>(j, K, cin, cout, mirror)];
+}
+
+template <typename I>
+__device__ __forceinline__ I weight_pack_src(I e, int K, int cin, int cout, int NB, int wt) {
+  const int nq = cin >> 3, BN = NB * 32;
+  I r = e;
+  const int j = (int)(r & 3); r >>= 2;
+  const int ln = (int)(r & 63); r >>= 6;
+  const int nb = (int)(r % (I)NB); r /= (I)NB;
+  const int q = (int)(r % (I)nq); r /= (I)nq;
+  const int k = (int)(r % (I)K);
+  const int cb = (int)(r / (I)K);
+  const int i = ln & 31, h = ln >> 5;
+  const int c = 8 * q + 4 * h + j, n = cb * BN + NB * i + nb;
+  if (wt == 0) return ((I)k * (I)cin + (I)c) * (I)cout + (I)n;
+  return ((I)(wt == 1 ? K - 1 - k : k) * (I)cout + (I)n) * (I)cin + (I)c;
+}
 __global__ void weight_pack_kernel(const float* __restrict__ W, int K, int cin, int cout, int NB, int wt,
                                    float* __restrict__ out) {
   const int64_t total = (int64_t)K * cin * cout;
-  const int nq = cin >> 3, BN = NB * 32;
-  for (int64_t e = (int64_t)blockIdx.x * blockDim.x + threadIdx.x; e < total; e += (int64_t)gridDim.x * blockDim.x) {
-    int64_t r = e;
-    const int j = (int)(r & 3); r >>= 2;
-    const int ln = (int)(r & 63); r >>= 6;
-    const int nb = (int)(r % NB); r /= NB;
-    const int q = (int)(r % nq); r /= nq;
-    const int k = (int)(r % K);
-    const int cb = (int)(r / K);
-    const int i = ln & 31, h = ln >> 5;
-    const int c = 8 * q + 4 * h + j, n = cb * BN + NB * i + nb;
-    out[e] = wt ? W[((int64_t)(K - 1 - k) * cout + n) * cin + c] : W[((int64_t)k * cin + c) * cout + n];
+  for (int64_t e = (int64_t)blockIdx.x * blockDim.x + threadIdx.x; e < total; e += (int64_t)gridDim.x * blockDim.x)
+    out[e] = W[weight_pack_src<int64_t>(e, K, cin, cout, NB, wt)];
+}
+
+constexpr int kWprepMax = 64;
+constexpr int kWprepBlockItems = 2048;
+struct WprepBatch {
+  const float* W[kWprepMax];
+  int64_t dst_off[kWprepMax];
+  int32_t K[kWprepMax], cin[kWprepMax], cout[kWprepMax], form[kWprepMax], nb[kWprepMax], blk_end[kWprepMax];
+  int32_t n;
+};
+__global__ __launch_bounds__(256) void weight_prepare_kernel(const WprepBatch b, float* __restrict__ dst) {
+  int d = 0;
+  while (d < b.n - 1 && (int)blockIdx.x >= b.blk_end[d]) ++d;
+  const int first = d > 0 ? b.blk_end[d - 1] : 0;
+  const int K = b.K[d], cin = b.cin[d], cout = b.cout[d], form = b.form[d], NB = b.nb[d];
+  const float* __restrict__ W = b.W[d];
+  float* __restrict__ out = dst + b.dst_off[d];
+  const uint32_t total = (uint32_t)K * (uint32_t)cin * (uint32_t)cout;
+  const uint32_t lo = (uint32_t)((int)blockIdx.x - first) * kWprepBlockItems;
+  const uint32_t hi = lo + kWprepBlockItems < total ? lo + kWprepBlockItems : total;
+  if (form <= USC_WPREP_PACK_WT_PLAIN) {
+    for (uint32_t e = lo + threadIdx.x; e < hi; e += 256) out[e] = W[weight_pack_src<uint32_t>(e, K, cin, cout, NB, form)];
+  } else {
+    const int mirror = form == USC_WPREP_TRANSPOSE_MIRROR;
+    for (uint32_t e = lo + threadIdx.x; e < hi; e += 256) out[e] = W[weight_transpose_src<uint32_t>(e, K, cin, cout, mirror)];
   }
 }
 
@@ -982,14 +1015,17 @@
   return has_table && cin >= 1 && cin <= 4 && cout == 32 && K >= 1 && K <= 32;
 }
 
+static int compact_nb(int cout) {
+  const int cb = cout / 32;
+  return (cb % 3 == 0) ? 3 : (cb % 2 == 0 ? 2 : 1);
+}
 static GemmPlan plan_table(int64_t n_out, int cin, int cout, int K) {
   GemmPlan pl{pick_nb(cout), 1, false, 0};
   const bool al = (cin % 32 == 0) && (cout % 32 == 0);
   if (!al) return pl;
   pl.aligned = true;
   if (K > 1 && K <= kMaxK && n_out >= 24576 && cin >= 64 && cin <= kZeroRowFloats) {
-    const int cb = cout / 32;
-    const int nb = (cb % 3 == 0) ? 3 : (cb % 2 == 0 ? 2 : 1);
+    const int nb = compact_nb(cout);
     constexpr int kTmMax3 = 192;
     constexpr int64_t kTileSlots = 256;
     const int tm_max = nb == 3 ? kTmMax3 : 256;
@@ -1132,9 +1168,59 @@
   return khz;
 }
 
+static int gather_gemm_impl(const float* in, int64_t n_in, int32_t cin, const float* W, int32_t K, int32_t cout,
+                            const int32_t* nbr, int64_t n_out, const float* bias, float* out, int32_t accumulate,
+                            int32_t w_transposed, void* ws, int64_t ws_bytes, usc_stream_t s, const float* packed);
+
 int usc_spconv_gather_gemm(const float* in, int64_t n_in, int32_t cin, const float* W, int32_t K, int32_t cout,
                            const int32_t* nbr, int64_t n_out, const float* bias, float* out, int32_t accumulate,
                            int32_t w_transposed, void* ws, int64_t ws_bytes, usc_stream_t s) {
+  return gather_gemm_impl(in, n_in, cin, W, K, cout, nbr, n_out, bias, out, accumulate, w_transposed, ws, ws_bytes, s, nullptr);
+}
+
+int usc_spconv_gather_gemm_prepared(const float* in, int64_t n_in, int32_t cin, const float* Wp, int32_t K, int32_t cout,
+                                    const int32_t* nbr, int64_t n_out, const float* bias, float* out, int32_t accumulate,
+                                    usc_stream_t s) {
+  USC_REQUIRE(Wp, "usc_spconv_gather_gemm_prepared: null pointer");
+  USC_REQUIRE(cin >= 1 && cout >= 1 && K >= 1 && n_out >= 0 && nbr && plan_table(n_out, cin, cout, K).TM > 0,
+              "usc_spconv_gather_gemm_prepared: packed weights are read by the tile-compacted kernel only "
+              "(usc_spconv_plan bit 12)");
+  return gather_gemm_impl(in, n_in, cin, Wp, K, cout, nbr, n_out, bias, out, accumulate, 0, nullptr, 0, s, Wp);
+}
+
+int usc_weight_prepare(const usc_wprep* descs, int32_t n, float* dst, int64_t dst_floats, usc_stream_t s) {
+  USC_REQUIRE(n >= 0 && (n == 0 || (descs && dst)), "usc_weight_prepare: bad argument");
+  for (int i = 0; i < n; ++i) {
+    const usc_wprep& d = descs[i];
+    USC_REQUIRE(d.W && d.K >= 1 && d.cin >= 1 && d.cout >= 1 && d.form >= USC_WPREP_PACK && d.form <= USC_WPREP_TRANSPOSE_MIRROR,
+                "usc_weight_prepare: bad descriptor %d", i);
+    const int64_t total = (int64_t)d.K * d.cin * d.cout;
+    USC_REQUIRE(d.dst_off >= 0 && d.dst_off + total <= dst_floats, "usc_weight_prepare: descriptor %d leaves the destination", i);
+    USC_REQUIRE(d.form > USC_WPREP_PACK_WT_PLAIN || (d.cin % 32 == 0 && d.cout % 32 == 0),
+                "usc_weight_prepare: the packed forms need channel counts in multiples of 32 (descriptor %d)", i);
+    USC_REQUIRE(total <= (int64_t)1 << 30, "usc_weight_prepare: descriptor %d is too large", i);
+  }
+  hipStream_t st = as_stream(s);
+  for (int i0 = 0; i0 < n; i0 += kWprepMax) {
+    WprepBatch b{};
+    int blocks = 0;
+    b.n = n - i0 < kWprepMax ? n - i0 : kWprepMax;
+    for (int j = 0; j < b.n; ++j) {
+      const usc_wprep& d = descs[i0 + j];
+      b.W[j] = d.W; b.dst_off[j] = d.dst_off; b.K[j] = d.K; b.cin[j] = d.cin; b.cout[j] = d.cout; b.form[j] = d.form;
+      b.nb[j] = compact_nb(d.cout);
+      blocks += (int)ceil_div((int64_t)d.K * d.cin * d.cout, (int64_t)kWprepBlockItems);
+      b.blk_end[j] = blocks;
+    }
+    hipLaunchKernelGGL(weight_prepare_kernel, dim3((unsigned)blocks), dim3(256), 0, st, b, dst);
+  }
+  USC_CHECK_LAUNCH("usc_weight_prepare");
+  return USC_OK;
+}
+
+static int gather_gemm_impl(const float* in, int64_t n_in, int32_t cin, const float* W, int32_t K, int32_t cout,
+                            const int32_t* nbr, int64_t n_out, const float* bias, float* out, int32_t accumulate,
+                            int32_t w_transposed, void* ws, int64_t ws_bytes, usc_stream_t s, const float* packed) {
   USC_REQUIRE(cin >= 1 && cout >= 1 && K >= 1 && n_out >= 0 && n_in >= 0, "usc_spconv_gather_gemm: bad sizes");
   USC_REQUIRE(nbr || K == 1, "usc_spconv_gather_gemm: K>1 needs a neighbour table");
   USC_REQUIRE(nbr || n_in == n_out, "usc_spconv_gather_gemm: identity map needs n_in == n_out");
@@ -1163,10 +1249,14 @@
   p.wt1 = wt1 ? 1 : 0;
   if (pl.TM > 0) {
     p.TM = pl.TM;
-    USC_REQUIRE(ws && ws_bytes >= (int64_t)K * cin * cout * 4, "usc_spconv_gather_gemm: workspace too small");
-    hipLaunchKernelGGL(weight_pack_kernel, dim3(stream_grid((int64_t)K * cin * cout, 256)), dim3(256), 0, st, W, (int)K,
-                       (int)cin, (int)cout, pl.NB, (int)w_transposed, (float*)ws);
-    p.W = (const float*)ws;
+    if (packed) {
+      p.W = packed;
+    } else {
+      USC_REQUIRE(ws && ws_bytes >= (int64_t)K * cin * cout * 4, "usc_spconv_gather_gemm: workspace too small");
+      hipLaunchKernelGGL(weight_pack_kernel, dim3(stream_grid((int64_t)K * cin * cout, 256)), dim3(256), 0, st, W, (int)K,
+                         (int)cin, (int)cout, pl.NB, w_transposed ? 1 : 0, (float*)ws);
+      p.W = (const float*)ws;
+    }
     dim3 cgrid((unsigned)ceil_div(n_out, pl.TM), (unsigned)(cout / (pl.NB * 32)));
     const size_t lds = compact_lds_bytes(pl.NB, pl.TM);
     if (g_lstats.ring && g_lstats.count < g_lstats.slots) {
diff --git a/unscene3d_amd/csrc/units.hip b/unscene3d_amd/csrc/units.hip
--- a/unscene3d_amd/csrc/units.hip
+++ b/unscene3d_amd/csrc/units.hip
@@ -42,10 +42,12 @@
 
 int table_gemm(const usc_kmap* m, const int32_t* nbr, const float* in, int64_t n_in, int cin, const float* W, int K,
                int cout, int64_t n_out, const float* bias, float* out, int accumulate, int wt, WsCursor ws,
-               usc_stream_t s, Slices* left = nullptr) {
+               usc_stream_t s, Slices* left = nullptr, const float* prepared = nullptr) {
   if (left) *left = Slices{};
   if (n_out == 0) return USC_OK;
   const bool compact = nbr && table_is_compact(n_out, cin, cout, K);
+  if (prepared && compact)
+    return usc_spconv_gather_gemm_prepared(in, n_in, cin, prepared, K, cout, nbr, n_out, bias, out, accumulate, s);
   if (nbr && nbr == m->nbr && sorted_ok(m, cin, cout) && !compact) {
     const int64_t b = usc_spconv_sorted_ws_bytes(n_out, cin, cout, K);
     void* w = b > 0 ? ws.take(b) : nullptr;
@@ -56,6 +58,10 @@
     if (!rc && left && G > 0) { left->partial = (const float*)w; left->G = G; }
     return rc;
   }
+  if (wt && prepared) {
+    W = prepared;
+    wt = 0;
+  }
   if (wt && !compact) {
     float* Wt = (float*)ws.take((int64_t)K * cin * cout * 4);
     USC_REQUIRE(Wt, "usc unit: workspace too small (weight transpose)");
@@ -68,6 +74,16 @@
   void* w = b > 0 ? ws.take(b) : nullptr;
   USC_REQUIRE(b == 0 || w, "usc unit: workspace too small (gather gemm)");
   return usc_spconv_gather_gemm(in, n_in, cin, W, K, cout, nbr, n_out, bias, out, accumulate, wt, w, b, s);
+}
+
+int table_prep_form(const usc_kmap* m, int64_t n_out, int cin, int cout, int K, int wt, bool pre_t) {
+  if (n_out == 0) return -1;
+  const bool compact = m->nbr && table_is_compact(n_out, cin, cout, K);
+  if (compact) return pre_t ? USC_WPREP_PACK_WT_PLAIN : (wt ? USC_WPREP_PACK_WT : USC_WPREP_PACK);
+  if (pre_t) return USC_WPREP_TRANSPOSE;
+  if (m->nbr && sorted_ok(m, cin, cout)) return -1;
+  if (wt) return K > 1 ? USC_WPREP_TRANSPOSE_MIRROR : USC_WPREP_TRANSPOSE;
+  return -1;
 }
 
 struct HeldWgrad { const float* x; const float* dy; float* dW; const int32_t* a_idx; const int32_t* b_idx; const int64_t* koff;
@@ -304,7 +320,8 @@
 }
 
 static int conv_forward_impl(const usc_kmap* m, int32_t kind, const float* x, int32_t cin, const float* W, int32_t cout,
-                             const float* bias, float* y, void* ws, int64_t ws_bytes, usc_stream_t s, Slices* left);
+                             const float* bias, float* y, void* ws, int64_t ws_bytes, usc_stream_t s, Slices* left,
+                             const float* Wprep = nullptr);
 
 int usc_conv_forward(const usc_kmap* m, int32_t kind, const float* x, int32_t cin, const float* W, int32_t cout,
                      const float* bias, float* y, void* ws, int64_t ws_bytes, usc_stream_t s) {
@@ -312,7 +329,8 @@
 }
 
 static int conv_forward_impl(const usc_kmap* m, int32_t kind, const float* x, int32_t cin, const float* W, int32_t cout,
-                             const float* bias, float* y, void* ws, int64_t ws_bytes, usc_stream_t s, Slices* left) {
+                             const float* bias, float* y, void* ws, int64_t ws_bytes, usc_stream_t s, Slices* left,
+                             const float* Wprep) {
   if (left) *left = Slices{};
   int rc = check_map(m, kind, cin, cout, "usc_conv_forward");
   if (rc) return rc;
@@ -325,7 +343,7 @@
     USC_REQUIRE(!bias, "usc_conv_forward: bias is not supported on the pair-list form");
     return usc_spconv_pairs_gemm(x, cin, W, m->K, cout, m->pair_out, m->pair_in, m->koff, sh.n_out, y, s);
   }
-  return table_gemm(m, m->nbr, x, sh.n_in, cin, W, m->K, cout, sh.n_out, bias, y, 0, 0, cur, s, left);
+  return table_gemm(m, m->nbr, x, sh.n_in, cin, W, m->K, cout, sh.n_out, bias, y, 0, 0, cur, s, left, Wprep);
 }
 
 struct Pending { float* dx = nullptr; const float* partial = nullptr; int G = 0; int64_t n = 0; int c = 0; int accumulate = 0; };
@@ -339,7 +357,7 @@
 
 static int conv_backward_impl(const usc_kmap* m, int32_t kind, const float* x, int32_t cin, const float* W, int32_t cout,
                               const float* dy, float* dx, int32_t dx_accumulate, float* dW, int32_t dW_accumulate, void* ws,
-                              int64_t ws_bytes, usc_stream_t s, Pending* out, int planes = 0);
+                              int64_t ws_bytes, usc_stream_t s, Pending* out, int planes = 0, const float* Wprep = nullptr);
 
 int usc_conv_backward(const usc_kmap* m, int32_t kind, const float* x, int32_t cin, const float* W, int32_t cout,
                       const float* dy, float* dx, int32_t dx_accumulate, float* dW, int32_t dW_accumulate, void* ws,
@@ -349,7 +367,7 @@
 
 static int conv_backward_impl(const usc_kmap* m, int32_t kind, const float* x, int32_t cin, const float* W, int32_t cout,
                               const float* dy, float* dx, int32_t dx_accumulate, float* dW, int32_t dW_accumulate, void* ws,
-                              int64_t ws_bytes, usc_stream_t s, Pending* out, int planes) {
+                              int64_t ws_bytes, usc_stream_t s, Pending* out, int planes, const float* Wprep) {
   if (out) *out = Pending{};
   int rc = check_map(m, kind, cin, cout, "usc_conv_backward");
   if (rc) return rc;
@@ -405,7 +423,15 @@
     if (split_dx) {
       rc = split_gemm(m, dy, sh.n_out, cout, W, cin, sh.n_in, planes, 1, dx, dx_accumulate, cur, s, "usc_conv_backward");
     } else if (kind == USC_CONV_SAME) {
-      rc = table_gemm(m, m->nbr, dy, sh.n_out, cout, W, K, cin, sh.n_in, nullptr, dx, dx_accumulate, 1, cur, s, want);
+      rc = table_gemm(m, m->nbr, dy, sh.n_out, cout, W, K, cin, sh.n_in, nullptr, dx, dx_accumulate, 1, cur, s, want, Wprep);
+    } else if (Wprep && kind == USC_CONV_DOWN) {
+      USC_REQUIRE(!dx_accumulate, "usc_conv_backward: accumulate is not supported on the pair-list form");
+      USC_REQUIRE(m->pair_in && m->pair_out && m->koff, "usc_conv_backward: strided conv needs the pair lists");
+      rc = usc_spconv_pairs_gemm(dy, cout, Wprep, K, cin, m->pair_out, m->pair_in, m->koff, sh.n_in, dx, s);
+    } else if (Wprep) {
+      const bool packed = table_prep_form(m, sh.n_in, cout, cin, K, 0, true) == USC_WPREP_PACK_WT_PLAIN;
+      rc = table_gemm(m, m->nbr, dy, sh.n_out, cout, Wprep, K, cin, sh.n_in, nullptr, dx, dx_accumulate, 0, cur, s, want,
+                      packed ? Wprep : nullptr);
     } else if (kind == USC_CONV_DOWN) {
       USC_REQUIRE(!dx_accumulate, "usc_conv_backward: accumulate is not supported on the pair-list form");
       USC_REQUIRE(m->pair_in && m->pair_out && m->koff, "usc_conv_backward: strided conv needs the pair lists");
@@ -449,9 +475,19 @@
          align_up(2 * (int64_t)cout * 4, 256) + 256;
 }
 
+static int unit_forward_impl(const usc_kmap* m, int32_t kind, const float* x, int32_t cin, const float* W, int32_t cout,
+                             const usc_bn* bn, const float* residual, int32_t relu, float* y, float* stats, float* out,
+                             void* ws, int64_t ws_bytes, usc_stream_t s, const float* Wprep);
+
 int usc_conv_bn_act_forward(const usc_kmap* m, int32_t kind, const float* x, int32_t cin, const float* W, int32_t cout,
                             const usc_bn* bn, const float* residual, int32_t relu, float* y, float* stats, float* out,
                             void* ws, int64_t ws_bytes, usc_stream_t s) {
+  return unit_forward_impl(m, kind, x, cin, W, cout, bn, residual, relu, y, stats, out, ws, ws_bytes, s, nullptr);
+}
+
+static int unit_forward_impl(const usc_kmap* m, int32_t kind, const float* x, int32_t cin, const float* W, int32_t cout,
+                             const usc_bn* bn, const float* residual, int32_t relu, float* y, float* stats, float* out,
+                             void* ws, int64_t ws_bytes, usc_stream_t s, const float* Wprep) {
   USC_REQUIRE(bn && bn->c == cout, "usc_conv_bn_act_forward: batch-norm width must equal the conv's output width");
   USC_REQUIRE(y && stats && out && bn->gamma && bn->beta, "usc_conv_bn_act_forward: null pointer");
   const ConvShape sh = conv_shape(m, kind);
@@ -461,7 +497,7 @@
   USC_REQUIRE(sws, "usc_conv_bn_act_forward: workspace too small");
   const bool tile = bn->training && tile_rows_ok(sh.n_out, cout) && sb >= usc_bn_tile_ws_bytes(cout);
   Slices left;
-  int rc = conv_forward_impl(m, kind, x, cin, W, cout, nullptr, y, cur.rest(), cur.left(), s, tile ? &left : nullptr);
+  int rc = conv_forward_impl(m, kind, x, cin, W, cout, nullptr, y, cur.rest(), cur.left(), s, tile ? &left : nullptr, Wprep);
   if (rc) return rc;
   if (sh.n_out == 0) return USC_OK;
   float* mean = stats, *invstd = stats + cout, *scale = stats + 2 * cout, *shift = stats + 3 * cout;
@@ -541,7 +577,8 @@
                               const usc_bn* bn, const float* y, const float* stats, const float* out_relu,
                               const float* dout, float* dy, float* dres, float* dx, int32_t dx_accumulate, float* dW,
                               int32_t dW_accumulate, float* dgamma, float* dbeta, int32_t dbn_accumulate, void* ws,
-                              int64_t ws_bytes, usc_stream_t s, Pending* in, Pending* out, int planes = 0);
+                              int64_t ws_bytes, usc_stream_t s, Pending* in, Pending* out, int planes = 0,
+                              const float* Wprep = nullptr);
 
 int usc_conv_bn_act_backward(const usc_kmap* m, int32_t kind, const float* x, int32_t cin, const float* W, int32_t cout,
                              const usc_bn* bn, const float* y, const float* stats, const float* out_relu,
@@ -556,7 +593,7 @@
                               const usc_bn* bn, const float* y, const float* stats, const float* out_relu,
                               const float* dout, float* dy, float* dres, float* dx, int32_t dx_accumulate, float* dW,
                               int32_t dW_accumulate, float* dgamma, float* dbeta, int32_t dbn_accumulate, void* ws,
-                              int64_t ws_bytes, usc_stream_t s, Pending* in, Pending* out, int planes) {
+                              int64_t ws_bytes, usc_stream_t s, Pending* in, Pending* out, int planes, const float* Wprep) {
   if (out) *out = Pending{};
   USC_REQUIRE(bn && bn->c == cout, "usc_conv_bn_act_backward: batch-norm width must equal the conv's output width");
   USC_REQUIRE(y && stats && dout && dy && dgamma && dbeta && bn->gamma, "usc_conv_bn_act_backward: null pointer");
@@ -589,7 +626,7 @@
     if (rc) return rc;
   }
   return conv_backward_impl(m, kind, x, cin, W, cout, dy, dx, dx_accumulate, dW, dW_accumulate, cur.rest(), cur.left(), s, out,
-                            planes);
+                            planes, Wprep);
 }
 
 static int check_split(const usc_kmap* m, int32_t kind, int32_t P, const char* who) {
@@ -680,6 +717,59 @@
 }
 
 int64_t usc_program_ws_bytes(const usc_step* steps, int32_t n_steps) { return 2 * program_half_bytes(steps, n_steps) + 256; }
+
+static void unit_prep_forms(const usc_step& t, int* ffwd, int* fbwd) {
+  const usc_kmap* m = t.map;
+  const ConvShape sh = conv_shape(m, t.kind);
+  const int K = m->K;
+  *ffwd = t.kind == USC_CONV_UP ? -1 : table_prep_form(m, sh.n_out, t.cin, t.cout, K, 0, false);
+  if (sh.n_in == 0) *fbwd = -1;
+  else if (t.kind == USC_CONV_SAME) *fbwd = table_prep_form(m, sh.n_in, t.cout, t.cin, K, 1, false);
+  else if (t.kind == USC_CONV_DOWN) *fbwd = USC_WPREP_TRANSPOSE;
+  else *fbwd = table_prep_form(m, sh.n_in, t.cout, t.cin, K, 0, true);
+}
+static bool prepack_step(const usc_step& t) {
+  return t.op == USC_STEP_UNIT_FWD && !t.split_planes && t.map && t.W && t.cin >= 1 && t.cout >= 1 && t.map->K >= 1 &&
+         (t.map->nbr || (t.map->K == 1 && t.kind == USC_CONV_SAME));
+}
+
+int64_t usc_program_prepack_floats(const usc_step* steps, int32_t n_steps) {
+  int64_t need = 64;
+  if (!steps) return need;
+  for (int i = 0; i < n_steps; ++i)
+    if (prepack_step(steps[i])) need += 2 * align_up((int64_t)steps[i].map->K * steps[i].cin * steps[i].cout, 64);
+  return need;
+}
+
+int usc_program_prepack(usc_step* steps, int32_t n_steps, int32_t with_backward, float* buf, int64_t buf_floats,
+                        usc_stream_t s) {
+  USC_REQUIRE(steps && n_steps >= 0 && buf, "usc_program_prepack: null pointer");
+  for (int i = 0; i < n_steps; ++i) steps[i].W_fwd_prep = steps[i].W_bwd_prep = nullptr;
+  USC_REQUIRE(buf_floats >= usc_program_prepack_floats(steps, n_steps),
+              "usc_program_prepack: buffer too small (usc_program_prepack_floats)");
+  std::vector<usc_wprep> descs;
+  int64_t off = 0;
+  for (int i = 0; i < n_steps; ++i) {
+    usc_step& t = steps[i];
+    if (!prepack_step(t)) continue;
+    int form[2];
+    unit_prep_forms(t, &form[0], &form[1]);
+    if (!with_backward) form[1] = -1;
+    const int64_t numel = (int64_t)t.map->K * t.cin * t.cout;
+    for (int f = 0; f < 2; ++f) {
+      if (form[f] < 0) continue;
+      const bool swap = form[f] == USC_WPREP_PACK_WT || form[f] == USC_WPREP_PACK_WT_PLAIN;
+      descs.push_back(usc_wprep{t.W, off, t.map->K, swap ? t.cout : t.cin, swap ? t.cin : t.cout, form[f]});
+      (f ? t.W_bwd_prep : t.W_fwd_prep) = buf + off;
+      off += align_up(numel, 64);
+    }
+  }
+  if (descs.empty()) return USC_OK;
+  const int rc = usc_weight_prepare(descs.data(), (int32_t)descs.size(), buf, buf_floats, s);
+  if (rc)
+    for (int i = 0; i < n_steps; ++i) steps[i].W_fwd_prep = steps[i].W_bwd_prep = nullptr;
+  return rc;
+}
 
 int usc_program_run(const usc_step* steps, int32_t begin, int32_t end, void* ws_all, int64_t ws_all_bytes, usc_stream_t s) {
   USC_REQUIRE(steps && begin >= 0 && end >= begin, "usc_program_run: bad step range");
@@ -705,8 +795,8 @@
                                              t.y, t.stats, t.out, ws, ws_bytes, s);
           break;
         }
-        rc = usc_conv_bn_act_forward(t.map, t.kind, t.x, t.cin, t.W, t.cout, t.bn, t.residual, t.relu, t.y, t.stats, t.out,
-                                     ws, ws_bytes, s);
+        rc = unit_forward_impl(t.map, t.kind, t.x, t.cin, t.W, t.cout, t.bn, t.residual, t.relu, t.y, t.stats, t.out, ws,
+                               ws_bytes, s, t.W_fwd_prep);
         break;
       case USC_STEP_UNIT_FWD_BF16:
         rc = usc_conv_bn_act_forward_bf16(t.map, t.kind, t.x, t.cin, (const uint16_t*)t.W, t.cout, t.bn, t.residual, t.relu,
@@ -727,7 +817,8 @@
         if (rc) break;
         rc = unit_backward_impl(t.map, t.kind, t.x, t.cin, t.W, t.cout, t.bn, t.y, t.stats, t.out, t.dout, t.dy, t.dres,
                                 t.dx, t.dx_accumulate, defer ? nullptr : t.dW, t.dW_accumulate, t.dgamma, t.dbeta,
-                                t.dbn_accumulate, ws, ws_bytes, s, &pend, two ? &next : nullptr, t.split_planes);
+                                t.dbn_accumulate, ws, ws_bytes, s, &pend, two ? &next : nullptr, t.split_planes,
+                                t.split_planes ? nullptr : t.W_bwd_prep);
         if (!rc && pend.G > 0) rc = flush_pending(pend, s);
         pend = next;
         if (!rc && defer) {
diff --git a/unscene3d_amd/program.py b/unscene3d_amd/program.py
--- a/unscene3d_amd/program.py
+++ b/unscene3d_amd/program.py
@@ -19,6 +19,8 @@
         self.ops, self.bufs, self.levels = [], {}, []
         self.input = None
         self.params = []
+        self.prepack = os.environ.get("USC3D_WEIGHT_PREPACK", "1") == "1"
+        self.prep_bufs, self.prep_gen = {}, 0
 
     def new(self, level, c):
         i = len(self.bufs)
@@ -244,17 +246,29 @@
                 stats_ptr.append(None)
                 kmaps.append(None)
                 bnrefs.append(None)
+        wprep = None
+        if pl.prepack:
+            need = lib.usc_program_prepack_floats(steps, len(pl.ops))
+            buf = pl.prep_bufs.get(dev)
+            if buf is None or buf.numel() < need:
+                buf = pl.prep_bufs[dev] = torch.empty(need, dtype=torch.float32, device=dev)
+            check(lib.usc_program_prepack(steps, len(pl.ops), int(any(ctx.needs_input_grad)), buf.data_ptr(), buf.numel(),
+                                          ops._stream()), "usc_program_prepack")
+            pl.prep_gen += 1
+            wprep = (pl.prep_gen, [steps[i].W_bwd_prep for i in range(len(pl.ops))])
         wsb = lib.usc_program_ws_bytes(steps, len(pl.ops))
         ws = units.workspace(wsb, dev)
         check(lib.usc_program_run(steps, 0, len(pl.ops), ws.data_ptr(), ws.numel(), ops._stream()), "usc_program_run")
         outs = tuple(car.view(offs[b], rows[pl.bufs[b][0]], pl.bufs[b][1]) for b in pl.levels)
-        ctx.state = (model, pl, cm, ts, feats, car, ptr, stats_ptr, kmaps, bnrefs, rows, split)
+        ctx.state = (model, pl, cm, ts, feats, car, ptr, stats_ptr, kmaps, bnrefs, rows, split, wprep)
         return outs
 
     @staticmethod
     def backward(ctx, *gouts):
-        model, pl, cm, ts, feats, car, ptr, stats_ptr, kmaps, bnrefs, rows, split = ctx.state
+        model, pl, cm, ts, feats, car, ptr, stats_ptr, kmaps, bnrefs, rows, split, wprep = ctx.state
         dev = feats.device
+        if wprep is not None and wprep[0] != pl.prep_gen:
+            wprep = None
         gar = _Pool(dev, max(rows[0] * 256, 1 << 20))
         lane = units._lane(dev)
         if lane is not None:
@@ -360,6 +374,8 @@
             st.defer_wgrad = int(units.GROUP_WGRAD)
             if split:
                 st.split_planes = split.get(i, 0)
+            if wprep is not None:
+                st.W_bwd_prep = wprep[1][i]
             cur_params.extend((conv.kernel, bn.weight, bn.bias))
             for f in (fres, fdx):
                 if f is not None:
```
